# gligen/GLIGEN

Hardware: AMD Instinct MI355X
Metric: 512x512 images/sec @ 50 PLMS steps, box+text (CFG 7.5), UNet step ms (higher is better)
Workload: dtype bf16; 1 GPU; C2: box+text, 8 boxes (30 grounding tokens), 512x512, 50 PLMS steps, CFG 7.5, bf16 storage / fp32 accumulate; plms_steps=50, unet_evals_per_image=102, hipgraph=True, batches_in_flight=3

## Files before the change

gligen_amd/_lib.py:

```python
from __future__ import annotations

import ctypes as C
from pathlib import Path

_HERE = Path(__file__).resolve().parent
LIB_PATH = _HERE / "libgligen_amd.so"


class GligenAmdError(RuntimeError):
    pass


class UNetConfig(C.Structure):
    _fields_ = [
        ("in_channels", C.c_int), ("out_channels", C.c_int), ("model_channels", C.c_int),
        ("num_res_blocks", C.c_int), ("num_heads", C.c_int), ("context_dim", C.c_int),
        ("n_mult", C.c_int), ("channel_mult", C.c_int * 8),
        ("n_attn", C.c_int), ("attention_resolutions", C.c_int * 8),
        ("inpaint_mode", C.c_int), ("grounding_kind", C.c_int),
        ("gr_in_dim", C.c_int), ("gr_out_dim", C.c_int), ("max_persons", C.c_int), ("fuser_kind", C.c_int),
        ("extra_channels", C.c_int), ("tok_resize", C.c_int), ("tok_in_dim", C.c_int),
    ]


# ... 36 lines not shown
        ("fuser_scale", C.POINTER(C.c_float)), ("guidance_scale", C.c_float),
        ("x", C.c_void_p), ("inpaint_extra", C.c_void_p), ("mask", C.c_void_p), ("x0", C.c_void_p),
        ("noise", C.c_void_p), ("mask_B", C.c_int), ("x0_B", C.c_int), ("noise_B", C.c_int),
        ("sqrt_ac", C.POINTER(C.c_float)), ("sqrt_1mac", C.POINTER(C.c_float)),
        ("use_graph", C.c_int), ("sd_conv_w", C.c_void_p), ("sd_conv_b", C.c_void_p), ("sd_conv_step", C.c_int), ("ddim", C.c_int),
    ]


class TrainUNetIn(C.Structure):
    _fields_ = [(n, C.c_int) for n in ("B", "H", "W", "ctx_T", "Ng")] + \
               [(n, C.c_void_p) for n in ("x", "timesteps", "context", "boxes", "masks", "positive_embeddings", "target")] + \
               [("fuser_scale", C.c_float)] + [(n, C.c_void_p) for n in ("text_masks", "image_masks", "image_embeddings")] + [("checkpoint", C.c_int), ("use_weight_cache", C.c_int)]


class TrainSpatialIn(C.Structure):
    _fields_ = [("map", C.c_void_p)] + [(n, C.c_int) for n in ("map_channels", "map_h", "map_w")] + [("mask", C.c_void_p), ("extra", C.c_void_p)] + \
               [(n, C.c_int) for n in ("extra_in_channels", "extra_h", "extra_w", "ds_resize", "ds_mode", "ds_n_in", "ds_mid")]


class TrainSpatialClassesIn(C.Structure):
    _fields_ = [("map", C.c_void_p), ("map_h", C.c_int), ("map_w", C.c_int), ("mask", C.c_void_p), ("extra", C.c_void_p)] + \
               [(n, C.c_int) for n in ("extra_h", "extra_w", "ds_resize", "ds_mode", "ds_n_in", "ds_mid")]


class TrainStepInputsArgs(C.Structure):
    _fields_ = [("struct_size", C.c_uint)] + [(n, C.c_int) for n in ("B", "C", "H", "W", "n_t", "n_boxes", "inpaint")] + \
               [(n, C.c_void_p) for n in ("z", "noise", "timesteps", "sqrt_alphas_cumprod", "sqrt_one_minus_alphas_cumprod", "boxes", "mask",
                                          "x_rows", "target_rows", "t_float")]


class BoxCalibration(C.Structure):
    _fields_ = [("hbm_copy_gbs", C.c_float), ("lds_dma_tbs", C.c_float), ("mfma_bf16_tflops", C.c_float)]


class MfmaCalibration(C.Structure):
    _fields_ = [("tflops", C.c_float), ("sclk_mhz", C.c_float), ("ms", C.c_float), ("cycles_per_mfma", C.c_float)]


class ProfRec(C.Structure):
    _fields_ = [("name", C.c_char * 96), ("calls", C.c_int), ("ms", C.c_double), ("flops", C.c_double), ("bytes", C.c_double)]


_P = C.c_void_p
_I = C.c_int
SYMBOLS = {
    "gl_last_error": (C.c_char_p, []),
    "gl_ctx_create": (_I, [_I, C.c_size_t, C.POINTER(_P)]),
    "gl_ctx_fork": (_I, [_P, C.c_size_t, C.POINTER(_P)]),
    "gl_ctx_memory": (_I, [_P, C.POINTER(C.c_size_t), C.POINTER(C.c_size_t), C.POINTER(_I)]),
    "gl_ctx_destroy": (_I, [_P]),
    "gl_unet_configure": (_I, [_P, C.POINTER(UNetConfig)]),
    "gl_vae_configure": (_I, [_P, C.POINTER(VaeConfig)]),
    "gl_weight_upload": (_I, [_P, C.c_char_p, _P, _I, C.POINTER(C.c_int64), _I]),
    "gl_finalize": (_I, [_P]),
    "gl_clip_text_configure": (_I, [_P, C.POINTER(ClipTextConfig)]),
    "gl_clip_text_encode": (_I, [_P, _P, _P, _I, _I, _P, _P, _P]),
    "gl_clip_vision_configure": (_I, [_P, C.POINTER(ClipVisionConfig)]),
    "gl_clip_vision_encode": (_I, [_P, _P, _I, _P, _P, _P, _P]),
    "gl_op_clip_attention": (_I, [_P, _P, _P, _I, _I, _I, _I, _P]),
    "gl_unet_set_cond": (_I, [_P, _I, _P, _I, C.POINTER(Grounding), _P]),
    "gl_unet_set_fuser_scale": (_I, [_P, C.c_float, _P]),
    "gl_unet_set_fuser_scales": (_I, [_P, C.POINTER(C.c_float), _I, _P]),
    "gl_unet_grounding_tokens": (_I, [_P, _P, _P]),
    "gl_op_spatial_tokens": (_I, [_P, _P, _I, _I, _I, _I, _P, _P, _P]),
    "gl_op_grounding_downsample": (_I, [_P, _P, _I, _I, _I, _I, _I, _I, _I, _P, _P, _I, _P, _P, _I, _P, _P]),
    "gl_unet_restore_first_conv": (_I, [_P, _P, _P, _P]),
    "gl_unet_forward": (_I, [_P, _I, _I, _I, _P, _I, _P, _P, _I, _P, _P]),
    "gl_vae_decode": (_I, [_P, _I, _I, _I, _P, _P, _P]),
    "gl_vae_encode": (_I, [_P, _I, _I, _I, _P, _P, _P, _P]),
    "gl_sample_plms": (_I, [_P, C.POINTER(PlmsArgs), _P]),
    "gl_sampler_timing": (_I, [_P, C.POINTER(C.c_float), C.POINTER(C.c_float), C.POINTER(_I)]),
    "gl_unet_profile": (_I, [_P, _I, _I, _I, _P, _I, _P, _P, _I, _P, C.POINTER(ProfRec), _I, C.POINTER(_I), _P]),
    "gl_to_uint8": (_I, [_P, _P, _I, _I, _I, _P]),
    "gl_arena_high_water": (_I, [_P, C.POINTER(C.c_size_t)]),
    "gl_launch_count": (_I, [_P, C.POINTER(C.c_int64)]),
    "gl_set_ff_rows_policy": (_I, [_I]),
    "gl_ff_rows_policy_report": (_I, [C.c_char_p, C.c_size_t]),
    "gl_box_calibrate": (_I, [_P, C.POINTER(BoxCalibration), _P]),
    "gl_mfma_calibrate": (_I, [_P, _I, _I, _I, _I, C.c_float, C.POINTER(MfmaCalibration), _P]),
    "gl_op_linear": (_I, [_P, _P, _P, _P, _P, _P, _I, _I, _I, _I, _I, _P]),
    "gl_op_geglu": (_I, [_P, _P, _P, _P, _P, _I, _I, _I, _P]),
    "gl_op_ln_linear": (_I, [_P, _P, _I, _I, _P, _P, _P, _I, _P, _P, _P, _P, _I, _I, _I, _P, _P, C.POINTER(_I), _P]),
    "gl_op_feedforward": (_I, [_P, _P, _I, _I, _P, _P, _P, _P, _P, _P, _P, _P, _P, _P, C.POINTER(_I), _P]),
    "gl_train_block_param_names": (C.POINTER(C.c_char_p), []),
    "gl_op_block_train": (_I, [_P, _P, C.POINTER(_P), _P, _P, _P, _P, _P, _P, _P, _P, C.POINTER(_P), _P]),
    "gl_train_st_param_names": (C.POINTER(C.c_char_p), []),
    "gl_op_st_train": (_I, [_P, _P, C.POINTER(_P), _P, _P, _P, _P, _P, _P, _P, _P, C.POINTER(_P), _P]),
    "gl_train_resblock_param_names": (C.POINTER(C.c_char_p), []),
    "gl_op_resblock_train": (_I, [_P, _P, C.POINTER(_P), _P, _P, _P, _P, _P, _P, _P]),
    "gl_op_resample_train": (_I, [_P, _I, _I, _I, _I, _I, _P, _P, _P, _P, _P, _P, _P, _P]),
    "gl_unet_train_step": (_I, [_P, C.POINTER(UNetConfig), C.POINTER(TrainUNetIn), _I, C.POINTER(C.c_char_p), C.POINTER(_P), C.POINTER(_P), _P, _P, _P]),
    "gl_unet_train_step_spatial": (_I, [_P, C.POINTER(UNetConfig), C.POINTER(TrainUNetIn), C.POINTER(TrainSpatialIn), _I, C.POINTER(C.c_char_p),
                                        C.POINTER(_P), C.POINTER(_P), _P, _P, _P]),
    "gl_train_wait_grads": (_I, [_P, _I, _P]),
    "gl_train_weight_cache": (_I, [_P, _I, C.POINTER(C.c_size_t)]),
    "gl_op_adamw_step": (_I, [_P, _P, _P, _P, _P, C.c_int64, C.c_double, C.c_double, C.c_double, C.c_double, C.c_double, _I, _P]),
    "gl_op_ff_chain": (_I, [_P, _P, _I, _I] + [_P] * 16),
    "gl_op_conv3x3": (_I, [_P, _P, _I, _P, _I, _I, _I, _I, _P, _P, _I, _I, _I, _I, _P, _P, _P]),
    "gl_op_groupnorm": (_I, [_P, _P, _I, _P, _I, _I, _I, _P, _P, C.c_float, _I, _P, _P]),
    "gl_op_gn_silu_conv3x3": (_I, [_P, _P, _I, _P, _I, _I, _I, _I, _P, _P, C.c_float, _P, _P, _I, _P, _P, _P, _I, _P, _P]),
    "gl_op_layernorm": (_I, [_P, _P, _P, _I, _I, _I, _I, _I, _P, _P, C.c_float, _P, _P]),
    "gl_op_attention": (_I, [_P, _P, _P, _I, _I, _I, _I, _I, _I, _P, _P, _P, _P, _P]),
    "gl_attn_regime_counters": (_I, [_P, _I, C.POINTER(C.c_uint), C.POINTER(C.c_uint)]),
    "gl_op_ff_chain_q": (_I, [_P, _P, _I, _I, _I, _P, _P, _P, _P, _P, _P, _P, _P, _P, _P, _P, _P, _P, _P, _P, _P, _P]),
    "gl_op_proj_attention": (_I, [_P, _P, _I, _I, _I, _I, _P, _P, _P, _P, _P, _P, _P, _P, _I, _P, _P, C.POINTER(_I), _P]),
}

IMAGE_SYMBOLS = {
    "gl_op_image_resample": (_I, [_P, C.POINTER(ImageDesc), _I, _I, _I, C.POINTER(C.c_float), _P, _P]),
    "gl_image_resample_coeffs": (_I, [_I, _I, _I, C.POINTER(_I), C.POINTER(_I), _I, C.POINTER(_I), _I]),
}

MAP_SYMBOLS = {
    "gl_op_class_map_resize": (_I, [_P, C.POINTER(ClassMapDesc), _I, _I, _I, _P, _P]),
    "gl_class_map_index_table": (_I, [_I, _I, _I, C.POINTER(_I), _I]),
    "gl_op_spatial_tokens_classes": (_I, [_P, _P, _I, _I, _I, _P, _P, _P]),
    "gl_op_grounding_downsample_classes": (_I, [_P, _P, _I, _I, _I, _I, _I, _P, _P, _I, _P, _P, _I, _P, _P]),
}

TRAIN_MAP_SYMBOLS = {
    "gl_unet_train_step_spatial_classes": (_I, [_P, C.POINTER(UNetConfig), C.POINTER(TrainUNetIn), C.POINTER(TrainSpatialClassesIn), _I, C.POINTER(C.c_char_p),
                                                C.POINTER(_P), C.POINTER(_P), _P, _P, _P]),
    "gl_op_class_conv_wgrad": (_I, [_P, _I, _P, _I, _I, _I, _I, _I, _P, _I, _P, _P, _P]),
}

TRAIN_INPUT_SYMBOLS = {
    "gl_train_step_inputs": (_I, [_P, C.POINTER(TrainStepInputsArgs), _P]),
}

TRAIN_FUSER_SYMBOLS = {
    "gl_op_block_train_fuser": (_I, [_P, _I, _P, C.POINTER(_P), _P, _P, _P, _P, _P, _P, _P, _P, C.POINTER(_P), _P]),
    "gl_op_grid_resize": (_I, [_P, _P, _I, _I, _I, _I, _P, _P]),
    "gl_op_grid_resize_backward": (_I, [_P, _P, _I, _I, _I, _I, _P, _P]),
}

_F = C.c_float
TRAIN_PRIM_SYMBOLS = {
    "gl_op_train_attention": (_I, [_P, _I, _I, _I, _I, _I] + [_P] * 9 + [_P]),
    "gl_op_train_linear": (_I, [_P, _I, _I, _I] + [_P] * 8 + [_P]),
    "gl_op_train_layernorm": (_I, [_P, _I, _I, _F, _P, _P, _P, _P, _I] + [_P] * 6 + [_P]),
    "gl_op_train_groupnorm": (_I, [_P, _I, _I, _I, _I, _F, _P, _P, _P, _P, _I] + [_P] * 4 + [_P]),
    "gl_op_train_geglu": (_I, [_P, _I, _I, _P, _P, _P, _P, _P]),
    "gl_op_train_dot": (_I, [_P, C.c_int64, _P, _P, _P, _F, _I, _P, _P]),
}

TRAINER_SYMBOLS = {
    "gl_op_adamw_ema_step": (_I, [_P, _P, _P, _P, _P, _P, C.c_int64, C.c_double, C.c_double, C.c_double, C.c_double, C.c_double, C.c_double, _I, _P]),
}

SAMPLER_SYMBOLS = {
    "gl_set_cfg_shared_prefix": (_I, [_I]),
}

FUSER_KINDS = {"gatedSA": 0, "gatedSA2": 1, "gatedCA": 2}


def fuser_kind(fuser_type) -> int:
    try:
        return FUSER_KINDS[fuser_type or "gatedSA"]
    except KeyError:
        raise ValueError(f"fuser_type {fuser_type!r}: one of {sorted(FUSER_KINDS)}") from None


_lib = None


def load() -> C.CDLL:
    global _lib
    if _lib is not None:
        return _lib
    if not LIB_PATH.exists():
        raise GligenAmdError(
            f"{LIB_PATH} not found: build it with `python -m gligen_amd.build` "
            "(gligen_amd has no fallback path without its HIP library)")
    import torch
    lib = C.CDLL(str(LIB_PATH))
    for name, (res, args) in {**SYMBOLS, **IMAGE_SYMBOLS, **MAP_SYMBOLS, **TRAIN_MAP_SYMBOLS, **TRAIN_INPUT_SYMBOLS, **TRAIN_FUSER_SYMBOLS, **TRAIN_PRIM_SYMBOLS,
                              **TRAINER_SYMBOLS, **SAMPLER_SYMBOLS}.items():
        fn = getattr(lib, name)
        fn.restype = res
        fn.argtypes = args
    _lib = lib
    return lib


def check(rc: int) -> None:
    if rc != 0:
        msg = load().gl_last_error()
        raise GligenAmdError(f"libgligen_amd error {rc}: {msg.decode() if msg else '?'}")
```

gligen_amd/csrc/attention.h:

```cpp
#pragma once
#include "common.h"

namespace gl {

struct AttnParams {
    const bf16* q;
    const bf16* k;
    const bf16* vt;
    bf16* o;
    int H, d;
    int Nq, Nk;
    int Tq_pad, Tk_pad;
    int ldo;
    int o_rows_per_b;
    int nqb;
    float scale_log2e;
    int vt_layout;
    unsigned* counters = nullptr;
};
enum { ATTN_CTR_LAZY_MOVES = 0,
       ATTN_CTR_RERUNS = 1,
       ATTN_CTR_N = 2 };

int attn_dims(int d, int* DP, int* DPV);
int attn_vt_layout(int d, int Nk, int* DPV);
int attn_launch(const AttnParams& P, int B, hipStream_t stream);
const char* attn_kernel_name(int d, int Nk, int vt_layout = -1);
int attn_vt_ones_launch(bf16* vt, int BH, int d, int Tk_pad, hipStream_t stream, int DPV = 0);

int attn_k_init_launch(bf16* k, int BH, int d, int Tk_pad, hipStream_t stream);

}
```

gligen_amd/csrc/attention.hip:

```cpp
#include "attention.h"
#include "gemm.h"

#include <cstdlib>
#include <type_traits>

namespace gl {

__device__ __forceinline__ float max_xor32(float x) {
    const unsigned u = __float_as_uint(x);
    const auto r = __builtin_amdgcn_permlane32_swap(u, u, false, false);
    return fmaxf(__uint_as_float(r[0]), __uint_as_float(r[1]));
}

template <int DP, int DPV, bool ONES>
__global__ void __launch_bounds__(256, DP == 48 ? 3 : 1) attn_kernel(AttnParams P) {
    constexpr bool BIAS = DP == 48 && ONES;
    constexpr int KS = DP / 16;
    constexpr int DT = DPV / 32;
    constexpr int KROW = DP * 2 + 16;
    constexpr int VROW = 64 * 2 + 16;
    constexpr int KBYTES = 64 * KROW;
    constexpr int VBYTES = DPV * VROW;
    constexpr int STAGE = KBYTES + VBYTES;
    constexpr int KCH = 64 * DP / 8;
// ... 398 lines not shown
            for (int i = 0; i < DT; ++i) {
                ot[i] = __builtin_amdgcn_mfma_f32_32x32x16_bf16(vfa[2 * i], pb0, ot[i], 0, 0, 0);
                ot[i] = __builtin_amdgcn_mfma_f32_32x32x16_bf16(vfa[2 * i + 1], pb1, ot[i], 0, 0, 0);
            }
#pragma unroll
            for (int e = 0; e < 8; ++e) {
                pb2[e] = f2bf(__builtin_amdgcn_exp2f(BIAS ? sc[1][e] : sc[1][e] - m_run));
                pb3[e] = f2bf(__builtin_amdgcn_exp2f(BIAS ? sc[1][8 + e] : sc[1][8 + e] - m_run));
            }
            __builtin_amdgcn_sched_barrier(0);
            asm volatile("s_waitcnt lgkmcnt(0)");
            pin_regs(vfb);
#pragma unroll
            for (int i = 0; i < DT; ++i) {
                ot[i] = __builtin_amdgcn_mfma_f32_32x32x16_bf16(vfb[2 * i], pb2, ot[i], 0, 0, 0);
                ot[i] = __builtin_amdgcn_mfma_f32_32x32x16_bf16(vfb[2 * i + 1], pb3, ot[i], 0, 0, 0);
            }
        }
        if constexpr (QK) {
            if constexpr (TAILCK) {
                const int kv0 = j << 6;
                if (kv0 + 64 > P.Nk) {
#pragma unroll
                    for (int u = 0; u < 2; ++u)
#pragma unroll
                        for (int r = 0; r < 16; ++r) {
                            const int kv = kv0 + 32 * u + (r & 3) + 8 * (r >> 2) + 4 * half;
                            if (kv >= P.Nk) sn[u][r] = -1e30f;
                        }
                }
            }
            float mx = sn[0][0];
#pragma unroll
            for (int u = 0; u < 2; ++u)
#pragma unroll
                for (int r = 0; r < 16; ++r) mx = fmaxf(mx, sn[u][r]);
            mx = max_xor32(mx);
            __builtin_amdgcn_sched_barrier(0);
            if constexpr (BIAS) {
                const bool move = FIRSTMOVE || mx > 6.f;
                if (__builtin_amdgcn_ballot_w64(move) != 0) {
                    const bf16 mb = f2bf(m_run + mx);
                    const float m_upd = move ? (float)mb : m_run;
                    const float delta = m_upd - m_run;
                    if constexpr (!FIRSTMOVE) {
                        const float alpha = __builtin_amdgcn_exp2f(-delta);
#pragma unroll
                        for (int i = 0; i < DT; ++i)
#pragma unroll
                            for (int r = 0; r < 16; ++r) ot[i][r] *= alpha;
                    }
#pragma unroll
                    for (int u = 0; u < 2; ++u)
#pragma unroll
                        for (int r = 0; r < 16; ++r) sn[u][r] -= delta;
                    m_run = m_upd;
                    const bf16 nb = f2bf(-m_upd);
                    if (half == 1) qf[2][0] = nb;
                }
            } else {
                const bool move = FIRSTMOVE || mx - m_run > 6.f;
                if (__builtin_amdgcn_ballot_w64(move) != 0) {
                    const float m_upd = move ? mx : m_run;
                    if constexpr (!FIRSTMOVE) {
                        const float alpha = __builtin_amdgcn_exp2f(m_run - m_upd);
#pragma unroll
                        for (int i = 0; i < DT; ++i)
#pragma unroll
                            for (int r = 0; r < 16; ++r) ot[i][r] *= alpha;
                    }
                    m_run = m_upd;
                }
            }
        }
    };

    using T_ = std::true_type;
    using F_ = std::false_type;
    using S0 = std::integral_constant<int, 0>;
    using S1 = std::integral_constant<int, 1>;
    using SR = std::integral_constant<int, -1>;
    using I0 = std::integral_constant<int, 0>;
    using I1 = std::integral_constant<int, 1>;
    using I2 = std::integral_constant<int, 2>;
    using I3 = std::integral_constant<int, 3>;
    f32x16 sa[2], sb2[2];
    iter(0, sb2, sa, S0{}, I3{}, F_{}, T_{}, T_{}, T_{});
    if (nt == 1) {
        iter(1, sa, sb2, S1{}, I0{}, T_{}, F_{}, F_{}, F_{});
    } else {
        int j = 1;
        for (; j + 1 <= nt - 2; j += 2) {
            iter(j, sa, sb2, S1{}, I1{}, T_{}, T_{}, F_{}, F_{});
            iter(j + 1, sb2, sa, S0{}, I1{}, T_{}, T_{}, F_{}, F_{});
        }
        if (j <= nt - 2) {
            iter(j, sa, sb2, S1{}, I1{}, T_{}, T_{}, F_{}, F_{});
            ++j;
            iter(j, sb2, sa, S0{}, I2{}, T_{}, T_{}, T_{}, F_{});
            iter(j + 1, sa, sb2, S1{}, I0{}, T_{}, F_{}, F_{}, F_{});
        } else {
            iter(j, sa, sb2, S1{}, I2{}, T_{}, T_{}, T_{}, F_{});
            iter(j + 1, sb2, sa, S0{}, I0{}, T_{}, F_{}, F_{}, F_{});
        }
    }

    const int off = P.d & 31;
    const int rr = ((off >> 3) << 2) | (off & 3);
    float cand = 0.f;
#pragma unroll
    for (int i = 0; i < DT; ++i)
#pragma unroll
        for (int r = 0; r < 16; ++r)
            if (i == (P.d >> 5) && r == rr) cand = ot[i][r];
    const float other = __shfl_xor(cand, 32, 64);
    const float l_tot = (((off >> 2) & 1) == half) ? cand : other;
    const float inv = 1.f / l_tot;
    if (myq < P.Nq) {
        bf16* orow = P.o + ((size_t)b * P.o_rows_per_b + myq) * P.ldo + h * P.d;
#pragma unroll
        for (int i = 0; i < DT; ++i)
#pragma unroll
            for (int q4 = 0; q4 < 4; ++q4) {
                int dd0 = 32 * i + 8 * q4 + 4 * half;
                if (dd0 < P.d) {
                    U2BF4 o;
#pragma unroll
                    for (int e = 0; e < 4; ++e) o.e[e] = f2bf(ot[i][4 * q4 + e] * inv);
                    *reinterpret_cast<uint2*>(orow + dd0) = o.u;
                }
            }
    }
}

__device__ __forceinline__ void swap16(bf16x8& x, bf16x8& y) {
    typedef unsigned u32x4_t __attribute__((ext_vector_type(4)));
    u32x4_t a = __builtin_bit_cast(u32x4_t, x), b = __builtin_bit_cast(u32x4_t, y);
#pragma unroll
    for (int w = 0; w < 4; ++w) {
        const auto r = __builtin_amdgcn_permlane16_swap(a[w], b[w], false, false);
        a[w] = r[0];
        b[w] = r[1];
    }
    x = __builtin_bit_cast(bf16x8, a);
    y = __builtin_bit_cast(bf16x8, b);
}
template <int N, int I = 0>
__device__ __forceinline__ void lds_rd_v16(bf16x8 (&d)[N], unsigned a) {
    if constexpr (I < N) {
        lds_rd16<I * 2048>(d[I], a);
        lds_rd_v16<N, I + 1>(d, a);
    }
}
template <int DP, int DPV, bool BIAS, int NW, bool COUNT>
__global__ void __launch_bounds__(NW * 64, NW == 4 ? 2 : 1) attn3_kernel(AttnParams P) {
    static_assert(DP % 16 == 0 && DPV % 16 == 0 && DPV > DP - 8, "tile geometry");
    constexpr int KS = DP / 16;
    constexpr int DB = DPV / 16;
    constexpr int KP = DP / 8, VP = DPV / 8;
    constexpr int KBYTES = KP * 1024, VBYTES = VP * 1024, STAGE = KBYTES + VBYTES;
    constexpr int KR = (KP + NW - 1) / NW, VR = (VP + NW - 1) / NW;
    constexpr bool LATE_V = DPV > 64;
    typedef float f32x4_t __attribute__((ext_vector_type(4)));

    extern __shared__ __attribute__((aligned(16))) unsigned char smem[];

    const int t = threadIdx.x;
    const int lane = t & 63;
    const int wave = __builtin_amdgcn_readfirstlane(t >> 6);
    const int lrow = lane & 31;
    const int half = lane >> 5;
    const int l15 = lane & 15;
    const int g4 = lane >> 4;
    int lin = blockIdx.x;
    {
        const int total = gridDim.x;
        if ((total & 7) == 0) lin = (lin & 7) * (total >> 3) + (lin >> 3);
    }
    const int qblk = lin % P.nqb;
    const int bhi = lin / P.nqb;
    const int h = bhi % P.H;
    const int b = bhi / P.H;
    const size_t bh = (size_t)bhi;

    const bf16* __restrict__ Qg = P.q + bh * P.Tq_pad * DP;
    const bf16* __restrict__ Kg = P.k + bh * P.Tk_pad * DP;
    const bf16* __restrict__ Vg = P.vt + bh * DPV * P.Tk_pad;
    const __amdgpu_buffer_rsrc_t rk = __builtin_amdgcn_make_buffer_rsrc((void*)Kg, 0, 0x80000000u, 0x00020000);
    const __amdgpu_buffer_rsrc_t rv = __builtin_amdgcn_make_buffer_rsrc((void*)Vg, 0, 0x80000000u, 0x00020000);

    const int nt = (P.Nk + 63) >> 6;
    const int q0 = qblk * (NW * 32) + wave * 32;
    const int myq = q0 + lrow;
    const int myq_ld = myq < P.Tq_pad ? myq : P.Tq_pad - 1;

    const lds_ptr lbase = (lds_ptr)smem;
    const int w1k = wave * 1024;
    const unsigned lane16 = (unsigned)lane * 16u;
    unsigned vvoff[VR];
#pragma unroll
    for (int i = 0; i < VR; ++i) {
        const int r = 8 * (wave + NW * i) + (lane >> 3);
        const int c = (lane & 7) ^ ((r >> 1) & 7);
        vvoff[i] = (unsigned)(r * P.Tk_pad) * 2u + (unsigned)c * 16u;
    }
    auto issue_k = [&](int jj, int slot) {
        const lds_ptr st = lbase + slot * STAGE + w1k;
        const int so = jj * KBYTES + w1k;
#pragma unroll
        for (int i = 0; i < KR; ++i) {
            if ((i + 1) * NW <= KP) GL_BLDS16(rk, st + i * NW * 1024, lane16, so + i * NW * 1024);
            else if (wave < KP - i * NW) GL_BLDS16(rk, st + i * NW * 1024, lane16, so + i * NW * 1024);
        }
    };
    auto issue_v = [&](int jj, int slot) {
        const lds_ptr st = lbase + slot * STAGE + KBYTES + w1k;
        const int so = (jj - 1) * 128;
#pragma unroll
        for (int i = 0; i < VR; ++i) {
            if ((i + 1) * NW <= VP) GL_BLDS16(rv, st + i * NW * 1024, vvoff[i], so);
            else if (wave < VP - i * NW) GL_BLDS16(rv, st + i * NW * 1024, vvoff[i], so);
        }
    };
    issue_k(0, 0);

    bf16x8 qf[KS];
#pragma unroll
    for (int s = 0; s < KS; ++s) qf[s] = *reinterpret_cast<const bf16x8*>(Qg + (size_t)myq_ld * DP + 16 * s + 8 * half);
#pragma unroll
    for (int s = 0; s < KS; ++s)
#pragma unroll
        for (int e = 0; e < 8; ++e) qf[s][e] = f2bf((float)qf[s][e] * P.scale_log2e);
    if constexpr (BIAS) {
        if (half == 1) qf[2][0] = f2bf(0.f);
    }

    f32x4_t ot[2][DB];
#pragma unroll
    for (int qh = 0; qh < 2; ++qh)
#pragma unroll
        for (int i = 0; i < DB; ++i)
#pragma unroll
            for (int r = 0; r < 4; ++r) ot[qh][i][r] = 0.f;
    float m_run = BIAS ? 0.f : -1e30f;
    constexpr bool LAZY = BIAS;
    constexpr int LAZY_LOG2 = 40;
    constexpr int D_ROW = BIAS ? 40 : DP;
    constexpr int OB = D_ROW >> 4, OG = (D_ROW & 15) >> 2, ORR = D_ROW & 3;
    bool overshoot = false;

    const unsigned k_lane = (unsigned)(lrow * 16 + half * 1024);
    const unsigned v_lane = KBYTES + (unsigned)(l15 * 128) + (unsigned)((g4 ^ ((l15 >> 1) & 7)) << 4);

    auto iter = [&](int j, f32x16 (&sc)[2], f32x16 (&sn)[2], auto slot_c, auto issue_c, auto sm_c, auto qk_c, auto tail_c, auto first_c, auto safe_c) {
        constexpr bool SAFE = !LAZY || decltype(safe_c)::value;
        constexpr int SLOT = decltype(slot_c)::value, ISSUE = decltype(issue_c)::value;
        constexpr bool SM = decltype(sm_c)::value, QK = decltype(qk_c)::value, TAILCK = decltype(tail_c)::value, FIRSTMOVE = decltype(first_c)::value;
        __builtin_amdgcn_s_waitcnt(0x0F70);
        __builtin_amdgcn_s_barrier();
        asm volatile("" ::: "memory");
        const int slot = SLOT >= 0 ? SLOT : (j & 1);
        if constexpr (ISSUE != 0) {
            if constexpr (ISSUE == 1) issue_k(j + 1, slot ^ 1);
            if constexpr (ISSUE == 3) { if (j + 1 < nt) issue_k(j + 1, slot ^ 1); }
            issue_v(j + 1, slot ^ 1);
        }
        if constexpr (LAZY && SM && !SAFE) {
            {
                const bool big = g4 == OG && (ot[0][OB][ORR] > __builtin_ldexpf(1.f, LAZY_LOG2) || ot[1][OB][ORR] > __builtin_ldexpf(1.f, LAZY_LOG2));
                if (__builtin_amdgcn_ballot_w64(big) != 0) {
                    if constexpr (COUNT) { if (lane == 0) atomicAdd(P.counters + ATTN_CTR_LAZY_MOVES, 1u); }
                    const float la = __shfl(ot[0][OB][ORR], 16 * OG + l15, 64), lb = __shfl(ot[1][OB][ORR], 16 * OG + l15, 64);
                    const float lq = lrow < 16 ? la : lb;
                    overshoot |= !(lq < 1.0e30f);
                    const float e = lq > __builtin_ldexpf(1.f, LAZY_LOG2) ? (float)((int)((__float_as_uint(lq) >> 23) & 0xffu) - 127) : 0.f;
                    const bf16 mb = f2bf(m_run + e);
                    const float m_upd = (float)mb;
                    const float delta = m_upd - m_run;
                    const float alpha = __builtin_amdgcn_exp2f(-delta);
                    const auto ar = __builtin_amdgcn_permlane16_swap(__float_as_uint(alpha), __float_as_uint(alpha), false, false);
                    const float a0 = __uint_as_float(ar[0]), a1 = __uint_as_float(ar[1]);
#pragma unroll
                    for (int i = 0; i < DB; ++i)
#pragma unroll
                        for (int r = 0; r < 4; ++r) { ot[0][i][r] *= a0; ot[1][i][r] *= a1; }
#pragma unroll
                    for (int u = 0; u < 2; ++u)
#pragma unroll
                        for (int r = 0; r < 16; ++r) sc[u][r] -= delta;
                    m_run = m_upd;
                    const bf16 nb = f2bf(-m_upd);
                    if (half == 1) qf[2][0] = nb;
                }
            }
        }
        const unsigned sb = (unsigned)(slot * STAGE);
        const unsigned ak = k_lane + sb;
        const unsigned av0 = v_lane + sb, av1 = av0 ^ 64u;

        bf16x8 kf[2 * KS], vfa[DB], vfb[LATE_V ? 1 : DB];
        if constexpr (QK) lds_rd_k(kf, ak);
        if constexpr (SM && !LATE_V) lds_rd_v16(vfa, av0);
        if constexpr (QK) {
            if constexpr (SM && !LATE_V) asm volatile("s_waitcnt lgkmcnt(%0)" ::"n"(DB));
            else asm volatile("s_waitcnt lgkmcnt(0)");
            pin_regs(kf);
            const f32x16 zero = {0.f, 0.f, 0.f, 0.f, 0.f, 0.f, 0.f, 0.f, 0.f, 0.f, 0.f, 0.f, 0.f, 0.f, 0.f, 0.f};
            sn[0] = __builtin_amdgcn_mfma_f32_32x32x16_bf16(kf[0], qf[0], zero, 0, 0, 0);
            sn[1] = __builtin_amdgcn_mfma_f32_32x32x16_bf16(kf[1], qf[0], zero, 0, 0, 0);
#pragma unroll
            for (int s = 1; s < KS; ++s) {
                sn[0] = __builtin_amdgcn_mfma_f32_32x32x16_bf16(kf[2 * s], qf[s], sn[0], 0, 0, 0);
                sn[1] = __builtin_amdgcn_mfma_f32_32x32x16_bf16(kf[2 * s + 1], qf[s], sn[1], 0, 0, 0);
            }
        }
        if constexpr (SM) {
            bf16x8 px, py;
#pragma unroll
            for (int e = 0; e < 8; ++e) {
                px[e] = f2bf(__builtin_amdgcn_exp2f(BIAS ? sc[0][e] : sc[0][e] - m_run));
                py[e] = f2bf(__builtin_amdgcn_exp2f(BIAS ? sc[0][8 + e] : sc[0][8 + e] - m_run));
            }
            if constexpr (!LATE_V) {
                swap16(px, py);
                __builtin_amdgcn_sched_barrier(0);
                lds_rd_v16(vfb, av1);
                asm volatile("s_waitcnt lgkmcnt(%0)" ::"n"(DB));
            } else {
                __builtin_amdgcn_sched_barrier(0);
                lds_rd_v16(vfa, av0);
                swap16(px, py);
                asm volatile("s_waitcnt lgkmcnt(0)");
            }
            pin_regs(vfa);
#pragma unroll
            for (int i = 0; i < DB; ++i) {
                ot[0][i] = __builtin_amdgcn_mfma_f32_16x16x32_bf16(vfa[i], px, ot[0][i], 0, 0, 0);
                ot[1][i] = __builtin_amdgcn_mfma_f32_16x16x32_bf16(vfa[i], py, ot[1][i], 0, 0, 0);
            }
            bf16x8 pz, pw;
#pragma unroll
            for (int e = 0; e < 8; ++e) {
                pz[e] = f2bf(__builtin_amdgcn_exp2f(BIAS ? sc[1][e] : sc[1][e] - m_run));
                pw[e] = f2bf(__builtin_amdgcn_exp2f(BIAS ? sc[1][8 + e] : sc[1][8 + e] - m_run));
            }
            if constexpr (!LATE_V) {
                swap16(pz, pw);
                __builtin_amdgcn_sched_barrier(0);
                asm volatile("s_waitcnt lgkmcnt(0)");
                pin_regs(vfb);
            } else {
                __builtin_amdgcn_sched_barrier(0);
                lds_rd_v16(vfa, av1);
                swap16(pz, pw);
                asm volatile("s_waitcnt lgkmcnt(0)");
                pin_regs(vfa);
            }
            bf16x8 (&vf2)[DB] = *reinterpret_cast<bf16x8 (*)[DB]>(LATE_V ? &vfa[0] : &vfb[0]);
#pragma unroll
            for (int i = 0; i < DB; ++i) {
                ot[0][i] = __builtin_amdgcn_mfma_f32_16x16x32_bf16(vf2[i], pz, ot[0][i], 0, 0, 0);
                ot[1][i] = __builtin_amdgcn_mfma_f32_16x16x32_bf16(vf2[i], pw, ot[1][i], 0, 0, 0);
            }
        }
        if constexpr (QK) {
            if constexpr (TAILCK) {
                const int kv0 = j << 6;
                if (kv0 + 64 > P.Nk) {
#pragma unroll
                    for (int u = 0; u < 2; ++u)
#pragma unroll
                        for (int r = 0; r < 16; ++r) {
                            const int kv = kv0 + 32 * u + (r & 3) + 8 * (r >> 2) + 4 * half;
                            if (kv >= P.Nk) sn[u][r] = -1e30f;
                        }
                }
            }
          if constexpr (FIRSTMOVE || SAFE) {
            float mx = sn[0][0];
#pragma unroll
            for (int u = 0; u < 2; ++u)
#pragma unroll
                for (int r = 0; r < 16; ++r) mx = fmaxf(mx, sn[u][r]);
            mx = max_xor32(mx);
            __builtin_amdgcn_sched_barrier(0);
            auto rescale_o = [&](float alpha) {
                const auto ar = __builtin_amdgcn_permlane16_swap(__float_as_uint(alpha), __float_as_uint(alpha), false, false);
                const float a0 = __uint_as_float(ar[0]), a1 = __uint_as_float(ar[1]);
#pragma unroll
                for (int i = 0; i < DB; ++i)
#pragma unroll
                    for (int r = 0; r < 4; ++r) { ot[0][i][r] *= a0; ot[1][i][r] *= a1; }
            };
            if constexpr (BIAS) {
                const bool move = FIRSTMOVE || mx > 6.f;
                if (__builtin_amdgcn_ballot_w64(move) != 0) {
                    const bf16 mb = f2bf(m_run + mx);
                    const float m_upd = move ? (float)mb : m_run;
                    const float delta = m_upd - m_run;
                    if constexpr (!FIRSTMOVE) rescale_o(__builtin_amdgcn_exp2f(-delta));
#pragma unroll
                    for (int u = 0; u < 2; ++u)
#pragma unroll
                        for (int r = 0; r < 16; ++r) sn[u][r] -= delta;
                    m_run = m_upd;
                    const bf16 nb = f2bf(-m_upd);
                    if (half == 1) qf[2][0] = nb;
                }
            } else {
                const bool move = FIRSTMOVE || mx - m_run > 6.f;
                if (__builtin_amdgcn_ballot_w64(move) != 0) {
                    const float m_upd = move ? mx : m_run;
                    if constexpr (!FIRSTMOVE) rescale_o(__builtin_amdgcn_exp2f(m_run - m_upd));
                    m_run = m_upd;
                }
            }
          }
        }
    };

    using T_ = std::true_type;
    using F_ = std::false_type;
    using S0 = std::integral_constant<int, 0>;
    using S1 = std::integral_constant<int, 1>;
    using I0 = std::integral_constant<int, 0>;
    using I1 = std::integral_constant<int, 1>;
    using I2 = std::integral_constant<int, 2>;
    using I3 = std::integral_constant<int, 3>;
    f32x16 sa[2], sb2[2];
#define GL_ATTN3_TILES(SAFE_T) \
    iter(0, sb2, sa, S0{}, I3{}, F_{}, T_{}, T_{}, T_{}, SAFE_T{}); \
    if (nt == 1) { \
        iter(1, sa, sb2, S1{}, I0{}, T_{}, F_{}, F_{}, F_{}, SAFE_T{}); \
    } else { \
        int j = 1; \
        for (; j + 1 <= nt - 2; j += 2) { \
            iter(j, sa, sb2, S1{}, I1{}, T_{}, T_{}, F_{}, F_{}, SAFE_T{}); \
            iter(j + 1, sb2, sa, S0{}, I1{}, T_{}, T_{}, F_{}, F_{}, SAFE_T{}); \
        } \
        if (j <= nt - 2) { \
            iter(j, sa, sb2, S1{}, I1{}, T_{}, T_{}, F_{}, F_{}, SAFE_T{}); \
            ++j; \
            iter(j, sb2, sa, S0{}, I2{}, T_{}, T_{}, T_{}, F_{}, SAFE_T{}); \
            iter(j + 1, sa, sb2, S1{}, I0{}, T_{}, F_{}, F_{}, F_{}, SAFE_T{}); \
        } else { \
            iter(j, sa, sb2, S1{}, I2{}, T_{}, T_{}, T_{}, F_{}, SAFE_T{}); \
            iter(j + 1, sb2, sa, S0{}, I0{}, T_{}, F_{}, F_{}, F_{}, SAFE_T{}); \
        } \
    }
    GL_ATTN3_TILES(F_)
    if constexpr (LAZY) {
        const float c0 = ot[0][OB][ORR], c1 = ot[1][OB][ORR];
        const bool bad = overshoot || (g4 == OG && (!(c0 > 0.f && c0 < 1.0e30f) || !(c1 > 0.f && c1 < 1.0e30f)));
        volatile unsigned* flags = reinterpret_cast<volatile unsigned*>(smem);
        __builtin_amdgcn_s_barrier();
        const unsigned wave_bad = __builtin_amdgcn_ballot_w64(bad) != 0 ? 1u : 0u;
        if (lane == 0) flags[wave] = wave_bad;
        __builtin_amdgcn_s_waitcnt(0xC07F);
        __builtin_amdgcn_s_barrier();
        unsigned any_bad = 0;
#pragma unroll
        for (int w = 0; w < NW; ++w) any_bad |= flags[w];
        __builtin_amdgcn_s_waitcnt(0xC07F);
        __builtin_amdgcn_s_barrier();
        if (any_bad) {
            if constexpr (COUNT) { if (t == 0) atomicAdd(P.counters + ATTN_CTR_RERUNS, 1u); }
#pragma unroll
            for (int qh = 0; qh < 2; ++qh)
#pragma unroll
                for (int i = 0; i < DB; ++i)
#pragma unroll
                    for (int r = 0; r < 4; ++r) ot[qh][i][r] = 0.f;
            m_run = 0.f;
            if (half == 1) qf[2][0] = f2bf(0.f);
            issue_k(0, 0);
            GL_ATTN3_TILES(T_)
        }
    }
#undef GL_ATTN3_TILES

    const int ob = P.d >> 4, og = (P.d & 15) >> 2, orr = P.d & 3;
#pragma unroll
    for (int qh = 0; qh < 2; ++qh) {
        float cand = 0.f;
#pragma unroll
        for (int i = 0; i < DB; ++i)
#pragma unroll
            for (int r = 0; r < 4; ++r)
                if (i == ob && r == orr) cand = ot[qh][i][r];
        const float l_tot = __shfl(cand, 16 * og + l15, 64);
        const float inv = 1.f / l_tot;
        const int q = q0 + 16 * qh + l15;
        if (q < P.Nq) {
            bf16* orow = P.o + ((size_t)b * P.o_rows_per_b + q) * P.ldo + h * P.d;
#pragma unroll
            for (int i = 0; i < DB; ++i) {
                const int dd0 = 16 * i + 4 * g4;
                if (dd0 < P.d) {
                    U2BF4 o;
#pragma unroll
                    for (int e = 0; e < 4; ++e) o.e[e] = f2bf(ot[qh][i][e] * inv);
                    *reinterpret_cast<uint2*>(orow + dd0) = o.u;
                }
            }
        }
    }
}

template <int DP, int DPV, bool BIAS, int NW>
static int launch_attn3(const AttnParams& P, int B, hipStream_t stream) {
    const size_t lds = 2 * ((DP / 8) * 1024 + (DPV / 8) * 1024);
    AttnParams Q = P;
    Q.nqb = cdiv(P.Nq, NW * 32);
    dim3 grid(Q.nqb * P.H * B);
    if (P.counters) hipLaunchKernelGGL((attn3_kernel<DP, DPV, BIAS, NW, true>), grid, dim3(NW * 64), lds, stream, Q);
    else hipLaunchKernelGGL((attn3_kernel<DP, DPV, BIAS, NW, false>), grid, dim3(NW * 64), lds, stream, Q);
    GL_LAUNCH_CHECK();
    return GL_OK;
}

template <int DP, int DPV, bool BIAS, int NW>
static int launch_attn2(const AttnParams& P, int B, hipStream_t stream) {
    const size_t lds = 2 * ((DP / 8) * 1024 + (DPV / 8) * 1024);
    AttnParams Q = P;
    Q.nqb = cdiv(P.Nq, NW * 32);
    dim3 grid(Q.nqb * P.H * B);
    return launch_lds<attn2_kernel<DP, DPV, BIAS, NW>>(grid, dim3(NW * 64), lds, stream, Q);
}

template <int DP, int DPV, bool ONES>
static int launch_attn(const AttnParams& P, int B, hipStream_t stream) {
    constexpr int KROW = DP * 2 + 16, VROW = 144;
    size_t lds = 2 * (64 * KROW + DPV * VROW);
    AttnParams Q = P;
    Q.nqb = cdiv(P.Nq, 128);
    dim3 grid(Q.nqb * P.H * B);
    return launch_lds<attn_kernel<DP, DPV, ONES>>(grid, dim3(256), lds, stream, Q);
}

int attn_dims(int d, int* DP, int* DPV) {
    switch (d) {
        case 40: *DP = 48; *DPV = 64; return GL_OK;
        case 80: *DP = 80; *DPV = 96; return GL_OK;
        case 160: *DP = 160; *DPV = 160; return GL_OK;
        default: return set_error(GL_ERR_UNSUPPORTED, "attention: head dim %d not supported (40, 80, 160)", d);
    }
}

__global__ void vt_ones_kernel(bf16* vt, int DPV, int Tk_pad, int d) {
    bf16* row = vt + ((size_t)blockIdx.x * DPV + d) * Tk_pad;
    for (int i = threadIdx.x; i < Tk_pad; i += blockDim.x) row[i] = (bf16)1.0f;
}
int attn_vt_ones_launch(bf16* vt, int BH, int d, int Tk_pad, hipStream_t stream, int DPV) {
    int dp, dpv;
    GL_TRY(attn_dims(d, &dp, &dpv));
    if (DPV) dpv = DPV;
    if (dpv == d) return GL_OK;
    hipLaunchKernelGGL(vt_ones_kernel, dim3(BH), dim3(256), 0, stream, vt, dpv, Tk_pad, d);
    GL_LAUNCH_CHECK();
    return GL_OK;
}

static int attn_v2_mode() {
    static const int m = dev_env("GL_ATTN_V2") ? atoi(dev_env("GL_ATTN_V2")) : 3;
    return m;
}

static bool attn_use_v2(int d, int Nk) { return Nk > 128 && ((d == 40 && attn_v2_mode() != 0) || (d == 80 && attn_v2_mode() == 3)); }

int attn_vt_layout(int d, int Nk, int* DPV) {
    int dp, dpv = 0;
    (void)attn_dims(d, &dp, &dpv);
    const int layout = (attn_use_v2(d, Nk) && attn_v2_mode() >= 3) ? 1 : 0;
    if (DPV) *DPV = (layout && d == 40) ? 48 : dpv;
    return layout;
}

const char* attn_kernel_name(int d, int Nk, int vt_layout) {
    int v2 = attn_use_v2(d, Nk) ? attn_v2_mode() : 0;
    if (vt_layout == 0 && v2 >= 3) v2 = 1;
    if (d == 40) return v2 == 0 ? "attn_kernel<48, 64, true>" : v2 == 1 ? "attn2_kernel<48, 64, true, 4>" : v2 == 2 ? "attn2_kernel<48, 64, true, 8>" : "attn3_kernel<48, 48, true, 4>";
    if (d == 80) return (v2 >= 3 && vt_layout != 0) ? "attn3_kernel<80, 96, false, 4>" : "attn_kernel<80, 96, true>";
    return "attn_kernel<160, 160, false>";
}

__global__ void k_ones_kernel(bf16* k, int DP, int Tk_pad, int col) {
    bf16* slab = k + (size_t)blockIdx.x * Tk_pad * DP;
    for (int t = threadIdx.x; t < Tk_pad; t += blockDim.x) slab[ktile_off(0, Tk_pad, t, col, DP)] = (bf16)1.0f;
}
int attn_k_init_launch(bf16* k, int BH, int d, int Tk_pad, hipStream_t stream) {
    if (d != 40) return GL_OK;
    hipLaunchKernelGGL(k_ones_kernel, dim3(BH), dim3(256), 0, stream, k, 48, Tk_pad, 40);
    GL_LAUNCH_CHECK();
    return GL_OK;
}

int attn_launch(const AttnParams& P, int B, hipStream_t stream) {
    if (P.Nq <= 0 || P.Nk <= 0) return set_error(GL_ERR_ARG, "attention: empty Nq=%d Nk=%d", P.Nq, P.Nk);
    if (P.Tq_pad % 128 != 0 || P.Tk_pad % 64 != 0 || P.Tq_pad < P.Nq || P.Tk_pad < P.Nk)
        return set_error(GL_ERR_ARG, "attention: bad padding Tq_pad=%d Tk_pad=%d (Nq=%d Nk=%d)", P.Tq_pad, P.Tk_pad, P.Nq, P.Nk);
    int v2 = attn_use_v2(P.d, P.Nk) ? attn_v2_mode() : 0;
    if (P.vt_layout == 1) {
        if (P.d == 40) return launch_attn3<48, 48, true, 4>(P, B, stream);
        if (P.d == 80) return launch_attn3<80, 96, false, 4>(P, B, stream);
        return set_error(GL_ERR_ARG, "attention: vt_layout 1 exists for head dims 40 and 80 (d = %d)", P.d);
    }
    if (v2 >= 3) v2 = 1;
    switch (P.d) {
        case 40:
            if (v2 == 1) return launch_attn2<48, 64, true, 4>(P, B, stream);
            if (v2 >= 2) return launch_attn2<48, 64, true, 8>(P, B, stream);
            return launch_attn<48, 64, true>(P, B, stream);
        case 80:
            return launch_attn<80, 96, true>(P, B, stream);
        case 160: return launch_attn<160, 160, false>(P, B, stream);
        default: return set_error(GL_ERR_UNSUPPORTED, "attention: head dim %d not supported (40, 80, 160)", P.d);
    }
}

}
```

gligen_amd/csrc/capi.hip:

```cpp
#include "classmap.h"
#include "engine_impl.h"
#include "image.h"
#include "train.h"
#include "train_fusers.h"
#include "../../include/gligen_amd_train_maps.h"
#include "../../include/gligen_amd_train_inputs.h"
#include "../../include/gligen_amd_train_fusers.h"
#include "../../include/gligen_amd_train_prims.h"
#include "../../include/gligen_amd_trainer.h"
#include "../../include/gligen_amd_sampler.h"

#include <cstdlib>

#include <cmath>

using namespace gl;

struct gl_ctx {
    std::shared_ptr<Engine> holder;
    Engine* eng;
    ImageStage image_stage;
};

#define GL_API_BEGIN try {
#define GL_API_END                                       \
    }                                                    \
    catch (const gl::GlError& e) {                       \
        return gl::set_error(e.code, "%s", e.what());    \
    }                                                    \
    catch (const std::exception& e) {                    \
        return gl::set_error(GL_ERR_STATE, "%s", e.what()); \
    }                                                    \
    return GL_OK;

struct DeviceGuard {
    int prev = -1;
    bool ok = true;
    explicit DeviceGuard(int dev) {
        if (hipGetDevice(&prev) != hipSuccess) prev = -1;
        if (prev != dev) ok = hipSetDevice(dev) == hipSuccess;
        else prev = -1;
    }
    ~DeviceGuard() {
        if (prev >= 0) (void)hipSetDevice(prev);
    }
};
#define NEED(ctx)                                                         \
    if (!(ctx) || !(ctx)->eng) return gl::set_error(GL_ERR_ARG, "null context"); \
    DeviceGuard device_guard_((ctx)->eng->device());                      \
    if (!device_guard_.ok) return gl::set_error(GL_ERR_HIP, "hipSetDevice(%d) failed", (ctx)->eng->device());

static inline hipStream_t S(gl_stream s) { return reinterpret_cast<hipStream_t>(s); }
#define HIPCK_API(expr)                                                                           \
    do {                                                                                          \
        hipError_t _e = (expr);                                                                   \
        if (_e != hipSuccess) throw GlError(GL_ERR_HIP, std::string(#expr) + ": " + hipGetErrorString(_e)); \
    } while (0)

extern "C" {

const char* gl_last_error(void) { return gl::last_error(); }

int gl_ctx_create(int device, size_t arena_bytes, gl_ctx** out) {
    if (!out) return gl::set_error(GL_ERR_ARG, "null out pointer");
    GL_API_BEGIN
    int ndev = 0;
    hipError_t e = hipGetDeviceCount(&ndev);
    if (e != hipSuccess || ndev <= 0)
        throw GlError(GL_ERR_HIP, "no HIP device available: libgligen_amd has no CPU path");
    if (device < 0 || device >= ndev) throw GlError(GL_ERR_ARG, "device index out of range");
    if (hipSetDevice(device) != hipSuccess) throw GlError(GL_ERR_HIP, "hipSetDevice failed");
    hipDeviceProp_t prop;
    if (hipGetDeviceProperties(&prop, device) != hipSuccess) throw GlError(GL_ERR_HIP, "hipGetDeviceProperties failed");
    if (std::string(prop.gcnArchName).rfind("gfx950", 0) != 0)
        throw GlError(GL_ERR_UNSUPPORTED, std::string("libgligen_amd is built for gfx950 (MI355X); device is ") + prop.gcnArchName);
    std::shared_ptr<Engine> eng(new Engine(device));
    eng->arena().init(arena_bytes ? arena_bytes : (size_t(8) << 30));
    eng->init_workspace();
    *out = new gl_ctx{eng, eng.get(), {}};
    GL_API_END
}

int gl_ctx_fork(gl_ctx* parent, size_t arena_bytes, gl_ctx** out) {
    NEED(parent);
    if (!out) return gl::set_error(GL_ERR_ARG, "null out pointer");
    GL_API_BEGIN
    std::shared_ptr<Engine> e = Engine::fork(parent->holder, arena_bytes);
    *out = new gl_ctx{e, e.get(), {}};
    GL_API_END
}

int gl_ctx_memory(gl_ctx* ctx, size_t* own_bytes, size_t* arena_bytes, int* is_fork) {
    NEED(ctx);
    GL_API_BEGIN
    if (own_bytes) *own_bytes = ctx->eng->weight_bytes();
    if (arena_bytes) *arena_bytes = ctx->eng->arena_bytes();
    if (is_fork) *is_fork = ctx->eng->is_fork() ? 1 : 0;
    GL_API_END
}

int gl_ctx_destroy(gl_ctx* ctx) {
    if (!ctx) return GL_OK;
    GL_API_BEGIN
    (void)hipDeviceSynchronize();
    delete ctx;
    GL_API_END
}

int gl_unet_configure(gl_ctx* ctx, const gl_unet_config* cfg) {
    NEED(ctx);
    if (!cfg) return gl::set_error(GL_ERR_ARG, "null config");
    GL_API_BEGIN
    ctx->eng->configure_unet(*cfg);
    GL_API_END
}

int gl_vae_configure(gl_ctx* ctx, const gl_vae_config* cfg) {
    NEED(ctx);
    if (!cfg) return gl::set_error(GL_ERR_ARG, "null config");
    GL_API_BEGIN
    ctx->eng->configure_vae(*cfg);
    GL_API_END
}

int gl_weight_upload(gl_ctx* ctx, const char* key, const void* data, int ndim, const int64_t* shape, int is_device) {
    NEED(ctx);
    if (!key || !data || ndim < 0 || (ndim > 0 && !shape)) return gl::set_error(GL_ERR_ARG, "bad weight upload arguments");
    GL_API_BEGIN
    ctx->eng->upload(key, data, ndim, shape, is_device != 0);
    GL_API_END
}

int gl_finalize(gl_ctx* ctx) {
    NEED(ctx);
    GL_API_BEGIN
    ctx->eng->finalize();
    GL_API_END
}

int gl_clip_text_configure(gl_ctx* ctx, const gl_clip_text_config* cfg) {
    NEED(ctx);
    if (!cfg) return gl::set_error(GL_ERR_ARG, "null config");
    GL_API_BEGIN
    ctx->eng->configure_clip_text(*cfg);
    GL_API_END
}

int gl_clip_text_encode(gl_ctx* ctx, const int32_t* ids, const int32_t* eos_index, int n_seq, int n_tok, float* last_hidden, float* pooled, gl_stream s) {
    NEED(ctx);
    GL_API_BEGIN
    ctx->eng->clip_text_encode(ids, eos_index, n_seq, n_tok, last_hidden, pooled, S(s));
    GL_API_END
}

int gl_clip_vision_configure(gl_ctx* ctx, const gl_clip_vision_config* cfg) {
    NEED(ctx);
    if (!cfg) return gl::set_error(GL_ERR_ARG, "null config");
    GL_API_BEGIN
    ctx->eng->configure_clip_vision(*cfg);
    GL_API_END
}

int gl_clip_vision_encode(gl_ctx* ctx, const float* pixel_values, int n_img, float* last_hidden, float* pooled, float* image_embeds, gl_stream s) {
// ... 818 lines not shown
    return train_step_spatial("gl_unet_train_step_spatial_classes", ctx, cfg, in, spi, n_params, names, params, grads, eps_out, loss, s);
}

int gl_train_step_inputs(gl_ctx* ctx, const gl_train_step_inputs_args* args, gl_stream s) {
    NEED(ctx);
    if (!args) return gl::set_error(GL_ERR_ARG, "gl_train_step_inputs: null args");
    if (args->struct_size != sizeof(gl_train_step_inputs_args))
        return gl::set_error(GL_ERR_ARG, "gl_train_step_inputs: args->struct_size is %u, this library's gl_train_step_inputs_args has %zu bytes (set it to "
                                         "sizeof(gl_train_step_inputs_args))", args->struct_size, sizeof(gl_train_step_inputs_args));
    GL_API_BEGIN
    gl::TrainStepInputs a{args->B, args->C, args->H, args->W, args->n_t, args->n_boxes, args->inpaint ? 1 : 0, args->z, args->noise, args->timesteps,
                          args->sqrt_alphas_cumprod, args->sqrt_one_minus_alphas_cumprod, args->boxes, args->mask, args->x_rows, args->target_rows, args->t_float};
    GL_TRY(gl::train_step_inputs_launch(a, S(s)));
    ++ctx->eng->n_launches;
    GL_API_END
}

int gl_op_class_conv_wgrad(gl_ctx* ctx, int kind, const uint8_t* cls, int B, int H, int W, int n_classes, int R, const float* dy, int c_out,
                           float* dW, float* db, gl_stream s) {
    NEED(ctx);
    if (!cls || !dy || (!dW && !db)) return gl::set_error(GL_ERR_ARG, "gl_op_class_conv_wgrad: null class map / dy, or neither gradient asked for");
    GL_API_BEGIN
    size_t n = 0;
    GL_TRY(class_conv_wgrad_partial_floats(kind, B, H, W, n_classes, c_out, R, &n));
    gl::Arena& ar = ctx->eng->arena();
    const size_t mk = ar.mark();
    float* part = ar.get<float>(n);
    const size_t Ro = kind == kClassWgradDown ? R / 2 : R;
    const int rc = class_conv_wgrad_launch(kind, cls, dy, {(size_t)c_out * Ro * Ro, Ro * Ro, Ro, 1}, part, dW, db, B, H, W, n_classes, c_out, R, S(s));
    ar.release(mk);
    if (rc != GL_OK) return rc;
    ctx->eng->n_launches += 2;
    GL_API_END
}

int gl_train_weight_cache(gl_ctx* ctx, int enable, size_t* bytes) {
    NEED(ctx);
    GL_API_BEGIN
    Engine& eng = *ctx->eng;
    if (enable && !eng.train_cache) eng.train_cache = gl::train_cache_create();
    if (!enable && eng.train_cache) {
        HIPCK_API(hipDeviceSynchronize());
        gl::train_cache_destroy(eng.train_cache);
        eng.train_cache = nullptr;
    }
    if (bytes) *bytes = gl::train_cache_bytes(eng.train_cache);
    GL_API_END
}

int gl_train_wait_grads(gl_ctx* ctx, int index, gl_stream s) {
    NEED(ctx);
    GL_API_BEGIN
    Engine& eng = *ctx->eng;
    if (index < 0 || index >= Engine::kTrainEvents) throw GlError(GL_ERR_ARG, "gl_train_wait_grads: milestone index out of range");
    if (!eng.train_events_recorded) throw GlError(GL_ERR_STATE, "gl_train_wait_grads: no gl_unet_train_step has run on this context");
    HIPCK_API(hipStreamWaitEvent(S(s), eng.train_events()[index], 0));
    GL_API_END
}

int gl_op_conv3x3(gl_ctx* ctx, const void* x0, int C0, const void* x1, int C1, int B, int H, int W,
                  const float* w_oihw, const float* bias, int Cout, int stride, int ups, int pad_lo,
                  const void* res, void* y, gl_stream s) {
    NEED(ctx);
    GL_API_BEGIN
    Arena& ar = ctx->eng->arena();
    ar.reset();
    const int Cin = C0 + C1;
    if (stride == 1 && ups == 1 && pad_lo == 1 && !res && Engine::upconv_phase_form(Cin, Cout)) {
        ConvW c;
        c.Cin = Cin; c.Cout = Cout; c.Npad = Cout; c.b = bias;
        bf16* w4 = ar.get<bf16>((size_t)16 * Cout * Cin);
        const int rp = pack_upconv_phases_launch(w_oihw, w4, Cout, Cin, Cout, S(s));
        if (rp != GL_OK) throw GlError(rp, gl::last_error());
        c.w4 = w4;
        ctx->eng->conv3x3(TRef{(const bf16*)x0, C0, (const bf16*)x1, C1}, B, H, W, c, 1, 1, 1, nullptr, 0, nullptr, S(s), (bf16*)y);
        return GL_OK;
    }
    bf16* wp = ar.get<bf16>((size_t)Cout * 9 * Cin);
    int r = pack_conv_weight_launch(w_oihw, wp, Cout, Cin, 3, 3, Cout, S(s));
    if (r != GL_OK) throw GlError(r, gl::last_error());
    const int Hup = H << ups, Wup = W << ups;
    const int Ho = stride == 1 ? Hup : (pad_lo ? (Hup + 2 - 3) / 2 + 1 : (Hup + 1 - 3) / 2 + 1);
    const int Wo = stride == 1 ? Wup : (pad_lo ? (Wup + 2 - 3) / 2 + 1 : (Wup + 1 - 3) / 2 + 1);
    AOperand A{};
    A.p0 = (const bf16*)x0; A.C0 = C0; A.ld0 = C0; A.p1 = (const bf16*)x1; A.C1 = C1; A.ld1 = C1;
    A.mode = A_CONV3; A.Hin = H; A.Win = W; A.Ho = Ho; A.Wo = Wo; A.stride = stride; A.ups = ups; A.pad_lo = pad_lo;
    Epilogue E;
    epilogue_defaults(E);
    E.out = y; E.ldo = Cout; E.bias = bias; E.res = (const bf16*)res; E.ldres = Cout; E.rows_per_b = Ho * Wo;
    r = gemm_launch(A, wp, B * Ho * Wo, Cout, 9 * Cin, E, ctx->eng->splitk_ws(), ctx->eng->splitk_ws_bytes(), S(s));
    if (r != GL_OK) throw GlError(r, gl::last_error());
    GL_API_END
}

int gl_op_gn_silu_conv3x3(gl_ctx* ctx, const void* x0, int C0, const void* x1, int C1, int B, int H, int W, const float* gamma, const float* beta,
                          float eps, const float* w_oihw, const float* bias, int Cout, const float* bias2, const void* res, void* y, int mode,
                          int* used_prologue, gl_stream s) {
    NEED(ctx);
    if (!x0 || !gamma || !beta || !w_oihw || !y || !used_prologue) return gl::set_error(GL_ERR_ARG, "gl_op_gn_silu_conv3x3: null pointer");
    GL_API_BEGIN
    Engine& eng = *ctx->eng;
    Arena& ar = eng.arena();
    ar.reset();
    const int Cin = C0 + C1;
    bf16* wp = ar.get<bf16>((size_t)Cout * 9 * Cin);
    int r = pack_conv_weight_launch(w_oihw, wp, Cout, Cin, 3, 3, Cout, S(s));
    if (r != GL_OK) throw GlError(r, gl::last_error());
    NormW n;
    n.g = gamma; n.b = beta; n.C = Cin;
    ConvW c;
    c.w = wp; c.b = bias; c.Cin = Cin; c.Cout = Cout;
    const bool saved = eng.gn_prologue_;
    if (mode >= 0) eng.gn_prologue_ = mode != 0;
    const int64_t n0 = eng.n_prologue_convs;
    try {
        eng.gn_silu_conv3x3(TRef{(const bf16*)x0, C0, (const bf16*)x1, C1}, B, H, W, n, eps, c, bias2, Cout, (const bf16*)res, (bf16*)y, S(s));
    } catch (...) {
        eng.gn_prologue_ = saved;
        throw;
    }
    eng.gn_prologue_ = saved;
    *used_prologue = eng.n_prologue_convs > n0 ? 1 : 0;
    if (mode == 1 && !*used_prologue) throw GlError(GL_ERR_UNSUPPORTED, "gl_op_gn_silu_conv3x3: this shape has no GroupNorm prologue (conv_halo_kernel, H W % 256 == 0)");
    GL_API_END
}

int gl_op_groupnorm(gl_ctx* ctx, const void* x0, int C0, const void* x1, int C1, int B, int HW,
                    const float* gamma, const float* beta, float eps, int silu, void* y, gl_stream s) {
    NEED(ctx);
    GL_API_BEGIN
    Arena& ar = ctx->eng->arena();
    ar.reset();
    GNParams P{};
    P.x0 = (const bf16*)x0; P.C0 = C0; P.x1 = (const bf16*)x1; P.C1 = C1; P.B = B; P.HW = HW; P.eps = eps;
    P.gamma = gamma; P.beta = beta; P.y = (bf16*)y; P.silu = silu;
    P.partial = reinterpret_cast<float*>(ar.alloc(gn_partial_bytes(B, HW)));
    int r = groupnorm_launch(P, S(s));
    if (r != GL_OK) throw GlError(r, gl::last_error());
    GL_API_END
}

int gl_op_layernorm(gl_ctx* ctx, const void* x, const void* x2, int B, int N1, int N2, int Tpad, int C,
                    const float* gamma, const float* beta, float eps, void* y, gl_stream s) {
    NEED(ctx);
    GL_API_BEGIN
    LNParams P{};
    P.x = (const bf16*)x; P.x2 = (const bf16*)x2; P.B = B; P.N1 = N1; P.N2 = N2; P.Tpad = Tpad; P.C = C; P.eps = eps;
    P.gamma = gamma; P.beta = beta; P.y = (bf16*)y;
    int r = layernorm_launch(P, S(s));
    if (r != GL_OK) throw GlError(r, gl::last_error());
    GL_API_END
}

int gl_op_attention(gl_ctx* ctx, const void* xq, const void* xkv, int B, int Nq, int Nk, int C, int Ck, int H,
                    const float* wq, const float* wk, const float* wv, void* o, gl_stream s) {
    NEED(ctx);
    GL_API_BEGIN
    Engine& eng = *ctx->eng;
    Arena& ar = eng.arena();
    ar.reset();
    if (C % H != 0) throw GlError(GL_ERR_ARG, "C must be divisible by H");
    const int d = C / H;
    int dp, dpv;
    int r = attn_dims(d, &dp, &dpv);
    if (r != GL_OK) throw GlError(r, gl::last_error());
    const int Tq = round_up(Nq, 64), Tk = round_up(Nk, 64);
    const int vt_layout = attn_vt_layout(d, Nk, &dpv);
    AttnBufs& bufs = eng.attn_bufs(B, H, d, Tq, Tk, dpv);
    bf16* wqb = ar.get<bf16>((size_t)C * C);
    bf16* wkb = ar.get<bf16>((size_t)C * Ck);
    bf16* wvb = ar.get<bf16>((size_t)C * Ck);
    bf16* xqp = ar.get<bf16>((size_t)B * Tq * C);
    bf16* xkp = ar.get<bf16>((size_t)B * Tk * Ck);
    auto ck = [&](int rc) { if (rc != GL_OK) throw GlError(rc, gl::last_error()); };
    ck(cast_f32_bf16_launch(wq, wqb, (int64_t)C * C, S(s)));
    ck(cast_f32_bf16_launch(wk, wkb, (int64_t)C * Ck, S(s)));
    ck(cast_f32_bf16_launch(wv, wvb, (int64_t)C * Ck, S(s)));
    ck(pad_rows_bf16_launch((const bf16*)xq, xqp, B, Nq, Tq, C, S(s)));
    ck(pad_rows_bf16_launch((const bf16*)xkv, xkp, B, Nk, Tk, Ck, S(s)));
    const bool fused = xq == xkv && C == Ck && Nq == Nk && gemm_supports_qkv() && (2 * C) % 128 == 0 &&
                       !(dev_env("GL_QKV_FUSED") && atoi(dev_env("GL_QKV_FUSED")) == 0);
    if (fused) {
        bf16* wqkv = ar.get<bf16>((size_t)3 * C * C);
        ck(cast_f32_bf16_launch(wq, wqkv, (int64_t)C * C, S(s)));
        ck(cast_f32_bf16_launch(wk, wqkv + (size_t)C * C, (int64_t)C * C, S(s)));
        ck(cast_f32_bf16_launch(wv, wqkv + (size_t)2 * C * C, (int64_t)C * C, S(s)));
        Epilogue E = e_heads(EPI_QKV_HEADS, bufs.q, bufs.k, C, H, d, dp, Tq, bufs.Tq_pad, bufs.Tk_pad);
        E.vt = bufs.vt; E.DPV = dpv; E.vt_perm32 = vt_layout;
        ck(gemm_launch(a_rows(xqp, C), wqkv, B * Tq, 3 * C, C, E, nullptr, 0, S(s)));
    } else {
        ck(gemm_launch(a_rows(xqp, C), wqb, B * Tq, C, C, e_heads(EPI_QK_HEADS, bufs.q, nullptr, C, H, d, dp, Tq, bufs.Tq_pad, 0), eng.splitk_ws(),
                       eng.splitk_ws_bytes(), S(s)));
        {
            Epilogue E = e_heads(EPI_QK_HEADS, bufs.k, nullptr, C, H, d, dp, Tk, bufs.Tk_pad, 0);
            E.q_tiled = 1;
            ck(gemm_launch(a_rows(xkp, Ck), wkb, B * Tk, C, Ck, E, eng.splitk_ws(), eng.splitk_ws_bytes(), S(s)));
        }
        {
            Epilogue E;
            epilogue_defaults(E);
            E.mode = EPI_VT_HEADS; E.out = bufs.vt; E.H = H; E.d = d; E.DPV = dpv; E.T = Tk; E.Tpad_k = bufs.Tk_pad; E.vt_perm32 = vt_layout;
            ck(gemm_launch_t(wvb, C, xkp, B * Tk, Ck, E, S(s)));
        }
    }
    AttnParams P = attn_params(bufs.q, bufs.k, bufs.vt, (bf16*)o, H, d, Nq, Nk, bufs.Tq_pad, bufs.Tk_pad, vt_layout);
    P.counters = eng.attn_counters();
    ck(attn_launch(P, B, S(s)));
    GL_API_END
}

int gl_attn_regime_counters(gl_ctx* ctx, int enable, unsigned* lazy_moves, unsigned* reruns) {
    NEED(ctx);
    if (!lazy_moves || !reruns) return gl::set_error(GL_ERR_ARG, "gl_attn_regime_counters: null pointer");
    GL_API_BEGIN
    unsigned c[ATTN_CTR_N];
    ctx->eng->attn_regime_counters(enable, c);
    *lazy_moves = c[ATTN_CTR_LAZY_MOVES];
    *reruns = c[ATTN_CTR_RERUNS];
    GL_API_END
}


int gl_op_proj_attention(gl_ctx* ctx, const void* x, int B, int N, int C, int H, const float* pre_w, const float* pre_b, const void* pre_res,
                         const float* gamma, const float* beta, const float* wq, const float* wk, const float* wv, int Nkv_extra,
                         void* mid, void* o, int* used_rows, gl_stream s) {
    NEED(ctx);
    if (!x || !pre_w || !pre_b || !gamma || !beta || !wq || !wk || !wv || !mid || !o || !used_rows)
        return gl::set_error(GL_ERR_ARG, "gl_op_proj_attention: null pointer");
    GL_API_BEGIN
    Engine& eng = *ctx->eng;
    Arena& ar = eng.arena();
    ar.reset();
    auto ck = [&](int rc) { if (rc != GL_OK) throw GlError(rc, gl::last_error()); };
    if (C % H != 0 || N % 64 != 0 || Nkv_extra != 0) throw GlError(GL_ERR_ARG, "gl_op_proj_attention: C % H == 0, N % 64 == 0");
    const int d = C / H, M = B * N;
    int dp, dpv;
    ck(attn_dims(d, &dp, &dpv));
    const int vt_layout = attn_vt_layout(d, N, &dpv);
    AttnBufs& bufs = eng.attn_bufs(B, H, d, N, N, dpv);
    bf16* wqkv = ar.get<bf16>((size_t)3 * C * C);
    float* bias = ar.get<float>((size_t)3 * C);
    {
        float* wf = ar.get<float>((size_t)C * C);
        const float* ws[3] = {wq, wk, wv};
        for (int i = 0; i < 3; ++i) {
            ck(ln_fold_launch(ws[i], nullptr, gamma, beta, wf, bias + (size_t)i * C, C, C, S(s)));
            ck(cast_f32_bf16_launch(wf, wqkv + (size_t)i * C * C, (int64_t)C * C, S(s)));
        }
    }
    const bool want = *used_rows != 0;
    const bool rows = want && qkv_rows_supported(M, C, d, N) && vt_layout == 1;
    *used_rows = rows ? 1 : 0;
    if (rows) {
        void* st = ar.alloc(qkv_rows_stream_bytes(C, true, 3));
        ck(qkv_rows_pack_launch(pre_w, wqkv, 3, st, C, S(s)));
        QkvRowsParams P{};
        P.x = (const bf16*)x; P.ldx = C; P.eps = 1e-5f; P.stream = st; P.M = M;
        P.pre = 1; P.pre_b = pre_b; P.pre_res = (const bf16*)pre_res; P.ld_pre_res = C; P.mid_out = (bf16*)mid; P.ld_mid = C;
        P.np = 3; P.bias = bias; P.q = bufs.q; P.k = bufs.k; P.vt = bufs.vt;
        P.H = H; P.d = d; P.DP = dp; P.DPV = dpv; P.T = N; P.Tpad_q = bufs.Tq_pad; P.Tpad_k = bufs.Tk_pad; P.vt_perm32 = vt_layout;
        ck(qkv_rows_launch(P, C, S(s)));
    } else {
        bf16* pw = ar.get<bf16>((size_t)C * C);
        ck(cast_f32_bf16_launch(pre_w, pw, (int64_t)C * C, S(s)));
        {
            ck(gemm_launch(a_rows((const bf16*)x, C), pw, M, C, C, e_rows_res(mid, C, pre_b, (const bf16*)pre_res), eng.splitk_ws(), eng.splitk_ws_bytes(), S(s)));
        }
        bf16* xn = ar.get<bf16>((size_t)M * C);
        LNParams L{};
        L.x = (const bf16*)mid; L.B = 1; L.N1 = M; L.N2 = 0; L.Tpad = M; L.C = C; L.eps = 1e-5f; L.y = xn;
        ck(layernorm_launch(L, S(s)));
        Epilogue E = e_heads(EPI_QKV_HEADS, bufs.q, bufs.k, C, H, d, dp, N, bufs.Tq_pad, bufs.Tk_pad);
        E.vt = bufs.vt; E.DPV = dpv; E.vt_perm32 = vt_layout; E.bias = bias;
        ck(gemm_launch(a_rows(xn, C), wqkv, M, 3 * C, C, E, nullptr, 0, S(s)));
    }
    ck(attn_launch(attn_params(bufs.q, bufs.k, bufs.vt, (bf16*)o, H, d, N, N, bufs.Tq_pad, bufs.Tk_pad, vt_layout), B, S(s)));
    GL_API_END
}

}
```

gligen_amd/csrc/engine.h:

```cpp
#pragma once
#include <array>
#include <map>
#include <memory>
#include <stdexcept>
#include <string>
#include <unordered_map>
#include <unordered_set>
#include <vector>

#include "arena.h"
#include "attention.h"
#include "clip.h"
#include "common.h"
#include "convnext.h"
#include "ffn.h"
#include "gemm.h"
#include "misc.h"
#include "norm.h"
#include "train.h"
#include "../../include/gligen_amd.h"

namespace gl {

struct RawTensor {
// ... 123 lines not shown
    Arena& arena() { return arena_; }
    float* splitk_ws() { return ws_; }
    size_t splitk_ws_bytes() const { return ws_bytes_; }
    void* persist(size_t bytes, bool zero);
    void init_workspace();
    AttnBufs& attn_bufs(int B, int H, int d, int Tq, int Tk, int dpv_layout = 0, int slot = 0);
    void attn_regime_counters(int enable, unsigned* out);
    unsigned* attn_counters() const { return attn_counting_ ? attn_ctr_ : nullptr; }

    bf16* gn_silu_conv3x3(const TRef& x, int B, int H, int W, const NormW& n, float eps, const ConvW& c, const float* bias2, int bias2_ld,
                          const bf16* res, bf16* out, hipStream_t s);
    bf16* conv3x3(const TRef& x, int B, int Hin, int Win, const ConvW& c, int stride, int ups, int pad_lo,
                  const float* bias2, int bias2_ld, const bf16* res, hipStream_t s, bf16* out = nullptr);
    static bool upconv_phase_form(int Cin, int Cout);
    bool gn_prologue_ = dev_env("GL_GN_PROLOGUE") && atoi(dev_env("GL_GN_PROLOGUE")) == 1;
    int64_t n_prologue_convs = 0;
    int device() const { return device_; }
    int64_t n_launches = 0;
    static constexpr int kTrainEvents = 64;
    hipEvent_t* train_events();
    bool train_events_recorded = false;
    TrainWeightCache* train_cache = nullptr;

    struct ProfRec { std::string name; int calls = 0; double ms = 0, flops = 0, bytes = 0; };
    void profile_begin();
    std::vector<ProfRec> profile_end(hipStream_t s);

   private:
    struct ProfEvt { std::string name; double flops, bytes; hipEvent_t e0, e1; };
    bool profiling_ = false;
    std::vector<ProfEvt> prof_;
    std::vector<hipEvent_t> prof_pool_;
    struct ProfScope {
        Engine* e; hipStream_t s; size_t idx;
        ProfScope(Engine* eng, hipStream_t st, const std::string& name, double flops, double bytes);
        ~ProfScope();
        void rename(const std::string& n) { if (e->profiling_) e->prof_[idx].name = n; }
    };
    friend struct ProfScope;
    const RawTensor& raw(const std::string& key) const;
    bool has(const std::string& key) const { return raw_.count(key) != 0; }
    const float* F(const std::string& key) const { return raw(key).p; }
    const float* FK(const std::string& key) { keep_raw_.insert(key); return raw(key).p; }
    std::unordered_set<std::string> keep_raw_;
    NormW norm(const std::string& prefix);
    LinW linear(const std::string& prefix, bool bias = true);
    ConvW conv3(const std::string& prefix, int Npad = 0, bool up2x = false);
    ConvW conv3_small(const std::string& prefix, int Cout);
    LinW conv1(const std::string& prefix);
    const bf16* cast_rows(const std::vector<std::string>& weight_keys);
    FFW ffw(const std::string& prefix, int C, const NormW* fold = nullptr, const std::string& pre_key = "", const std::string& post_key = "",
            const float* post_q_w = nullptr, const float* post_q_b = nullptr);
    struct FoldTmp { float* w = nullptr; float* b = nullptr; int N = 0, K = 0; };
    FoldTmp fold_ln(const std::string& weight_key, const float* bias, const NormW& n);
    std::vector<void*> fold_tmps_;
    ResW resw(const std::string& prefix, int Cin, int Cout, bool unet);

    void gemm(const AOperand& A, const bf16* W, int M, int N, int K, const Epilogue& E, hipStream_t s);
    bf16* linear_rows(const bf16* x, int M, const LinW& L, int act, const bf16* res, const float* gate, hipStream_t s, RowStats* stats = nullptr);
    bf16* layernorm_plain(const bf16* x, int B, int N, int C, bool pad64, hipStream_t s);
    bf16* groupnorm(const TRef& x, int B, int HW, const NormW& n, float eps, bool silu, hipStream_t s);
    bf16* layernorm(const bf16* x, int B, int N, int C, const NormW& n, bool pad64, hipStream_t s);
    bf16* conv3x3_small(const ConvW& c, Im2colParams P, int reps, hipStream_t s);
    void gn_silu_conv3x3_nchw(const bf16* x, int C, int B, int H, int W, const NormW& n, float eps, const ConvW& c, int n_real, float* out, hipStream_t s);
    bf16* resblock(const ResW& r, const TRef& x, int B, int H, int W, const float* embout, int emb_ld, float eps, hipStream_t s, bf16* out = nullptr);
    void replicate(const bf16* src, bf16* dst, size_t n, int reps, hipStream_t s);
    void attention(const bf16* q, const bf16* k, const bf16* vt, bf16* o, int B, int H, int d, int Nq, int Nk, int Tq_pad, int Tk_pad, int vt_layout,
                   hipStream_t s);
    void spatial_tokens_tail(int B, const float* img, const float* mask, float* out, hipStream_t s);

    Engine(const Engine&) = default;
    Engine& operator=(const Engine&) = delete;
    std::shared_ptr<Engine> parent_;
    size_t persist_bytes_ = 0;
    int device_;
    bool finalized_ = false;
    std::unordered_map<std::string, RawTensor> raw_;
    std::vector<void*> owned_;
    Arena arena_;
    float* ws_ = nullptr;
    size_t ws_bytes_ = 0;
    typedef std::array<int, 7> AttnKey;
    std::map<AttnKey, AttnBufs> attn_bufs_;
    unsigned* attn_ctr_ = nullptr;
    bool attn_counting_ = false;
    std::vector<hipEvent_t> train_events_;

    struct Unet {
        bool present = false;
        gl_unet_config cfg{};
        LinW te0, te2;
        LinW embcat;
        ConvW conv_in_small;
        std::vector<ResW> res;
        std::vector<STW> st;
        std::vector<ConvW> updown;
        std::vector<UNetBlock> in_blocks, out_blocks;
        UNetBlock mid_block;
        NormW out_norm;
        ConvW out_conv;
        const float* const* alpha_ptrs = nullptr;
        int gkind = 0;
        LinW pn[2][3];
        const float* pn_null_feat[2] = {nullptr, nullptr};
        const float* pn_null_pos = nullptr;
        const float* kp_table = nullptr;
        CnxNet cnx;
    } unet_;
    bool ln_fold_ = false;
    bool ff_rows_ = true;
    int ff_chain_ = 2;
    int qkv_rows_ = 1;
    bool fuser_hoist_ = true;
    void build_unet();
    float* gates_ = nullptr;
    float* fuser_scale_ = nullptr;
    bool fuser_off_ = false;
    struct Cond {
        int Beff = 0, Ng = 0, ctx_T = 0, ctx_Tpad = 0, obj_Tpad = 0;
        bf16* tokens = nullptr;
        int obj_stride = 0;
        std::vector<bf16*> objs;
        std::vector<bf16*> obj_k;
        std::vector<bf16*> obj_vt;
        std::vector<bf16*> ctx_k;
        std::vector<bf16*> ctx_vt;
        std::vector<void*> allocs;
    } cond_;
    void fuser_kv_fill(const STW& t, int B, int HW, hipStream_t s);
    void ensure_fuser_kv(const STW& t, int B, int HW, hipStream_t s);
    struct FuserKV { uint64_t epoch = 0; int B = 0, HW = 0; };
    std::vector<FuserKV> fuser_kv_;
    uint64_t cond_epoch_ = 0;

    bf16* transformer(const STW& t, const bf16* x, int B, int Bp, int H, int W, hipStream_t s);
    bf16* feedforward(const FFW& f, const bf16* ln, int M, const bf16* res, const float* gate, hipStream_t s, const RowStats* in_stats = nullptr,
                      RowStats* out_stats = nullptr, bool raw_rows = false, bool use_rows = false);
    bf16* fuser_ff_tail(const STW& t, const bf16* o, const bf16* t1, int B, int HW, bool rows, hipStream_t s, RowStats* st3, bool* q_done = nullptr);
    AttnBufs& to_q_heads(const LinW& q, const bf16* ln, int B, int Tp, int C, int d, int Tk_pad, const RowStats* st, const float* csum, hipStream_t s);
    void cross_q_gemm(const STW& t, const bf16* rows, const RowStats& st, int B, int HW, hipStream_t s);
    bf16* concat_layernorm(const STW& t, const bf16* x, int B, int HW, int Tf, hipStream_t s);
    void block_ff_tail(const STW& t, const bf16* o, const bf16* t3, const bf16* x, bf16* out, int B, int HW, bool rows, hipStream_t s);
    bf16* ff_behind(const FFW& f, const NormW& nw, const bf16* rows_in, RowStats& st_in, int B, int HW, const float* gate, bool rows, hipStream_t s,
                    RowStats* out_stats);
    bool can_fold(const RowStats& st, int M, int C, int Nc, int mode, int act, bool aligned);
    struct ChainQ { bf16* q; int DP, T, Tpad; };
    bf16* feedforward_chain(const FFW& f, const bf16* x, int M, const LinW& pre, const bf16* pre_res, const float* pre_gate, const float* gate,
                            const LinW* post, const bf16* post_res, bf16* out, hipStream_t s, RowStats* out_stats, const ChainQ* cq = nullptr);
    void self_attention(const SelfAttnW& a, const bf16* ln, int B, int T, int Nq, int Nk, int C, int d, bf16* o, hipStream_t s,
                        const RowStats* in_stats = nullptr, int Tbuf = 0, int slot = 0, bool projected = false);
    bool qkv_rows_ok(const SelfAttnW& a, int B, int T, int Nk, int C, int d) const;
    void qkv_project_gemm(const SelfAttnW& a, const bf16* ln, int B, int T, int Nk, int C, int d, hipStream_t s, const RowStats* in_stats, int Tbuf, int slot);
    void qkv_rows_project(const SelfAttnW& a, const bf16* x, int B, int T, int Nk, int C, int d, const LinW& pre, const bf16* pre_res, bf16* mid,
                          RowStats* mid_stats, int Tbuf, int slot, hipStream_t s, int Bin = 0);
    float* emb_rows(const int64_t* t_dev, int R, float* out, hipStream_t s);
    void emb_table_build(const int64_t* t_host, int R, hipStream_t s);
    float* emb_table_ = nullptr;
    float* emb_cur_ = nullptr;
    int64_t* emb_t_dev_ = nullptr;
    int emb_table_cap_ = 0;
    std::vector<int64_t> emb_t_cache_;

    bool ff_rows_for(const STW& t, int which, int B, int HW, hipStream_t s);
    bool qkv_rows_for(const STW& t, int which, int B, int HW, int Nk, hipStream_t s);
    template <class Run>
    bool timed_form(uint64_t key, int M, int C, int n_zero, const char* name, int form, hipStream_t s, Run&& run);

    void build_convnext(const std::string& PN);

    struct VaeLevel { std::vector<ResW> blocks; bool has_resample = false; ConvW resample; };
    struct VaeHalf {
        bool present = false;
        ConvW in_small;
        ResW mid1, mid2;
        VaeAttnW attn;
        std::vector<VaeLevel> levels;
        NormW norm_out;
        ConvW conv_out;
        const float* quant_w = nullptr;
        const float* quant_b = nullptr;
    };
    struct Vae { gl_vae_config cfg{}; VaeHalf dec, enc; } vae_;
    void build_vae();
    void build_vae_encoder();
    void build_vae_mid(VaeHalf& h, const std::string& prefix, int C);
    bf16* vae_attn(const VaeAttnW& a, const bf16* x, int B, int HW, hipStream_t s);

    struct ClipLayerW { NormW ln1, ln2; LinW qkv, out, fc1, fc2; };
    struct ClipText {
        bool present = false;
        gl_clip_text_config cfg{};
        const float* tok = nullptr;
        const float* pos = nullptr;
        std::vector<ClipLayerW> layers;
        NormW final_ln;
        unsigned* bad_ids = nullptr;
    } clipt_;
    void build_clip_text();
    void clip_expect_shape(const std::string& key, int64_t d0, int64_t d1) const;
    void build_clip_layers(const std::string& P, int n, int width, int intermediate, std::vector<ClipLayerW>& out);
    struct ClipStack { int width, heads, intermediate; float ln_eps; };
    const float* clip_layers_run(const std::vector<ClipLayerW>& layers, const ClipStack& c, float* h, float* tmp, int S, int T, bool causal, hipStream_t s);
    struct ClipVision {
        bool present = false;
        gl_clip_vision_config cfg{};
        const float* cls = nullptr;
        const float* pos = nullptr;
        LinW patch;
        NormW pre_ln, post_ln;
        LinW proj;
        std::vector<ClipLayerW> layers;
    } clipv_;
    void build_clip_vision();

    struct Sampler {
        int B = 0, h = 0, w = 0;
        float* x2 = nullptr;
        float* eps_pair = nullptr;
        float* hist[4] = {nullptr, nullptr, nullptr, nullptr};
        float* x_tmp = nullptr;
        int64_t* t_dev = nullptr;
        hipGraph_t graph[2] = {nullptr, nullptr};
        hipGraphExec_t exec[2] = {nullptr, nullptr};
        hipStream_t stream = nullptr;
        hipStream_t run_stream = nullptr;
        bool ran = false;
        hipEvent_t ev_in = nullptr, ev_out = nullptr;
        hipEvent_t ev_done = nullptr;
        std::vector<hipEvent_t> tev;
        int n_evals = 0;
        bool has_extra = false;
        const float* extra = nullptr;
        bool warm[2] = {false, false};
        unsigned policy_epoch = 0;
    } smp_;
    void sampler_release_graph();
    void sampler_wait_idle();
};

}
```

gligen_amd/csrc/engine_policy.hip:

```cpp
#include "engine_impl.h"
#include <algorithm>
#include <atomic>
#include <map>
#include <mutex>

namespace gl {

namespace ff_policy {
static std::mutex mu;
struct Entry { int rows; float us_rows, us_gemm; };
static std::map<uint64_t, Entry> table;
static std::atomic<int> mode{-1};
static std::atomic<unsigned> epoch{1};
static uint64_t key(int dev, int which, int form, int C, int M) {
    return ((uint64_t)dev << 56) | ((uint64_t)which << 52) | ((uint64_t)form << 48) | ((uint64_t)C << 32) | (uint64_t)(unsigned)M;
}
static bool static_rule(int M) { return M / 128 >= 224; }
static int current_mode() {
    static const bool env_once = [] {
        if (const char* e = dev_env("GL_FF_POLICY")) mode.store(atoi(e));
        return true;
    }();
    (void)env_once;
    return mode.load();
}
}

int ff_rows_policy_set(int mode) {
    if (mode < -1 || mode > 2) return set_error(GL_ERR_ARG, "ff_rows policy %d (expected -1 timed, 0 never, 1 wherever supported, 2 static rule)", mode);
    if (ff_policy::mode.exchange(mode) != mode) ff_policy::epoch.fetch_add(1);
    return GL_OK;
}
unsigned ff_rows_policy_epoch() { return ff_policy::epoch.load(); }

namespace cfg_prefix {
static std::atomic<int> on{-1};
static int current() {
    int v = on.load();
    if (v < 0) {
        const char* e = dev_env("GL_CFG_SHARED_PREFIX");
        const int want = (e && atoi(e) == 0) ? 0 : 1;
        int expect = -1;
        on.compare_exchange_strong(expect, want);
        v = on.load();
    }
    return v;
}
static std::atomic<long long> count[3];
}
bool cfg_shared_prefix() { return cfg_prefix::current() != 0; }
void cfg_shared_prefix_note(int what) { cfg_prefix::count[what].fetch_add(1); }
int cfg_shared_prefix_set(int on) {
    if (on != 0 && on != 1) return set_error(GL_ERR_ARG, "cfg shared prefix %d (expected 0 or 1)", on);
    if (cfg_prefix::current() != on) {
        cfg_prefix::on.store(on);
        ff_policy::epoch.fetch_add(1);
    }
    return GL_OK;
}
int ff_rows_policy_report(char* buf, size_t cap) {
    if (!buf || !cap) return set_error(GL_ERR_ARG, "ff_rows_policy_report: no buffer");
    std::lock_guard<std::mutex> lk(ff_policy::mu);
    size_t n = (size_t)snprintf(buf, cap, "mode=%d", ff_policy::mode.load());
    for (const auto& kv : ff_policy::table) {
        if (n + 96 + 128 >= cap) break;
        const uint64_t k = kv.first;
        n += (size_t)snprintf(buf + n, cap - n, ";dev%d %s form%d C%d M%d -> %s (rows %.1f us, gemm %.1f us)", (int)(k >> 56),
                              ((k >> 52) & 15) == 1 ? "fuser.ff" : ((k >> 52) & 15) == 2 ? "ff" : ((k >> 52) & 15) == 3 ? "proj_in+attn1.qkv" : "attn1.to_out+fuser.qkv", (int)((k >> 48) & 15), (int)((k >> 32) & 0xffff), (int)(k & 0xffffffffu),
                              kv.second.rows ? "rows" : "gemm", kv.second.us_rows, kv.second.us_gemm);
    }
    if (n + 128 < cap)
        snprintf(buf + n, cap - n, ";cfg_shared_prefix=%d evals=%lld rows_at_prefix=%lld rows_periodic=%lld", cfg_prefix::current(),
                 cfg_prefix::count[0].load(), cfg_prefix::count[1].load(), cfg_prefix::count[2].load());
    return GL_OK;
}

template <class Run>
bool Engine::timed_form(uint64_t key, int M, int C, int n_zero, const char* name, int form, hipStream_t s, Run&& run) {
    const int mode = ff_policy::current_mode();
    if (mode == 0) return false;
    if (mode == 1) return true;
    if (mode == 2) return ff_policy::static_rule(M);
    std::unique_lock<std::mutex> lk(ff_policy::mu);
    auto it = ff_policy::table.find(key);
    if (it != ff_policy::table.end()) return it->second.rows != 0;
    hipStreamCaptureStatus cap = hipStreamCaptureStatusNone;
    (void)hipStreamIsCapturing(s, &cap);
    if (cap != hipStreamCaptureStatusNone) {
        const bool rows = ff_policy::static_rule(M);
        ff_policy::table[key] = ff_policy::Entry{rows ? 1 : 0, 0.f, 0.f};
        return rows;
    }

    HIPCK(hipDeviceSynchronize());
    struct Restore {
        Engine* e; size_t mk; int64_t launches; bool prof;
        ~Restore() { e->arena_.release(mk); e->n_launches = launches; e->profiling_ = prof; }
    } restore{this, arena_.mark(), n_launches, profiling_};
    profiling_ = false;
    bf16* z[4];
    for (bf16*& p : z) p = arena_.get<bf16>((size_t)M * C);
    for (int i = 0; i < n_zero; ++i) HIPCK(hipMemsetAsync(z[i], 0, (size_t)M * C * sizeof(bf16), s));
    auto once = [&](bool rows) {
        const size_t m2 = arena_.mark();
        run(rows, z);
        arena_.release(m2);
    };
    hipEvent_t ev[2];
    HIPCK(hipEventCreate(&ev[0]));
    HIPCK(hipEventCreate(&ev[1]));
    struct EvGuard { hipEvent_t* e; ~EvGuard() { (void)hipEventDestroy(e[0]); (void)hipEventDestroy(e[1]); } } guard{ev};
    float best[2] = {1e30f, 1e30f};
    constexpr int REPS = 4, ROUNDS = 3;
    for (int form_i = 0; form_i < 2; ++form_i) once(form_i == 1);
    for (int r = 0; r < ROUNDS; ++r)
        for (int form_i = 0; form_i < 2; ++form_i) {
            HIPCK(hipEventRecord(ev[0], s));
            for (int i = 0; i < REPS; ++i) once(form_i == 1);
            HIPCK(hipEventRecord(ev[1], s));
            HIPCK(hipEventSynchronize(ev[1]));
            float ms = 0.f;
            HIPCK(hipEventElapsedTime(&ms, ev[0], ev[1]));
            best[form_i] = std::min(best[form_i], ms * 1e3f / REPS);
        }
    const ff_policy::Entry e{best[1] < best[0] ? 1 : 0, best[1], best[0]};
    ff_policy::table[key] = e;
    static const bool log = dev_env("GL_FF_POLICY_LOG") != nullptr;
    if (log) {
        const std::string f = form < 0 ? "" : fmt(" form %d", form);
        fprintf(stderr, "[ff policy] %s%s C %d M %d: rows %.1f us, gemm %.1f us -> %s\n", name, f.c_str(), C, M, e.us_rows, e.us_gemm, e.rows ? "rows" : "gemm");
    }
    return e.rows != 0;
}

bool Engine::ff_rows_for(const STW& t, int which, int B, int HW, hipStream_t s) {
    if (which == 1 && unet_.cfg.fuser_kind != 0) which = 2;
    const FFW& f = which == 1 ? t.fff : t.ff;
    const int M = B * HW, C = t.C;
    if (!f.folded || !f.rows_stream || !ff_rows_supported(M, C)) return false;
    const int form = f.chain_stream ? (f.chain_post ? 2 : 1) : 0;
    return timed_form(ff_policy::key(device_, which, form, C, M), M, C, 3, which == 1 ? "fuser.ff" : "ff", form, s, [&](bool rows, bf16* const* z) {
        RowStats st;
        if (which == 1) {
            bool qd = false;
            bf16* t3z = fuser_ff_tail(t, z[0], z[1], B, HW, rows, s, &st, &qd);
            if (!qd && unet_.cfg.fuser_kind == 0 && t.fff.chain_q_stream) cross_q_gemm(t, t3z, st, B, HW, s);
        } else block_ff_tail(t, z[0], z[1], z[2], z[3], B, HW, rows, s);
    });
}

bool Engine::qkv_rows_for(const STW& t, int which, int B, int HW, int Nk, hipStream_t s) {
    const SelfAttnW& a = which ? t.fa : t.a1;
    const int M = B * HW, C = t.C, d = t.d;
    if (!qkv_rows_ok(a, B, HW, Nk, C, d)) return false;
    if (qkv_rows_ >= 2) return true;
    const LinW& pre = which ? t.a1.out : t.proj_in;
    const int Tf = which ? round_up(Nk, 64) : 0, slot = which ? t.idx + 1 : 0;
    return timed_form(ff_policy::key(device_, 3 + which, 0, C, M), M, C, 2, which ? "attn1.to_out+fuser.qkv" : "proj_in+attn1.qkv", -1, s, [&](bool rows, bf16* const* z) {
        if (rows) {
            qkv_rows_project(a, z[0], B, HW, Nk, C, d, pre, which ? z[1] : nullptr, z[2], nullptr, Tf, slot, s);
        } else {
            RowStats st;
            bf16* mid = linear_rows(z[0], M, pre, ACT_NONE, which ? z[1] : nullptr, nullptr, s, &st);
            const bool f = can_fold(st, M, C, 3 * C, EPI_QKV_HEADS, ACT_NONE, true);
            const bf16* ln = f ? mid : layernorm_plain(mid, B, HW, C, !which, s);
            qkv_project_gemm(a, ln, B, HW, Nk, C, d, s, f ? &st : nullptr, Tf, slot);
        }
        self_attention(a, nullptr, B, HW, HW, Nk, C, d, z[3], s, nullptr, Tf, slot, true);
    });
}

}
```

gligen_amd/csrc/engine_unet.hip:

```cpp
#include "engine_impl.h"
#include <algorithm>
#include <cmath>

namespace gl {

void Engine::configure_unet(const gl_unet_config& c) {
    if (c.n_mult < 1 || c.n_mult > 8 || c.n_attn < 0 || c.n_attn > 8) throw GlError(GL_ERR_ARG, "bad unet config");
    if (c.model_channels % 64 != 0) throw GlError(GL_ERR_UNSUPPORTED, "model_channels must be a multiple of 64");
    if (c.fuser_kind < 0 || c.fuser_kind > 2) throw GlError(GL_ERR_ARG, "fuser_kind: 0 gatedSA, 1 gatedSA2, 2 gatedCA");
    if (c.extra_channels < 0 || c.extra_channels > 64) throw GlError(GL_ERR_ARG, "extra_channels out of range");
    if (c.extra_channels && c.inpaint_mode) throw GlError(GL_ERR_UNSUPPORTED, "inpaint_mode with a grounding downsampler is undefined in the reference");
    unet_.cfg = c;
    unet_.present = true;
}

void Engine::build_unet() {
    const gl_unet_config& c = unet_.cfg;
    const int mc = c.model_channels;
    const std::string U = "unet/";
    auto in_attn = [&](int ds) {
        for (int i = 0; i < c.n_attn; ++i)
            if (c.attention_resolutions[i] == ds) return true;
        return false;
    };
// ... 131 lines not shown
    for (int level = 0; level < c.n_mult; ++level) {
        const int mult = c.channel_mult[level];
        for (int r = 0; r < c.num_res_blocks; ++r) {
            UNetBlock b;
            const std::string p = U + fmt("input_blocks.%d", n);
            b.layers.push_back(add_res(p + ".0", ch, mult * mc));
            ch = mult * mc;
            if (in_attn(ds)) {
                b.layers.push_back(add_st(p + ".1", ch));
                st_prefix.push_back(p + ".1");
            }
            unet_.in_blocks.push_back(b);
            chans.push_back(ch);
            ++n;
        }
        if (level != c.n_mult - 1) {
            unet_.updown.push_back(conv3(U + fmt("input_blocks.%d.0.op", n)));
            unet_.in_blocks.push_back(UNetBlock{{Layer{L_DOWN, (int)unet_.updown.size() - 1}}});
            chans.push_back(ch);
            ds *= 2;
            ++n;
        }
    }
    unet_.mid_block.layers.clear();
    unet_.mid_block.layers.push_back(add_res(U + "middle_block.0", ch, ch));
    unet_.mid_block.layers.push_back(add_st(U + "middle_block.1", ch));
    st_prefix.push_back(U + "middle_block.1");
    unet_.mid_block.layers.push_back(add_res(U + "middle_block.2", ch, ch));

    unet_.out_blocks.clear();
    n = 0;
    for (int level = c.n_mult - 1; level >= 0; --level) {
        const int mult = c.channel_mult[level];
        for (int i = 0; i <= c.num_res_blocks; ++i) {
            const int ich = chans.back();
            chans.pop_back();
            UNetBlock b;
            const std::string p = U + fmt("output_blocks.%d", n);
            b.layers.push_back(add_res(p + ".0", ch + ich, mc * mult));
            ch = mc * mult;
            int j = 1;
            if (in_attn(ds)) {
                b.layers.push_back(add_st(p + ".1", ch));
                st_prefix.push_back(p + ".1");
                j = 2;
            }
            if (level && i == c.num_res_blocks) {
                unet_.updown.push_back(conv3(p + fmt(".%d.conv", j), 0, true));
                b.layers.push_back(Layer{L_UP, (int)unet_.updown.size() - 1});
                ds /= 2;
            }
            unet_.out_blocks.push_back(b);
            ++n;
        }
    }
    unet_.out_norm = norm(U + "out.0");
    unet_.out_conv = conv3(U + "out.2", 32);
    if (unet_.out_conv.Cout != c.out_channels) throw GlError(GL_ERR_ARG, "out conv channels do not match out_channels");

    unet_.embcat.w = cast_rows(emb_keys);
    unet_.embcat.K = 4 * mc;
    unet_.embcat.N = emb_total;
    {
        float* b = reinterpret_cast<float*>(persist(emb_total * sizeof(float), false));
        int off = 0;
        for (size_t i = 0; i < emb_bias.size(); ++i) {
            HIPCK(hipMemcpy(b + off, emb_bias[i], emb_n[i] * sizeof(float), hipMemcpyDeviceToDevice));
            off += emb_n[i];
        }
        unet_.embcat.b = b;
    }

    {
        std::vector<const float*> ptrs;
        for (auto& p : st_prefix) {
            ptrs.push_back(F(p + ".transformer_blocks.0.fuser.alpha_attn"));
            ptrs.push_back(F(p + ".transformer_blocks.0.fuser.alpha_dense"));
        }
        void* d = persist(ptrs.size() * sizeof(float*), false);
        HIPCK(hipMemcpy(d, ptrs.data(), ptrs.size() * sizeof(float*), hipMemcpyHostToDevice));
        unet_.alpha_ptrs = reinterpret_cast<const float* const*>(d);
        gates_ = reinterpret_cast<float*>(persist(ptrs.size() * sizeof(float), true));
        fuser_scale_ = reinterpret_cast<float*>(persist(unet_.st.size() * sizeof(float), true));
        CK(fill_f32_launch(fuser_scale_, 1.f, (int)unet_.st.size(), 0));
    }

    unet_.gkind = c.grounding_kind;
    const std::string PN = U + "position_net.";
    if (unet_.gkind == 0) {
        for (int i = 0; i < 3; ++i) unet_.pn[0][i] = linear(PN + fmt("linears.%d", 2 * i));
        unet_.pn_null_feat[0] = F(PN + "null_positive_feature");
        unet_.pn_null_pos = F(PN + "null_position_feature");
    } else if (unet_.gkind == 1) {
        for (int i = 0; i < 3; ++i) {
            unet_.pn[0][i] = linear(PN + fmt("linears_text.%d", 2 * i));
            unet_.pn[1][i] = linear(PN + fmt("linears_image.%d", 2 * i));
        }
        unet_.pn_null_feat[0] = F(PN + "null_text_feature");
        unet_.pn_null_feat[1] = F(PN + "null_image_feature");
        unet_.pn_null_pos = F(PN + "null_position_feature");
    } else if (unet_.gkind == 2) {
        for (int i = 0; i < 3; ++i) unet_.pn[0][i] = linear(PN + fmt("linears.%d", 2 * i));
        unet_.pn_null_feat[0] = F(PN + "null_person_feature");
        unet_.pn_null_pos = F(PN + "null_xy_feature");
        const RawTensor& pe = raw(PN + "person_embeddings");
        const RawTensor& ke = raw(PN + "keypoint_embeddings");
        const int P = (int)pe.shape[0], D = (int)pe.shape[1];
        std::vector<float> hp(pe.numel), hk(ke.numel), tab((size_t)P * 17 * D);
        HIPCK(hipMemcpy(hp.data(), pe.p, pe.numel * sizeof(float), hipMemcpyDeviceToHost));
        HIPCK(hipMemcpy(hk.data(), ke.p, ke.numel * sizeof(float), hipMemcpyDeviceToHost));
        for (int p = 0; p < P; ++p)
            for (int j = 0; j < 17; ++j)
                for (int k = 0; k < D; ++k) tab[((size_t)p * 17 + j) * D + k] = hp[(size_t)p * D + k] + hk[(size_t)j * D + k];
        float* d = reinterpret_cast<float*>(persist(tab.size() * sizeof(float), false));
        HIPCK(hipMemcpy(d, tab.data(), tab.size() * sizeof(float), hipMemcpyHostToDevice));
        unet_.kp_table = d;
    } else if (unet_.gkind == 3) {
        if (has(PN + "convnext_tiny_backbone.downsample_layers.0.0.weight")) build_convnext(PN);
    } else {
        throw GlError(GL_ERR_UNSUPPORTED, "grounding_kind must be 0 (text), 1 (text+image), 2 (keypoint) or 3 (precomputed tokens)");
    }
}

void Engine::fuser_kv_fill(const STW& t, int B, int HW, hipStream_t s) {
    const int Ng = cond_.Ng, C = t.C, d = t.d, H = C / d;
    const int Ng64 = round_up(Ng, 64), Tf = HW + Ng64;
    int dp, dpv;
    CK(attn_dims(d, &dp, &dpv));
    const int vt_layout = attn_vt_layout(d, HW + Ng, &dpv);
    AttnBufs& bufs = attn_bufs(B, H, d, Tf, Tf, dpv, t.idx + 1);
    const size_t mk = arena_.mark();
    bf16* lno = arena_.get<bf16>((size_t)B * Ng64 * C);
    {
        LNParams P{};
        P.x = cond_.objs[t.idx]; P.B = B; P.N1 = Ng; P.N2 = 0; P.Tpad = Ng64; P.C = C; P.eps = 1e-5f; P.y = lno;
        CK(layernorm_launch(P, s));
    }
    Epilogue E = e_heads(EPI_QKV_HEADS, bufs.q, bufs.k, C, H, d, dp, Ng64, bufs.Tq_pad, bufs.Tk_pad);
    E.vt = bufs.vt; E.DPV = dpv; E.tok_off = HW; E.vt_perm32 = vt_layout;
    E.bias = t.fa.b;
    CK(gemm_launch(a_rows(lno, C), t.fa.wqk, B * Ng64, 3 * C, C, E, ws_, ws_bytes_, s));
    arena_.release(mk);
    if (fuser_kv_.size() < unet_.st.size()) fuser_kv_.resize(unet_.st.size());
    fuser_kv_[t.idx] = FuserKV{cond_epoch_, B, HW};
}

bool Engine::qkv_rows_ok(const SelfAttnW& a, int B, int T, int Nk, int C, int d) const {
    if (!qkv_rows_ || !a.rows_stream || !a.fused || !a.folded || !qkv_rows_supported(B * T, C, d, T)) return false;
    int dpv = 0;
    return attn_vt_layout(d, Nk, &dpv) == 1;
}

void Engine::qkv_rows_project(const SelfAttnW& a, const bf16* x, int B, int T, int Nk, int C, int d, const LinW& pre, const bf16* pre_res, bf16* mid,
                              RowStats* mid_stats, int Tbuf, int slot, hipStream_t s, int Bin) {
    const int H = C / d, M = B * T;
    if (Bin < 0 || (Bin && B % Bin != 0)) throw GlError(GL_ERR_STATE, fmt("qkv_rows_project: %d input samples for a batch of %d", Bin, B));
    int dp, dpv;
    CK(attn_dims(d, &dp, &dpv));
    const int vt_layout = attn_vt_layout(d, Nk, &dpv);
    AttnBufs& bufs = attn_bufs(B, H, d, Tbuf ? Tbuf : T, Tbuf ? Tbuf : T, dpv, slot);
    QkvRowsParams P{};
    P.x = x; P.ldx = C; P.eps = 1e-5f; P.stream = a.rows_stream; P.M = M;
    P.in_period = (Bin && Bin != B) ? Bin * T : 0;
    P.pre = 1; P.pre_b = pre.b; P.pre_res = pre_res; P.ld_pre_res = C; P.mid_out = mid; P.ld_mid = C;
    if (mid_stats) {
        *mid_stats = RowStats{};
        if (ln_fold_) {
            mid_stats->ld = 1; mid_stats->nb = 1;
            mid_stats->p = arena_.get<float2>((size_t)M);
            P.stats_out = mid_stats->p;
        }
    }
    P.np = 3; P.bias = a.b; P.q = bufs.q; P.k = bufs.k; P.vt = bufs.vt;
    P.H = H; P.d = d; P.DP = dp; P.DPV = dpv; P.T = T; P.Tpad_q = bufs.Tq_pad; P.Tpad_k = bufs.Tk_pad; P.vt_perm32 = vt_layout;
    ProfScope ps(this, s, "qkv_rows_kernel<pre, 3>", 8.0 * M * (double)C * C, 0.0);
    CK(qkv_rows_launch(P, C, s));
    FILE* launch_log = launch_log_file();
    if (launch_log) {
        fprintf(launch_log, "qkv_rows_kernel<320, 40, true, 3>|%d|%d|%d|0|%.0f\n", M, 4 * C, C,
                (double)qkv_rows_stream_bytes(C, true, 3) + (pre_res ? 6.0 : 4.0) * M * C + 2.0 * M * H * (2.0 * dp + dpv));
        fflush(launch_log);
    }
    ++n_launches;
}

void Engine::self_attention(const SelfAttnW& a, const bf16* ln, int B, int T, int Nq, int Nk, int C, int d, bf16* o, hipStream_t s,
                            const RowStats* in_stats, int Tbuf, int slot, bool projected) {
    const int H = C / d;
    int dp, dpv;
    CK(attn_dims(d, &dp, &dpv));
    const int vt_layout = attn_vt_layout(d, Nk, &dpv);
    AttnBufs& bufs = attn_bufs(B, H, d, Tbuf ? Tbuf : T, Tbuf ? Tbuf : T, dpv, slot);
    if (in_stats && !(a.fused && a.folded)) throw GlError(GL_ERR_STATE, "self_attention: row statistics given to an unfolded projection");
    if (!projected) qkv_project_gemm(a, ln, B, T, Nk, C, d, s, in_stats, Tbuf, slot);
    attention(bufs.q, bufs.k, bufs.vt, o, B, H, d, Nq, Nk, bufs.Tq_pad, bufs.Tk_pad, vt_layout, s);
}

void Engine::qkv_project_gemm(const SelfAttnW& a, const bf16* ln, int B, int T, int Nk, int C, int d, hipStream_t s, const RowStats* in_stats, int Tbuf, int slot) {
    const int H = C / d;
    int dp, dpv;
    CK(attn_dims(d, &dp, &dpv));
    const int vt_layout = attn_vt_layout(d, Nk, &dpv);
    AttnBufs& bufs = attn_bufs(B, H, d, Tbuf ? Tbuf : T, Tbuf ? Tbuf : T, dpv, slot);
    if (a.fused) {
        Epilogue E = e_heads(EPI_QKV_HEADS, bufs.q, bufs.k, C, H, d, dp, T, bufs.Tq_pad, bufs.Tk_pad);
        E.vt = bufs.vt; E.DPV = dpv; E.vt_perm32 = vt_layout;
        if (a.folded) E.bias = a.b;
        if (in_stats) e_fold_ln(E, *in_stats, a.csum, C);
        gemm(a_rows(ln, C), a.wqk, B * T, 3 * C, C, E, s);
    } else {
        gemm(a_rows(ln, C), a.wqk, B * T, 2 * C, C, e_heads(EPI_QK_HEADS, bufs.q, bufs.k, C, H, d, dp, T, bufs.Tq_pad, bufs.Tk_pad), s);
        Epilogue E;
        epilogue_defaults(E);
        E.mode = EPI_VT_HEADS;
        E.out = bufs.vt; E.H = H; E.d = d; E.DPV = dpv; E.T = T; E.Tpad_k = bufs.Tk_pad; E.vt_perm32 = vt_layout;
        ProfScope ps(this, s, "gemm", 2.0 * C * (double)B * T * C, 0.0);
        CK(gemm_launch_t(a.wv, C, ln, B * T, C, E, s));
        if (profiling_) ps.rename(gemm_last_kernel_name());
        ++n_launches;
    }
}

bf16* Engine::feedforward_chain(const FFW& f, const bf16* x, int M, const LinW& pre, const bf16* pre_res, const float* pre_gate, const float* gate,
                                const LinW* post, const bf16* post_res, bf16* out, hipStream_t s, RowStats* out_stats, const ChainQ* cq) {
    const int C = f.C;
    if (!f.chain_stream || !ff_rows_supported(M, C) || (post != nullptr) != f.chain_post || (cq && (post || !f.chain_q_stream)))
        throw GlError(GL_ERR_STATE, "feedforward_chain: no chained stream of this shape");
    if (!out) out = arena_.get<bf16>((size_t)M * C);
    FFRowsParams P{};
    P.x = x; P.ldx = C; P.normalize = 1; P.eps = 1e-5f; P.stream = f.chain_stream; P.b2 = f.w2.b; P.gate = gate; P.out = out; P.ldo = C; P.M = M;
    P.pre = 1; P.pre_b = pre.b; P.pre_res = pre_res; P.ld_pre_res = C; P.pre_gate = pre_gate;
    P.mid_out = arena_.get<bf16>((size_t)M * C);
    P.ld_mid = C;
    if (post) { P.post = 1; P.post_b = post->b; P.post_res = post_res; P.ld_post_res = C; }
    if (cq) { P.post = 2; P.stream = f.chain_q_stream; P.post_b = f.chain_q_bias; P.q = cq->q; P.qDP = cq->DP; P.qT = cq->T; P.qTpad = cq->Tpad; }
    if (out_stats) {
        *out_stats = RowStats{};
        if (ln_fold_) {
            out_stats->ld = 1; out_stats->nb = 1;
            out_stats->p = arena_.get<float2>((size_t)M);
            P.stats_out = out_stats->p; P.stats_ld = 1;
        }
    }
    ProfScope ps(this, s, post ? "ff_rows_kernel<pre, post>" : cq ? "ff_rows_kernel<pre, to_q>" : "ff_rows_kernel<pre>", (24.0 + ((post || cq) ? 4.0 : 2.0)) * M * (double)C * C, 0.0);
    CK(ff_rows_launch(P, C, s));
    FILE* launch_log = launch_log_file();
    if (launch_log) {
        fprintf(launch_log, "ff_rows_kernel<320, 0, true, %d>|%d|%d|%d|0|%.0f\n", post ? 1 : cq ? 2 : 0, M, C, 4 * C,
                (double)ff_chain_stream_bytes(C, true, post != nullptr || cq != nullptr) + (post ? 8.0 : 6.0) * M * C + (cq ? 2.0 * M * (C / 40) * cq->DP : 0.0));
        fflush(launch_log);
    }
    ++n_launches;
    return out;
}

bool Engine::can_fold(const RowStats& st, int M, int C, int Nc, int mode, int act, bool aligned) {
    if (!st.nb || !aligned) return false;
    Epilogue E;
    epilogue_defaults(E);
    E.mode = mode; E.act = act; E.geglu16 = gemm_geglu_layout();
    return gemm_ln_fold_supported(a_rows(nullptr, C), M, Nc, C, E);
}

bf16* Engine::ff_behind(const FFW& f, const NormW& nw, const bf16* rows_in, RowStats& st_in, int B, int HW, const float* gate, bool rows, hipStream_t s,
                        RowStats* out_stats) {
    const int M = B * HW, C = f.C;
    const bool fold = rows || (f.folded && can_fold(st_in, M, C, 8 * C, EPI_ROWMAJOR, ACT_GEGLU, round_up(HW, 64) == HW));
    const bf16* ln = fold ? rows_in : (f.folded ? layernorm_plain(rows_in, B, HW, C, false, s) : layernorm(rows_in, B, HW, C, nw, false, s));
    return feedforward(f, ln, M, rows_in, gate, s, (fold && !rows) ? &st_in : nullptr, out_stats, rows, rows);
}

bf16* Engine::fuser_ff_tail(const STW& t, const bf16* o, const bf16* t1, int B, int HW, bool rows, hipStream_t s, RowStats* st3, bool* q_done) {
    const int M = B * HW;
    const float* g_attn = gates_ + 2 * t.idx;
    if (q_done) *q_done = false;
    if (rows && t.fff.chain_stream && !t.fff.chain_post) {
        if (q_done && t.fff.chain_q_stream && t.a2.folded && HW % 128 == 0) {
            int dp, dpv;
            CK(attn_dims(t.d, &dp, &dpv));
            AttnBufs& bufs = attn_bufs(B, t.C / t.d, t.d, HW, cond_.ctx_Tpad);
            const ChainQ cq{bufs.q, dp, HW, bufs.Tq_pad};
            *q_done = true;
            return feedforward_chain(t.fff, o, M, t.fa.out, t1, g_attn, g_attn + 1, nullptr, nullptr, nullptr, s, st3, &cq);
        }
        return feedforward_chain(t.fff, o, M, t.fa.out, t1, g_attn, g_attn + 1, nullptr, nullptr, nullptr, s, st3);
    }
    RowStats st2;
    bf16* t2 = linear_rows(o, M, t.fa.out, ACT_NONE, t1, g_attn, s, rows ? nullptr : &st2);
    return ff_behind(t.fff, t.fn2, t2, st2, B, HW, g_attn + 1, rows, s, st3);
}

void Engine::block_ff_tail(const STW& t, const bf16* o, const bf16* t3, const bf16* x, bf16* out, int B, int HW, bool rows, hipStream_t s) {
    const int M = B * HW, C = t.C;
    if (rows && t.ff.chain_stream && t.ff.chain_post) {
        feedforward_chain(t.ff, o, M, t.a2.out, t3, nullptr, nullptr, &t.proj_out, x, out, s, nullptr);
        return;
    }
    RowStats st4;
    bf16* t4 = linear_rows(o, M, t.a2.out, ACT_NONE, t3, nullptr, s, rows ? nullptr : &st4);
    bf16* t5 = ff_behind(t.ff, t.ln3, t4, st4, B, HW, nullptr, rows, s, nullptr);
    gemm(a_rows(t5, C), t.proj_out.w, M, C, C, e_rows_res(out, C, t.proj_out.b, x), s);
}

bf16* Engine::feedforward(const FFW& f, const bf16* ln, int M, const bf16* res, const float* gate, hipStream_t s, const RowStats* in_stats,
                          RowStats* out_stats, bool raw_rows, bool use_rows) {
    const int C = f.C;
    if (use_rows) {
        if (!f.rows_stream || !ff_rows_supported(M, C)) throw GlError(GL_ERR_STATE, "feedforward: no row-local stream of this shape");
        bf16* out = arena_.get<bf16>((size_t)M * C);
        FFRowsParams P{};
        P.x = ln; P.ldx = C; P.normalize = (raw_rows || in_stats) ? 1 : 0; P.eps = 1e-5f;
        if (P.normalize && !f.folded) throw GlError(GL_ERR_STATE, "feedforward: raw rows given to an unfolded projection");
        P.stream = f.rows_stream; P.b2 = f.w2.b; P.res = res; P.ldres = C; P.gate = gate; P.out = out; P.ldo = C; P.M = M;
        if (out_stats) {
            *out_stats = RowStats{};
            if (ln_fold_) {
                out_stats->ld = 1; out_stats->nb = 1;
                out_stats->p = arena_.get<float2>((size_t)M);
                P.stats_out = out_stats->p; P.stats_ld = 1;
            }
        }
        ProfScope ps(this, s, "ff_rows_kernel", 24.0 * M * (double)C * C, 0.0);
        CK(ff_rows_launch(P, C, s));
        FILE* launch_log = launch_log_file();
        if (launch_log) {
            fprintf(launch_log, "ff_rows_kernel<320, 0, false, false>|%d|%d|%d|0|%.0f\n", M, C, 4 * C, (double)ff_stream_bytes(C) + (res ? 6.0 : 4.0) * M * C);
            fflush(launch_log);
        }
        ++n_launches;
        return out;
    }
    if (raw_rows && !in_stats) throw GlError(GL_ERR_STATE, "feedforward: raw rows without statistics outside the row-local kernel");
    bf16* hbuf = arena_.get<bf16>((size_t)M * 4 * C);
    Epilogue E = e_rows(hbuf, 4 * C, f.b1);
    E.act = ACT_GEGLU; E.geglu16 = f.geglu16;
    if (in_stats) {
        if (!f.folded) throw GlError(GL_ERR_STATE, "feedforward: row statistics given to an unfolded projection");
        e_fold_ln(E, *in_stats, f.csum1, C);
    }
    gemm(a_rows(ln, C), f.w1, M, 8 * C, C, E, s);
    return linear_rows(hbuf, M, f.w2, ACT_NONE, res, gate, s, out_stats);
}

AttnBufs& Engine::to_q_heads(const LinW& q, const bf16* ln, int B, int Tp, int C, int d, int Tk_pad, const RowStats* st, const float* csum, hipStream_t s) {
    const int heads = C / d;
    int dp, dpv;
    CK(attn_dims(d, &dp, &dpv));
    AttnBufs& bufs = attn_bufs(B, heads, d, Tp, Tk_pad);
    Epilogue E = e_heads(EPI_QK_HEADS, bufs.q, nullptr, C, heads, d, dp, Tp, bufs.Tq_pad, 0);
    E.bias = q.b;
    if (st) e_fold_ln(E, *st, csum, C);
    gemm(a_rows(ln, C), q.w, B * Tp, C, C, E, s);
    return bufs;
}

void Engine::cross_q_gemm(const STW& t, const bf16* rows, const RowStats& st, int B, int HW, hipStream_t s) {
    const int C = t.C, M = B * HW;
    const int Tp = round_up(HW, 64);
    const bool f3 = t.a2.folded && can_fold(st, M, C, C, EPI_QK_HEADS, ACT_NONE, Tp == HW);
    const bf16* ln = f3 ? rows : (t.a2.folded ? layernorm_plain(rows, B, HW, C, true, s) : layernorm(rows, B, HW, C, t.ln2, true, s));
    to_q_heads(t.a2.q, ln, B, Tp, C, t.d, cond_.ctx_Tpad, f3 ? &st : nullptr, t.a2.q_csum, s);
}

void Engine::ensure_fuser_kv(const STW& t, int B, int HW, hipStream_t s) {
    if (fuser_kv_.size() < unet_.st.size()) fuser_kv_.resize(unet_.st.size());
    const FuserKV& kv = fuser_kv_[t.idx];
    if (kv.epoch == cond_epoch_ && kv.B == B && kv.HW == HW) return;
    hipStreamCaptureStatus cap = hipStreamCaptureStatusNone;
    (void)hipStreamIsCapturing(s, &cap);
    if (cap != hipStreamCaptureStatusNone) throw GlError(GL_ERR_STATE, "fuser keys of this prompt / shape were not projected before the graph capture");
    fuser_kv_fill(t, B, HW, s);
    n_launches += 2;
}

bf16* Engine::concat_layernorm(const STW& t, const bf16* x, int B, int HW, int Tf, hipStream_t s) {
    const int Ng = cond_.Ng, C = t.C;
    bf16* lnc = arena_.get<bf16>((size_t)B * Tf * C);
    LNParams P{};
    P.x = x; P.x2 = cond_.objs[t.idx]; P.B = B; P.N1 = HW; P.N2 = Ng; P.Tpad = Tf; P.C = C; P.eps = 1e-5f;
    P.gamma = t.fa.folded ? nullptr : t.fn1.g; P.beta = t.fa.folded ? nullptr : t.fn1.b; P.y = lnc;
    ProfScope ps(this, s, "ln_kernel", 0.0, 2.0 * B * (HW + Ng) * (double)C * 2);
    CK(layernorm_launch(P, s));
    ++n_launches;
    return lnc;
}

bf16* Engine::transformer(const STW& t, const bf16* x, int B, int Bp, int H, int W, hipStream_t s) {
    const int HW = H * W, M = B * HW, C = t.C, d = t.d, heads = C / d;
    bf16* out = arena_.get<bf16>((size_t)M * C);
    const size_t mk = arena_.mark();
    if (cond_.Beff != B) throw GlError(GL_ERR_STATE, fmt("unet_forward batch %d != batch %d of the conditioning set by gl_unet_set_cond", B, cond_.Beff));
    if (Bp <= 0 || B % Bp != 0) throw GlError(GL_ERR_STATE, fmt("transformer: prefix batch %d does not divide batch %d", Bp, B));
    const bool shared = Bp < B;
    const int Mp = Bp * HW;

    bf16* n = groupnorm(TRef{x, C, nullptr, 0}, Bp, HW, t.gn, 1e-6f, false, s);
    const int Tp = round_up(HW, 64);
    const bool aligned = Tp == HW;
    auto normed = [&](const bf16* rows, const NormW& nw, bool folded, bool fuse, bool pad64) -> const bf16* {
        if (fuse) return rows;
        return folded ? layernorm_plain(rows, Bp, HW, C, pad64, s) : layernorm(rows, Bp, HW, C, nw, pad64, s);
    };
    RowStats st0, st1, st2, st3;
    const bool r2 = !fuser_off_ && ff_rows_for(t, 1, B, HW, s), r4 = ff_rows_for(t, 2, B, HW, s);
    bf16* t0;
    const bf16* ln = nullptr;
    bf16* o = arena_.get<bf16>((size_t)M * C);
    bool rq1;
    {
    PlanAsBatch plan_as(B / Bp);
    rq1 = aligned && qkv_rows_for(t, 0, Bp, HW, HW, s);
    if (rq1) {
        t0 = arena_.get<bf16>((size_t)Mp * C);
        qkv_rows_project(t.a1, n, Bp, HW, HW, C, d, t.proj_in, nullptr, t0, nullptr, 0, 0, s);
        self_attention(t.a1, nullptr, Bp, Tp, HW, HW, C, d, o, s, nullptr, 0, 0, true);
        if (shared) cfg_shared_prefix_note(1);
    } else {
        t0 = linear_rows(n, Mp, t.proj_in, ACT_NONE, nullptr, nullptr, s, &st0);
        const bool f1 = t.a1.folded && can_fold(st0, Mp, C, 3 * C, EPI_QKV_HEADS, ACT_NONE, aligned);
        ln = normed(t0, t.ln1, t.a1.folded, f1, true);
        self_attention(t.a1, ln, Bp, Tp, HW, HW, C, d, o, s, f1 ? &st0 : nullptr);
    }
    }
    const int Ng = cond_.Ng;
    const bool rq2 = !fuser_off_ && unet_.cfg.fuser_kind == 0 && fuser_hoist_ && aligned && cond_.Ng > 0 && qkv_rows_for(t, 1, B, HW, HW + Ng, s);
    if (shared && !rq2) {
        replicate(o, o + (size_t)Mp * C, (size_t)Mp * C, B / Bp - 1, s);
        bf16* t0b = arena_.get<bf16>((size_t)M * C);
        replicate(t0, t0b, (size_t)Mp * C, B / Bp, s);
        t0 = t0b;
    }
    bf16* t1 = rq2 ? arena_.get<bf16>((size_t)M * C) : linear_rows(o, M, t.a1.out, ACT_NONE, t0, nullptr, s, &st1);

    bf16* t3;
    bool q_done = false;
    if (fuser_off_) {
        t3 = t1;
        st3 = st1;
    } else if (unet_.cfg.fuser_kind == 0) {
        const int Tf = round_up(HW + Ng, 64);
        if (rq2) {
            ensure_fuser_kv(t, B, HW, s);
            qkv_rows_project(t.fa, o, B, HW, HW + Ng, C, d, t.a1.out, t0, t1, nullptr, Tf, t.idx + 1, s, shared ? Bp : 0);
            if (shared) cfg_shared_prefix_note(2);
            self_attention(t.fa, nullptr, B, HW, HW, HW + Ng, C, d, o, s, nullptr, Tf, t.idx + 1, true);
        } else if (fuser_hoist_ && t.fa.fused && t.fa.folded && aligned) {
            ensure_fuser_kv(t, B, HW, s);
            const bool ff = can_fold(st1, M, C, 3 * C, EPI_QKV_HEADS, ACT_NONE, aligned);
            const bf16* rows = ff ? t1 : layernorm_plain(t1, B, HW, C, false, s);
            self_attention(t.fa, rows, B, HW, HW, HW + Ng, C, d, o, s, ff ? &st1 : nullptr, Tf, t.idx + 1);
        } else {
            self_attention(t.fa, concat_layernorm(t, t1, B, HW, Tf, s), B, Tf, HW, HW + Ng, C, d, o, s);
        }
        t3 = fuser_ff_tail(t, o, t1, B, HW, r2, s, &st3, &q_done);
    } else {
        bf16* t2;
        if (unet_.cfg.fuser_kind == 1) {
            int sg = 0;
            while (sg * sg < Ng) ++sg;
            if (sg * sg != Ng || H != W) throw GlError(GL_ERR_ARG, fmt("gatedSA2 needs square token grids (visual %dx%d, %d grounding tokens)", H, W, Ng));
            const int Ta = HW + Ng;
            const int Tf = round_up(Ta, 64);
            bf16* lnc = concat_layernorm(t, t1, B, HW, Tf, s);
            bf16* oa = arena_.get<bf16>((size_t)B * Ta * C);
            self_attention(t.fa, lnc, B, Tf, Ta, Ta, C, d, oa, s);
            bf16* pr = linear_rows(oa, B * Ta, t.fa.out, ACT_NONE, nullptr, nullptr, s);
            t2 = arena_.get<bf16>((size_t)M * C);
            CK(fuser_resize_launch(pr, t1, gates_ + 2 * t.idx, t2, B, Ta, HW, sg, H, C, s));
            ++n_launches;
        } else {
            ln = layernorm(t1, B, HW, C, t.fn1, true, s);
            const AttnBufs& bufs = to_q_heads(t.fca.q, ln, B, Tp, C, d, cond_.obj_Tpad, nullptr, nullptr, s);
            attention(bufs.q, cond_.obj_k[t.idx], cond_.obj_vt[t.idx], o, B, heads, d, HW, Ng, bufs.Tq_pad, cond_.obj_Tpad, 0, s);
            t2 = linear_rows(o, M, t.fca.out, ACT_NONE, t1, gates_ + 2 * t.idx, s, r2 ? nullptr : &st2);
        }
        t3 = ff_behind(t.fff, t.fn2, t2, st2, B, HW, gates_ + 2 * t.idx + 1, r2, s, &st3);
    }

    if (!q_done) cross_q_gemm(t, t3, st3, B, HW, s);
    {
        const AttnBufs& bufs = attn_bufs(B, heads, d, Tp, cond_.ctx_Tpad);
        attention(bufs.q, cond_.ctx_k[t.idx], cond_.ctx_vt[t.idx], o, B, heads, d, HW, cond_.ctx_T, bufs.Tq_pad, cond_.ctx_Tpad, 0, s);
    }
    block_ff_tail(t, o, t3, x, out, B, HW, r4, s);
    arena_.release(mk);
    return out;
}

void Engine::set_fuser_scale(float v, hipStream_t s) {
    if (!unet_.present || !finalized_) throw GlError(GL_ERR_STATE, "unet not finalized");
    CK(fill_f32_launch(fuser_scale_, v, (int)unet_.st.size(), s));
    fuser_off_ = v == 0.f;
}

void Engine::restore_first_conv(const float* w, const float* b, hipStream_t s) {
    if (!unet_.present || !finalized_) throw GlError(GL_ERR_STATE, "unet not finalized");
    if (unet_.cfg.inpaint_mode) throw GlError(GL_ERR_STATE, "first conv of an inpainting model is not restorable");
    const int mc = unet_.cfg.model_channels;
    CK(pack_conv_small_launch(w, const_cast<bf16*>(unet_.conv_in_small.w), mc, unet_.conv_in_small.Cin, unet_.conv_in_small.Kpad, s, unet_.cfg.in_channels));
    HIPCK(hipMemcpyAsync(const_cast<float*>(unet_.conv_in_small.b), b, mc * sizeof(float), hipMemcpyDeviceToDevice, s));
}

void Engine::set_cond(int Beff, const float* context, int n_ctx, const gl_grounding& g, hipStream_t s) {
    if (!unet_.present || !finalized_) throw GlError(GL_ERR_STATE, "unet not finalized");
    if (Beff <= 0 || n_ctx <= 0 || g.n <= 0) throw GlError(GL_ERR_ARG, "set_cond: empty batch / context / grounding");
    if (unet_.cfg.fuser_kind == 1) {
        int sg = 0;
        while (sg * sg < (unet_.gkind == 1 ? 2 * g.n : g.n)) ++sg;
        if (sg * sg != (unet_.gkind == 1 ? 2 * g.n : g.n)) throw GlError(GL_ERR_ARG, "gatedSA2 needs a square number of grounding tokens");
    }
    const gl_unet_config& c = unet_.cfg;
    const int Ng = unet_.gkind == 1 ? 2 * g.n : g.n;
    const int ctx_Tpad = round_up(n_ctx, 64);
    const int heads = c.num_heads;
    const bool ca = c.fuser_kind == 2;
    const int obj_Tpad = round_up(Ng, 64);
    const int obj_stride = ca ? obj_Tpad : Ng;
    if (cond_.Beff != Beff || cond_.Ng != Ng || cond_.ctx_Tpad != ctx_Tpad) {
        sampler_wait_idle();
        HIPCK(hipStreamSynchronize(s));
        sampler_release_graph();
        for (void* p : cond_.allocs) (void)hipFree(p);
        cond_ = Cond{};
        auto palloc = [&](size_t bytes) {
            void* p = nullptr;
            HIPCK(hipMalloc(&p, bytes));
            HIPCK(hipMemset(p, 0, bytes));
            cond_.allocs.push_back(p);
            return p;
        };
        for (const STW& t : unet_.st) {
            int dp, dpv;
            CK(attn_dims(t.d, &dp, &dpv));
            if (ca) {
                cond_.objs.push_back(nullptr);
                cond_.obj_k.push_back(reinterpret_cast<bf16*>(palloc((size_t)Beff * heads * obj_Tpad * dp * sizeof(bf16))));
                cond_.obj_vt.push_back(reinterpret_cast<bf16*>(palloc((size_t)Beff * heads * dpv * obj_Tpad * sizeof(bf16))));
                CK(attn_vt_ones_launch(cond_.obj_vt.back(), Beff * heads, t.d, obj_Tpad, 0));
                CK(attn_k_init_launch(cond_.obj_k.back(), Beff * heads, t.d, obj_Tpad, 0));
            } else {
                cond_.objs.push_back(reinterpret_cast<bf16*>(palloc((size_t)Beff * Ng * t.C * sizeof(bf16))));
            }
            cond_.ctx_k.push_back(reinterpret_cast<bf16*>(palloc((size_t)Beff * heads * ctx_Tpad * dp * sizeof(bf16))));
            cond_.ctx_vt.push_back(reinterpret_cast<bf16*>(palloc((size_t)Beff * heads * dpv * ctx_Tpad * sizeof(bf16))));
            CK(attn_vt_ones_launch(cond_.ctx_vt.back(), Beff * heads, t.d, ctx_Tpad, 0));
            CK(attn_k_init_launch(cond_.ctx_k.back(), Beff * heads, t.d, ctx_Tpad, 0));
        }
        cond_.tokens = reinterpret_cast<bf16*>(palloc((size_t)Beff * obj_stride * c.gr_out_dim * sizeof(bf16)));
        HIPCK(hipStreamSynchronize(0));
        cond_.Beff = Beff;
        cond_.Ng = Ng;
        cond_.ctx_Tpad = ctx_Tpad;
        cond_.obj_Tpad = obj_Tpad;
    }
    if (cond_.ctx_T != n_ctx && (smp_.exec[0] || smp_.exec[1])) {
        sampler_wait_idle();
        sampler_release_graph();
    }
    cond_.ctx_T = n_ctx;
    arena_.reset();

    const int out_dim = c.gr_out_dim;
    bf16* objs = arena_.get<bf16>((size_t)Beff * obj_stride * out_dim);
    if (ca) HIPCK(hipMemsetAsync(objs, 0, (size_t)Beff * obj_stride * out_dim * sizeof(bf16), s));
    const int rows = Beff * g.n;
    auto mlp = [&](int which, const PosNetIn& pin_in, int remap_off) {
        PosNetIn pin = pin_in;
        const int Kp = unet_.pn[which][0].K;
        pin.out = arena_.get<bf16>((size_t)rows * Kp);
        pin.ld_out = Kp;
        pin.rows = rows;
        CK(posnet_input_launch(pin, s));
        bf16* h1 = linear_rows(pin.out, rows, unet_.pn[which][0], ACT_SILU, nullptr, nullptr, s);
        bf16* h2 = linear_rows(h1, rows, unet_.pn[which][1], ACT_SILU, nullptr, nullptr, s);
        Epilogue E = e_rows(objs, out_dim, unet_.pn[which][2].b);
        E.remap_in = g.n; E.remap_out = obj_stride; E.remap_off = remap_off;
        gemm(a_rows(h2, unet_.pn[which][2].K), unet_.pn[which][2].w, rows, out_dim, unet_.pn[which][2].K, E, s);
    };
    PosNetIn pin{};
    pin.null_pos = unet_.pn_null_pos;
    pin.mask = g.masks;
    if (unet_.gkind == 0) {
        if (!g.boxes || !g.masks || !g.text_embeddings) throw GlError(GL_ERR_ARG, "text grounding needs boxes, masks, text_embeddings");
        pin.feat = g.text_embeddings; pin.pos = g.boxes; pin.F = c.gr_in_dim; pin.P = 4; pin.null_feat = unet_.pn_null_feat[0];
        mlp(0, pin, 0);
    } else if (unet_.gkind == 1) {
        if (!g.boxes || !g.masks || !g.text_masks || !g.image_masks || !g.text_embeddings || !g.image_embeddings)
            throw GlError(GL_ERR_ARG, "text+image grounding needs boxes, masks, text/image masks and embeddings");
        pin.pos = g.boxes; pin.F = c.gr_in_dim; pin.P = 4;
        pin.feat = g.text_embeddings; pin.fmask = g.text_masks; pin.null_feat = unet_.pn_null_feat[0];
        mlp(0, pin, 0);
        pin.feat = g.image_embeddings; pin.fmask = g.image_masks; pin.null_feat = unet_.pn_null_feat[1];
        mlp(1, pin, g.n);
    } else if (unet_.gkind == 3) {
// ... 195 lines not shown
```

gligen_amd/csrc/ffn.h:

```cpp
#pragma once
#include "common.h"

namespace gl {

struct FFRowsParams {
    const bf16* x;
    int ldx;
    int normalize;
    float eps;
    const void* stream;
    const float* b2;
    const bf16* res;
    int ldres;
    const float* gate;
    bf16* out;
    int ldo;
    float2* stats_out;
    int stats_ld;
    int M;
    int pre, post;
    const float* pre_b;
    const bf16* pre_res;
    int ld_pre_res;
    const float* pre_gate;
    bf16* mid_out;
    int ld_mid;
    const float* post_b;
    const bf16* post_res;
    int ld_post_res;
    bf16* q;
    int qDP, qT, qTpad;
};

bool ff_rows_supported(int M, int C);
size_t ff_stream_bytes(int C);
int ff_pack_launch(const float* w1, const float* b1, const float* w2, void* stream, int C, hipStream_t s);
int ff_rows_launch(const FFRowsParams& p, int C, hipStream_t s);
size_t ff_chain_stream_bytes(int C, bool pre, bool post);
int ff_chain_pack_launch(const float* w1, const float* b1, const float* w2, const float* pre_w, const float* post_w, void* stream, int C, hipStream_t s);

struct QkvRowsParams {
    const bf16* x;
    int ldx;
    int normalize;
    float eps;
    const void* stream;
    int M;
    int pre;
    const float* pre_b;
    const bf16* pre_res;
    int ld_pre_res;
    bf16* mid_out;
    int ld_mid;
    float2* stats_out;
    int np;
    const float* bias;
    bf16* q;
    bf16* k;
    bf16* vt;
    int H, d, DP, DPV, T, Tpad_q, Tpad_k, vt_perm32;
    int in_period;
};
bool qkv_rows_supported(int M, int C, int d, int T);
size_t qkv_rows_stream_bytes(int C, bool pre, int np);
int qkv_rows_pack_launch(const float* pre_w, const bf16* w, int np, void* stream, int C, hipStream_t s);
int qkv_rows_launch(const QkvRowsParams& p, int C, hipStream_t s);

}
```

gligen_amd/csrc/ffn.hip:

```cpp
#include "ffn.h"

#include <type_traits>
#include <utility>

namespace gl {

namespace {

typedef unsigned u32x4 __attribute__((ext_vector_type(4)));

template <int C>
struct FFGeom {
    static_assert(C % 32 == 0, "C must be a multiple of 32");
    static constexpr int KS = C / 16;
    static constexpr int NKP = KS + 1;
    static constexpr int NCB = C / 32;
    static constexpr int NCH = 4 * C / 32;
    static constexpr int NPB = 2 * NKP;
    static constexpr int NOB = 2 * NCB;
    static constexpr int NBLK = NPB + NOB;
    static constexpr int NBS = (NBLK + 3) / 4 * 4;
    static constexpr int STAGE = NBS * 1024;
    static_assert((NBLK - 1) * 1024 < 65536, "fragment reads address a stage through the 16-bit offset field");
    static constexpr int NSTAGE = NCH + 1;
// ... 641 lines not shown

    u32x4 rs;
    {
        const unsigned long long a = (unsigned long long)(uintptr_t)p.stream;
        rs.x = (unsigned)a;
        rs.y = (unsigned)(a >> 32);
        rs.z = (unsigned)((size_t)NSEG * G::PJ_BYTES);
        rs.w = 0x00020000u;
    }
    const unsigned lds0 = (unsigned)(uintptr_t)(__attribute__((address_space(3))) unsigned char*)smem;
    const unsigned lds_w = lds0 + (unsigned)wave * 1024u;
    unsigned dma_lds = lds_w;
    unsigned dma_off = (unsigned)wave * 1024u;
#pragma unroll
    for (int i = 0; i < 2 * (PJ_BLK / 4); ++i) ffr_dma<true>(rs, lane16, dma_lds, dma_off);

    bf16x8 xf[KS];
    {
        const bf16* src = p.x + (size_t)row_in * p.ldx + h * 8;
#pragma unroll
        for (int ks = 0; ks < KS; ++ks) xf[ks] = *reinterpret_cast<const bf16x8*>(src + ks * 16);
    }
    uint2 rv[PRE ? NCB : 1][4];
    const bool has_res = PRE && p.pre_res != nullptr;
    if constexpr (PRE) {
        if (has_res) {
            const bf16* src = p.pre_res + (size_t)row_in * p.ld_pre_res + h * 4;
#pragma unroll
            for (int cb = 0; cb < NCB; ++cb)
#pragma unroll
                for (int j = 0; j < 4; ++j) rv[cb][j] = *reinterpret_cast<const uint2*>(src + cb * 32 + j * 8);
        } else {
#pragma unroll
            for (int cb = 0; cb < NCB; ++cb)
#pragma unroll
                for (int j = 0; j < 4; ++j) rv[cb][j] = make_uint2(0u, 0u);
        }
    }
    float* lbias = reinterpret_cast<float*>(smem + 3 * PSTAGE);
    for (int i = t; i < NBIAS; i += 256) {
        float v;
        if (PRE && i < C) v = p.pre_b[i];
        else v = p.bias[i - (PRE ? C : 0)];
        lbias[i] = v;
    }
    if (!PRE && p.normalize) {
        float s = 0.f, ss = 0.f;
#pragma unroll
        for (int ks = 0; ks < KS; ++ks)
#pragma unroll
            for (int e = 0; e < 8; ++e) {
                const float v = bf2f(xf[ks][e]);
                s += v;
                ss = fmaf(v, v, ss);
            }
        s += __shfl_xor(s, 32, 64);
        ss += __shfl_xor(ss, 32, 64);
        const float mean = s * (1.f / C);
        const float var = fmaxf(ss * (1.f / C) - mean * mean, 0.f);
        const float rstd = rsqrtf(var + p.eps);
        const float nm = -mean * rstd;
#pragma unroll
        for (int ks = 0; ks < KS; ++ks)
#pragma unroll
            for (int e = 0; e < 8; ++e) xf[ks][e] = f2bf(fmaf(bf2f(xf[ks][e]), rstd, nm));
    }

    f32x16 acc[NCB];
    const unsigned ra_st[3] = {lds0 + lane16, lds0 + (unsigned)PSTAGE + lane16, lds0 + 2u * (unsigned)PSTAGE + lane16};
    constexpr int NSTG = NSEG * PJ_ST;

    auto phase = [&](bf16x8 (&xin)[KS], auto seg_c, auto swap_c, auto skip_c) {
        constexpr int SEG = decltype(seg_c)::value;
        constexpr bool SWAP = decltype(swap_c)::value, SKIP = decltype(skip_c)::value;
        static_for<PJ_ST>([&](auto sc) {
            constexpr int st = decltype(sc)::value, g = SEG * PJ_ST + st, BUF = g % 3;
            constexpr int pieces = g + 2 < NSTG ? PJ_BLK / 4 : 0;
            if constexpr (!(SKIP && st < 2)) asm volatile("s_waitcnt vmcnt(0)");
            __builtin_amdgcn_s_barrier();
            const unsigned ra = ra_st[BUF];
            dma_lds = lds_w + (unsigned)((g + 2) % 3) * (unsigned)PSTAGE;
            bf16x8 fr[NR];
            static_for<RD>([&](auto ic) {
                constexpr int i = decltype(ic)::value;
                ffr_rd16<i * 1024>(fr[i % NR], ra);
            });
            static_for<PJ_BLK>([&](auto ic) {
                constexpr int i = decltype(ic)::value;
                if constexpr (i % 4 == 0) {
                    constexpr int last = (i + RD - 1 < PJ_BLK - 1) ? i + RD - 1 : PJ_BLK - 1;
                    constexpr int need = (i + 3 < PJ_BLK - 1) ? i + 3 : PJ_BLK - 1;
                    ffr_wait_lgkm<last - need>();
                }
                constexpr int ks = st * PJ_KS + i / NCB, cb = i % NCB;
                if constexpr (ks == 0) {
                    if constexpr (SWAP) asm volatile("v_mfma_f32_32x32x16_bf16 %0, %1, %2, 0" : "=&a"(acc[cb]) : "a"(xin[0]), "v"(fr[i % NR]));
                    else asm volatile("v_mfma_f32_32x32x16_bf16 %0, %1, %2, 0" : "=&a"(acc[cb]) : "v"(fr[i % NR]), "a"(xin[0]));
                } else {
                    if constexpr (SWAP) asm volatile("v_mfma_f32_32x32x16_bf16 %0, %1, %2, %0" : "+a"(acc[cb]) : "a"(xin[ks]), "v"(fr[i % NR]));
                    else asm volatile("v_mfma_f32_32x32x16_bf16 %0, %1, %2, %0" : "+a"(acc[cb]) : "v"(fr[i % NR]), "a"(xin[ks]));
                }
                if constexpr (i + RD < PJ_BLK) ffr_rd16<(i + RD) * 1024>(fr[(i + RD) % NR], ra);
                if constexpr (i % 2 == 1 && i / 2 < pieces) ffr_dma(rs, lane16, dma_lds, dma_off);
            });
        });
        ffr_settle(acc);
        if constexpr (SEG + 1 < NSEG) asm volatile("s_waitcnt vmcnt(0)");
    };
    auto pin_x = [&]() {
#pragma unroll
        for (int ks = 0; ks < KS; ++ks) asm volatile("" : "+a"(xf[ks]));
        asm volatile("s_nop 7\n\ts_nop 7");
    };

    using S0 = std::integral_constant<int, 0>;
    using S1 = std::integral_constant<int, 1>;
    using S2 = std::integral_constant<int, 2>;
    using S3 = std::integral_constant<int, 3>;
    using T_ = std::true_type;
    using F_ = std::false_type;

    __builtin_amdgcn_s_waitcnt(0x0070);
    if constexpr (PRE) {
#pragma unroll
        for (int cb = 0; cb < NCB; ++cb)
#pragma unroll
            for (int j = 0; j < 4; ++j) asm volatile("" : "+v"(rv[cb][j].x), "+v"(rv[cb][j].y));
    }
    pin_x();
    if constexpr (PRE) {
        phase(xf, S0{}, F_{}, F_{});
        float tv[NCB][16];
        float s = 0.f, ss = 0.f;
        bf16* mrow = p.mid_out + (size_t)row * p.ld_mid + h * 4;
#pragma unroll
        for (int cb = 0; cb < NCB; ++cb) {
            float4 bv[4];
#pragma unroll
            for (int j = 0; j < 4; ++j) bv[j] = *reinterpret_cast<const float4*>(lbias + cb * 32 + j * 8 + h * 4);
#pragma unroll
            for (int j = 0; j < 4; ++j) {
                U2BF4 r, o;
                r.u = rv[cb][j];
                const float bj[4] = {bv[j].x, bv[j].y, bv[j].z, bv[j].w};
#pragma unroll
                for (int e = 0; e < 4; ++e) {
                    o.e[e] = f2bf(acc[cb][4 * j + e] + bj[e] + bf2f(r.e[e]));
                    const float t_ = bf2f(o.e[e]);
                    tv[cb][4 * j + e] = t_;
                    s += t_;
                    ss = fmaf(t_, t_, ss);
                }
                if constexpr (GL_QKV_ABL & 2) asm volatile("" ::"v"(o.u.x), "v"(o.u.y));
                else *reinterpret_cast<uint2*>(mrow + cb * 32 + j * 8) = o.u;
            }
        }
        s += __shfl_xor(s, 32, 64);
        ss += __shfl_xor(ss, 32, 64);
        if (p.stats_out && h == 0) p.stats_out[row] = make_float2(s, ss);
        const float mean = s * (1.f / C);
        const float var = fmaxf(ss * (1.f / C) - mean * mean, 0.f);
        const float rstd = rsqrtf(var + p.eps);
        const float nm = -mean * rstd;
#pragma unroll
        for (int ks = 0; ks < KS; ++ks)
#pragma unroll
            for (int e = 0; e < 8; ++e) xf[ks][e] = f2bf(fmaf(tv[ks >> 1][4 * (2 * (ks & 1) + (e >> 2)) + (e & 3)], rstd, nm));
        pin_x();
    }

    const int b = row0 / p.T;
    const int tw = row0 - b * p.T;
    const int tok = tw + l31;
    const float* hbias = lbias + (PRE ? C : 0);
    auto heads_qk = [&](auto which_c) {
        constexpr int WHICH = decltype(which_c)::value;
        const int tp = WHICH ? p.Tpad_k : p.Tpad_q;
        const size_t head_stride = (size_t)tp * p.DP;
        bf16* base = (WHICH ? p.k : p.q) + (size_t)b * p.H * head_stride +
                     (WHICH ? (size_t)(tok & ~63) * p.DP + (size_t)(tok & 63) * 8 + 4 * h : (size_t)tok * p.DP + 4 * h);
        const float* bias = hbias + WHICH * C + 4 * h;
#pragma unroll
        for (int cb = 0; cb < NCB; ++cb) {
            float4 bv[4];
#pragma unroll
            for (int j = 0; j < 4; ++j) bv[j] = *reinterpret_cast<const float4*>(bias + cb * 32 + j * 8);
#pragma unroll
            for (int j = 0; j < 4; ++j) {
                const int f0 = cb * 32 + j * 8, hd = f0 / D, dd = f0 % D;
                const float v[4] = {acc[cb][4 * j] + bv[j].x, acc[cb][4 * j + 1] + bv[j].y, acc[cb][4 * j + 2] + bv[j].z, acc[cb][4 * j + 3] + bv[j].w};
                U2BF4 o;
#pragma unroll
                for (int e = 0; e < 4; ++e) o.e[e] = f2bf(v[e]);
                bf16* dst = base + (size_t)hd * head_stride + (WHICH ? (size_t)(dd >> 3) * 512 : (size_t)dd);
                if constexpr (GL_QKV_ABL & 1) asm volatile("" ::"v"(o.u.x), "v"(o.u.y), "v"(dst));
                else *reinterpret_cast<uint2*>(dst) = o.u;
            }
        }
    };
    auto heads_vt = [&]() {
#pragma unroll
        for (int cb = 0; cb < NCB; ++cb) {
            const int f = cb * 32 + l31, hd = f / D, dd = f - hd * D;
            const float bn = hbias[2 * C + f];
            bf16* dst = p.vt + ((size_t)(b * p.H + hd) * p.DPV + dd) * p.Tpad_k + tw + 16 * h;
            U4BF8 o0, o1;
#pragma unroll
            for (int e = 0; e < 8; ++e) {
                o0.e[e] = f2bf(acc[cb][e] + bn);
                o1.e[e] = f2bf(acc[cb][8 + e] + bn);
            }
            if constexpr (GL_QKV_ABL & 1) asm volatile("" ::"v"(o0.u.x), "v"(o0.u.w), "v"(o1.u.x), "v"(o1.u.w), "v"(dst));
            else {
                *reinterpret_cast<uint4*>(dst) = o0.u;
                *reinterpret_cast<uint4*>(dst + 8) = o1.u;
            }
        }
    };
    if constexpr (NP == 1) {
        if constexpr (PRE) phase(xf, S1{}, F_{}, T_{}); else phase(xf, S0{}, F_{}, F_{});
        heads_qk(S0{});
    } else if constexpr ((GL_QKV_ABL & 4) != 0) {
        heads_qk(S0{});
        heads_qk(S1{});
        heads_vt();
    } else {
        if constexpr (PRE) phase(xf, S1{}, F_{}, T_{}); else phase(xf, S0{}, F_{}, F_{});
        heads_qk(S0{});
        if constexpr (PRE) phase(xf, S2{}, F_{}, T_{}); else phase(xf, S1{}, F_{}, T_{});
        heads_qk(S1{});
        if constexpr (PRE) phase(xf, S3{}, T_{}, T_{}); else phase(xf, S2{}, T_{}, T_{});
        heads_vt();
    }
}

template <int C>
__global__ void __launch_bounds__(256) qkv_rows_pack_kernel(const float* __restrict__ pre_w, const bf16* __restrict__ w, int np,
                                                            unsigned char* __restrict__ stream) {
    using G = FFGeom<C>;
    const size_t pre_bytes = pre_w ? G::PJ_BYTES : 0;
    const size_t n_pieces = (pre_bytes + (size_t)np * G::PJ_BYTES) / 16;
    for (size_t pc = (size_t)blockIdx.x * blockDim.x + threadIdx.x; pc < n_pieces; pc += (size_t)gridDim.x * blockDim.x) {
        const size_t byte = pc * 16;
        const int L = (int)(byte >> 4) & 63, r = L & 31, h = L >> 5;
        const bool pre = byte < pre_bytes;
        const size_t sb = pre ? byte : byte - pre_bytes;
        const int seg = (int)(sb / G::PJ_BYTES);
        const int blk = (int)((sb % G::PJ_BYTES) >> 10);
        const int st = blk / G::PJ_BLK, i = blk % G::PJ_BLK, ks = st * G::PJ_KS + i / G::NCB, cb = i % G::NCB;
        U4BF8 o;
        if (pre) {
            const float* src = pre_w + (size_t)(cb * 32 + r) * C;
#pragma unroll
            for (int e = 0; e < 8; ++e) o.e[e] = f2bf(src[ff_kidx(ks, h, e, false)]);
        } else {
            const bf16* src = w + (size_t)(seg * C + cb * 32 + r) * C;
#pragma unroll
            for (int e = 0; e < 8; ++e) o.e[e] = src[ff_kidx(ks, h, e, pre_w != nullptr)];
        }
        *reinterpret_cast<uint4*>(stream + byte) = o.u;
    }
}

}

bool ff_rows_supported(int M, int C) { return C == 320 && M > 0 && M % 128 == 0; }

size_t ff_stream_bytes(int C) {
    if (C == 320) return FFGeom<320>::STREAM_BYTES;
    return 0;
}

size_t ff_chain_stream_bytes(int C, bool pre, bool post) {
    if (C == 320) return FFGeom<320>::chain_bytes(pre, post);
    return 0;
}

int ff_chain_pack_launch(const float* w1, const float* b1, const float* w2, const float* pre_w, const float* post_w, void* stream, int C, hipStream_t s) {
    if (C != 320) return set_error(GL_ERR_UNSUPPORTED, "ff_pack: no row-local feed-forward kernel for C = %d", C);
    if (post_w && !pre_w) return set_error(GL_ERR_UNSUPPORTED, "ff_pack: a trailing projection is built only together with a leading one");
    hipLaunchKernelGGL(ff_pack_kernel<320>, dim3(1024), dim3(256), 0, s, w1, b1, w2, pre_w, post_w, reinterpret_cast<unsigned char*>(stream));
    GL_LAUNCH_CHECK();
    return GL_OK;
}

int ff_pack_launch(const float* w1, const float* b1, const float* w2, void* stream, int C, hipStream_t s) {
    return ff_chain_pack_launch(w1, b1, w2, nullptr, nullptr, stream, C, s);
}

#ifdef GL_FFN_ABLATE
static int g_ff_abl = 0;
void ff_rows_set_ablation(int abl) { g_ff_abl = abl; }
template <int ABL>
static int ff_abl_launch(const FFRowsParams& p, hipStream_t s) {
    using G = FFGeom<320>;
    auto kfn = ff_rows_kernel<320, ABL>;
    GL_HIP(hipFuncSetAttribute((const void*)kfn, hipFuncAttributeMaxDynamicSharedMemorySize, G::LDS_BYTES));
    hipLaunchKernelGGL(kfn, dim3(p.M / 128), dim3(256), G::LDS_BYTES, s, p);
    GL_LAUNCH_CHECK();
    return GL_OK;
}
#endif

int ff_rows_launch(const FFRowsParams& p, int C, hipStream_t s) {
#ifdef GL_FFN_ABLATE
    switch (g_ff_abl) {
        case 1: return ff_abl_launch<1>(p, s);
        case 2: return ff_abl_launch<2>(p, s);
        case 4: return ff_abl_launch<4>(p, s);
        case 8: return ff_abl_launch<8>(p, s);
        case 16: return ff_abl_launch<16>(p, s);
        case 24: return ff_abl_launch<24>(p, s);
        case 32: return ff_abl_launch<32>(p, s);
        case 3: return ff_abl_launch<3>(p, s);
        case 7: return ff_abl_launch<7>(p, s);
        case 6: return ff_abl_launch<6>(p, s);
        case 25: return ff_abl_launch<25>(p, s);
        case 31: return ff_abl_launch<31>(p, s);
        default: break;
    }
#endif
    if (!ff_rows_supported(p.M, C)) return set_error(GL_ERR_UNSUPPORTED, "ff_rows: M = %d, C = %d has no row-local kernel", p.M, C);
    if (p.ldx % 8 || p.ldo % 4 || (p.res && p.ldres % 4)) return set_error(GL_ERR_ARG, "ff_rows: row strides must keep 16-byte loads / 8-byte stores aligned");
    using G = FFGeom<320>;
    if (p.post && !p.pre) return set_error(GL_ERR_UNSUPPORTED, "ff_rows: a trailing projection is built only together with a leading one");
    if (p.post == 2 && (!p.post_b || !p.q || p.qT <= 0 || p.M % p.qT || p.qT % 32 || p.qDP < 40 || p.qDP % 4))
        return set_error(GL_ERR_ARG, "ff_rows: the trailing to_q projection needs its folded bias, the q buffer and its geometry");
    if (p.pre && (!p.normalize || !p.pre_b || !p.pre_res || !p.mid_out || p.ld_pre_res % 4 || p.ld_mid % 4))
        return set_error(GL_ERR_ARG, "ff_rows: the leading projection needs normalize = 1, its bias, residual and the buffer for its result");
    if (p.post == 1 && (!p.post_b || !p.post_res || p.ld_post_res % 4)) return set_error(GL_ERR_ARG, "ff_rows: the trailing projection needs its bias and residual");
    const dim3 grid(p.M / 128), block(256);
    if (p.pre && p.post == 2) return launch_lds<ff_rows_kernel<320, 0, true, 2>>(grid, block, G::LDS_BYTES, s, p);
    if (p.pre && p.post) return launch_lds<ff_rows_kernel<320, 0, true, 1>>(grid, block, G::LDS_BYTES, s, p);
    if (p.pre) return launch_lds<ff_rows_kernel<320, 0, true, 0>>(grid, block, G::LDS_BYTES, s, p);
    return launch_lds<ff_rows_kernel<320, 0, false, 0>>(grid, block, G::LDS_BYTES, s, p);
}


bool qkv_rows_supported(int M, int C, int d, int T) { return C == 320 && d == 40 && M > 0 && M % 128 == 0 && T > 0 && T % 128 == 0 && M % T == 0; }

size_t qkv_rows_stream_bytes(int C, bool pre, int np) {
    if (C != 320 || (np != 1 && np != 3)) return 0;
    return ((pre ? 1 : 0) + (size_t)np) * FFGeom<320>::PJ_BYTES;
}

int qkv_rows_pack_launch(const float* pre_w, const bf16* w, int np, void* stream, int C, hipStream_t s) {
    if (C != 320 || (np != 1 && np != 3) || !w || !stream) return set_error(GL_ERR_UNSUPPORTED, "qkv_rows_pack: C = %d, np = %d has no row-local projection kernel", C, np);
    hipLaunchKernelGGL(qkv_rows_pack_kernel<320>, dim3(512), dim3(256), 0, s, pre_w, w, np, reinterpret_cast<unsigned char*>(stream));
    GL_LAUNCH_CHECK();
    return GL_OK;
}

int qkv_rows_launch(const QkvRowsParams& p, int C, hipStream_t s) {
    if (!qkv_rows_supported(p.M, C, p.d, p.T)) return set_error(GL_ERR_UNSUPPORTED, "qkv_rows: M = %d, C = %d, d = %d, T = %d has no row-local projection kernel", p.M, C, p.d, p.T);
    if (p.np != 1 && p.np != 3) return set_error(GL_ERR_ARG, "qkv_rows: np must be 1 (q) or 3 (q, k, v^T)");
    if (p.ldx % 8 || !p.x || !p.stream || !p.q || !p.bias || (p.np == 3 && (!p.k || !p.vt))) return set_error(GL_ERR_ARG, "qkv_rows: null pointer / unaligned rows");
    if (p.np == 3 && (p.vt_perm32 != 1 || p.Tpad_k % 32)) return set_error(GL_ERR_UNSUPPORTED, "qkv_rows: v^T is written in the 32-token form only (attn3_kernel)");
    if (p.H * p.d != C || p.DP < p.d || p.DP % 8 || (p.np == 3 && p.DPV < p.d)) return set_error(GL_ERR_ARG, "qkv_rows: head geometry");
    if (p.pre && (!p.pre_b || !p.mid_out || p.ld_mid % 4 || (p.pre_res && p.ld_pre_res % 4))) return set_error(GL_ERR_ARG, "qkv_rows: the leading projection needs its bias and the buffer for its result");
    if (p.in_period < 0 || (p.in_period && (p.in_period % p.T || p.M % p.in_period))) return set_error(GL_ERR_ARG, "qkv_rows: the input period must be whole samples and divide M");
    using G = FFGeom<320>;
    constexpr int LDS = 3 * G::PJ_BLK * 1024 + 4 * 320 * (int)sizeof(float);
    const dim3 grid(p.M / 128), block(256);
    if (p.pre && p.np == 3) return launch_lds<qkv_rows_kernel<320, 40, true, 3>>(grid, block, LDS, s, p);
    if (p.pre) return launch_lds<qkv_rows_kernel<320, 40, true, 1>>(grid, block, LDS, s, p);
    if (p.np == 3) return launch_lds<qkv_rows_kernel<320, 40, false, 3>>(grid, block, LDS, s, p);
    return launch_lds<qkv_rows_kernel<320, 40, false, 1>>(grid, block, LDS, s, p);
}

}
```

gligen_amd/engine.py:

```python
from __future__ import annotations

import ctypes as C
from typing import Dict, Mapping, Optional, Sequence

import numpy as np
import torch

from . import _lib
from ._lib import Grounding, PlmsArgs, UNetConfig, VaeConfig, check

GROUNDING_KINDS = {"text": 0, "text_image": 1, "keypoint": 2, "tokens": 3}


def _stream(device=None) -> C.c_void_p:
    return C.c_void_p(torch.cuda.current_stream(device).cuda_stream)


def _ptr(t: Optional[torch.Tensor]) -> C.c_void_p:
    return C.c_void_p(0 if t is None else t.data_ptr())


def _f32(t: torch.Tensor, device) -> torch.Tensor:
    return t.to(device=device, dtype=torch.float32).contiguous()

# ... 890 lines not shown
        Nk = k.shape[1]
        if HD % heads or k.shape != (B, Nk, HD) or v.shape != k.shape or (dout is not None and dout.shape != q.shape):
            raise ValueError("op_train_attention: q / dout [B, Nq, H D], k / v [B, Nk, H D]")
        shapes = {"o": q.shape, "lse": (B, heads, Nq)}
        if dout is not None:
            shapes.update(dq=q.shape, dk=k.shape, dv=k.shape)
        o = self._prim_outs(shapes, out, required=("o", "lse"))
        check(self.lib.gl_op_train_attention(self._ctx, int(B), int(heads), int(HD // heads), int(Nq), int(Nk), _ptr(q), _ptr(k), _ptr(v), _ptr(dout),
                                             *[_ptr(o.get(n)) for n in ("o", "lse", "dq", "dk", "dv")], _stream(dev)))
        return o

    def op_train_linear(self, x, W, b=None, dy=None, out=None):
        dev = self.device
        x, W = _f32(x, dev), _f32(W, dev)
        b, dy = (None if t is None else _f32(t, dev) for t in (b, dy))
        (M, K), N = x.shape, W.shape[0]
        if W.shape != (N, K) or (b is not None and b.shape != (N,)) or (dy is not None and dy.shape != (M, N)):
            raise ValueError("op_train_linear: x [M, K], W [N, K], b [N], dy [M, N]")
        shapes = {"y": (M, N)}
        if dy is not None:
            shapes.update(dx=(M, K), dW=(N, K), db=(N,))
        o = self._prim_outs(shapes, out)
        check(self.lib.gl_op_train_linear(self._ctx, int(M), int(N), int(K), _ptr(x), _ptr(W), _ptr(b), _ptr(dy),
                                          *[_ptr(o.get(n)) for n in ("y", "dx", "dW", "db")], _stream(dev)))
        return o

    def op_train_layernorm(self, x, g, b, eps=1e-5, dy=None, accumulate=False, out=None):
        dev = self.device
        x, g, b = (_f32(t, dev) for t in (x, g, b))
        dy = None if dy is None else _f32(dy, dev)
        R, Cc = x.shape
        if g.shape != (Cc,) or b.shape != (Cc,) or (dy is not None and dy.shape != x.shape):
            raise ValueError("op_train_layernorm: x / dy [R, C], g / b [C]")
        shapes = {"y": x.shape, "xhat": x.shape, "rstd": (R,)}
        if dy is not None:
            shapes.update(dx=x.shape, dgamma=(Cc,), dbeta=(Cc,))
        o = self._prim_outs(shapes, out, required=("dx",) if accumulate else ())
        if accumulate and out is None:
            raise ValueError("op_train_layernorm: accumulate adds to out['dx']")
        check(self.lib.gl_op_train_layernorm(self._ctx, int(R), int(Cc), C.c_float(eps), _ptr(x), _ptr(g), _ptr(b), _ptr(dy), 1 if accumulate else 0,
                                             *[_ptr(o.get(n)) for n in ("y", "xhat", "rstd", "dx", "dgamma", "dbeta")], _stream(dev)))
        return o

    def op_train_groupnorm(self, x, g, b, silu=True, eps=1e-5, da=None, accumulate=False, out=None):
        dev = self.device
        x, g, b = (_f32(t, dev) for t in (x, g, b))
        da = None if da is None else _f32(da, dev)
        B, HW, Cc = x.shape
        if g.shape != (Cc,) or b.shape != (Cc,) or (da is not None and da.shape != x.shape):
            raise ValueError("op_train_groupnorm: x / da [B, HW, C], g / b [C]")
        shapes = {"a": x.shape, "xhat": x.shape, "rstd": (B, 32)}
        if da is not None:
            shapes.update(dx=x.shape)
        o = self._prim_outs(shapes, out, required=("dx",) if accumulate else ())
        if accumulate and out is None:
            raise ValueError("op_train_groupnorm: accumulate adds to out['dx']")
        check(self.lib.gl_op_train_groupnorm(self._ctx, int(B), int(HW), int(Cc), 1 if silu else 0, C.c_float(eps), _ptr(x), _ptr(g), _ptr(b), _ptr(da),
                                             1 if accumulate else 0, *[_ptr(o.get(n)) for n in ("a", "xhat", "rstd", "dx")], _stream(dev)))
        return o

    def op_train_geglu(self, u, dh=None, out=None):
        dev = self.device
        u = _f32(u, dev)
        dh = None if dh is None else _f32(dh, dev)
        R, I2 = u.shape
        if I2 % 2 or (dh is not None and dh.shape != (R, I2 // 2)):
            raise ValueError("op_train_geglu: u [R, 2 I], dh [R, I]")
        shapes = {"h": (R, I2 // 2)}
        if dh is not None:
            shapes.update(du=u.shape)
        o = self._prim_outs(shapes, out)
        check(self.lib.gl_op_train_geglu(self._ctx, int(R), int(I2 // 2), _ptr(u), _ptr(dh), _ptr(o.get("h")), _ptr(o.get("du")), _stream(dev)))
        return o

    def op_train_dot(self, a, b, mode, alpha=None, scale=1.0, out=None):
        dev = self.device
        a, b = _f32(a, dev).reshape(-1), _f32(b, dev).reshape(-1)
        alpha = None if alpha is None else _f32(alpha, dev)
        if a.shape != b.shape:
            raise ValueError("op_train_dot: a and b hold the same number of elements")
        o = self._prim_outs({"out": (1,)}, out, required=("out",))
        check(self.lib.gl_op_train_dot(self._ctx, int(a.numel()), _ptr(a), _ptr(b), _ptr(alpha), C.c_float(scale), int(mode), _ptr(o["out"]), _stream(dev)))
        return o

    def op_conv3x3(self, x0, w_oihw, bias, x1=None, stride=1, ups=0, pad_lo=1, res=None):
        B, H, W, C0 = x0.shape
        C1 = 0 if x1 is None else x1.shape[3]
        Cout = w_oihw.shape[0]
        Hup, Wup = H << ups, W << ups
        if stride == 1:
            Ho, Wo = Hup, Wup
        else:
            Ho = (Hup + (2 if pad_lo else 1) - 3) // 2 + 1
            Wo = (Wup + (2 if pad_lo else 1) - 3) // 2 + 1
        y = torch.empty((B, Ho, Wo, Cout), device=x0.device, dtype=torch.bfloat16)
        check(self.lib.gl_op_conv3x3(self._ctx, _ptr(x0), C0, _ptr(x1), C1, B, H, W, _ptr(w_oihw), _ptr(bias), Cout,
                                     stride, ups, pad_lo, _ptr(res), _ptr(y), _stream(self.device)))
        return y

    def op_gn_silu_conv3x3(self, x0, gamma, beta, eps, w_oihw, bias, x1=None, bias2=None, res=None, mode=-1):
        B, H, W, C0 = x0.shape
        C1 = 0 if x1 is None else x1.shape[3]
        Cout = w_oihw.shape[0]
        y = torch.empty((B, H, W, Cout), device=x0.device, dtype=torch.bfloat16)
        used = C.c_int(0)
        check(self.lib.gl_op_gn_silu_conv3x3(self._ctx, _ptr(x0), C0, _ptr(x1), C1, B, H, W, _ptr(gamma), _ptr(beta), C.c_float(eps),
                                             _ptr(w_oihw), _ptr(bias), Cout, _ptr(bias2), _ptr(res), _ptr(y), int(mode), C.byref(used),
                                             _stream(self.device)))
        return y, bool(used.value)

    def op_groupnorm(self, x0, gamma, beta, eps, silu, x1=None):
        B, HW, C0 = x0.shape
        C1 = 0 if x1 is None else x1.shape[2]
        y = torch.empty((B, HW, C0 + C1), device=x0.device, dtype=torch.bfloat16)
        check(self.lib.gl_op_groupnorm(self._ctx, _ptr(x0), C0, _ptr(x1), C1, B, HW, _ptr(gamma), _ptr(beta),
                                       C.c_float(eps), int(silu), _ptr(y), _stream(self.device)))
        return y

    def op_layernorm(self, x, gamma, beta, eps=1e-5, x2=None, Tpad=None):
        B, N1, Cc = x.shape
        N2 = 0 if x2 is None else x2.shape[1]
        Tpad = Tpad or (N1 + N2)
        y = torch.empty((B, Tpad, Cc), device=x.device, dtype=torch.bfloat16)
        check(self.lib.gl_op_layernorm(self._ctx, _ptr(x), _ptr(x2), B, N1, N2, Tpad, Cc, _ptr(gamma), _ptr(beta),
                                       C.c_float(eps), _ptr(y), _stream(self.device)))
        return y

    def op_ff_chain_q(self, x, pre_w, pre_b, pre_res, gamma, beta, w1, b1, w2, b2, gamma_q, beta_q, wq, pre_gate=None, gate=None):
        B, N, Cc = x.shape
        y = torch.empty_like(x)
        qbuf = torch.zeros((B * 8, N, 48), device=x.device, dtype=torch.bfloat16)
        check(self.lib.gl_op_ff_chain_q(self._ctx, _ptr(x), B, N, Cc, _ptr(pre_w), _ptr(pre_b), _ptr(pre_res), _ptr(pre_gate), _ptr(gamma), _ptr(beta),
                                        _ptr(w1), _ptr(b1), _ptr(w2), _ptr(b2), _ptr(gate), _ptr(gamma_q), _ptr(beta_q), _ptr(wq), _ptr(y), _ptr(qbuf),
                                        _stream(self.device)))
        return y, qbuf.view(B, 8, N, 48)[..., :40]

    def op_proj_attention(self, x, pre_w, pre_b, pre_res, gamma, beta, wq, wk, wv, heads, rows=True):
        B, N, Cc = x.shape
        mid = torch.empty_like(x)
        o = torch.empty_like(x)
        used = C.c_int(1 if rows else 0)
        check(self.lib.gl_op_proj_attention(self._ctx, _ptr(x), B, N, Cc, heads, _ptr(pre_w), _ptr(pre_b), _ptr(pre_res), _ptr(gamma), _ptr(beta),
                                            _ptr(wq), _ptr(wk), _ptr(wv), 0, _ptr(mid), _ptr(o), C.byref(used), _stream(self.device)))
        return mid, o, used.value

    def op_attention(self, xq, xkv, wq, wk, wv, heads):
        B, Nq, Cc = xq.shape
        _, Nk, Ck = xkv.shape
        o = torch.empty((B, Nq, Cc), device=xq.device, dtype=torch.bfloat16)
        check(self.lib.gl_op_attention(self._ctx, _ptr(xq), _ptr(xkv), B, Nq, Nk, Cc, Ck, heads, _ptr(wq), _ptr(wk), _ptr(wv),
                                       _ptr(o), _stream(self.device)))
        return o

    def attn_regime_counters(self, enable):
        lazy, reruns = C.c_uint(0), C.c_uint(0)
        check(self.lib.gl_attn_regime_counters(self._ctx, 1 if enable else 0, C.byref(lazy), C.byref(reruns)))
        return lazy.value, reruns.value
```

Baseline: 6.590 images/s.

## Share fuser attention prefix across CFG pair in one paired kernel

Adds a paired attention kernel for the gated self-attention fuser under classifier-free guidance. The cond and uncond samples share the same visual-token prefix and differ only in the last key tile of grounding tokens, so the shared tiles are processed once and the online-softmax state is then forked for each sample's final tile. The qkv-rows projection writes its mid output twice instead of computing the fuser q/k/v for both halves. This removes duplicated attention and projection work over the shared prefix, at the cost of extra register state, a second set of LDS slots, and a fallback rerun path.

```diff
diff --git a/gligen_amd/_lib.py b/gligen_amd/_lib.py
--- a/gligen_amd/_lib.py
+++ b/gligen_amd/_lib.py
@@ -212,6 +212,10 @@
     "gl_set_cfg_shared_prefix": (_I, [_I]),
 }
 
+PAIR_SYMBOLS = {
+    "gl_op_attention_pair": (_I, [_P, _P, _P, _I, _I, _I, _I, _I, _I, _P, _P, _P, _P, _I, _P]),
+}
+
 FUSER_KINDS = {"gatedSA": 0, "gatedSA2": 1, "gatedCA": 2}
 
 
@@ -236,7 +240,7 @@
     import torch
     lib = C.CDLL(str(LIB_PATH))
     for name, (res, args) in {**SYMBOLS, **IMAGE_SYMBOLS, **MAP_SYMBOLS, **TRAIN_MAP_SYMBOLS, **TRAIN_INPUT_SYMBOLS, **TRAIN_FUSER_SYMBOLS, **TRAIN_PRIM_SYMBOLS,
-                              **TRAINER_SYMBOLS, **SAMPLER_SYMBOLS}.items():
+                              **TRAINER_SYMBOLS, **SAMPLER_SYMBOLS, **PAIR_SYMBOLS}.items():
         fn = getattr(lib, name)
         fn.restype = res
         fn.argtypes = args
diff --git a/gligen_amd/csrc/attention.h b/gligen_amd/csrc/attention.h
--- a/gligen_amd/csrc/attention.h
+++ b/gligen_amd/csrc/attention.h
@@ -17,6 +17,8 @@
     float scale_log2e;
     int vt_layout;
     unsigned* counters = nullptr;
+    int n_shared = 0;
+    int Bp = 0;
 };
 enum { ATTN_CTR_LAZY_MOVES = 0,
        ATTN_CTR_RERUNS = 1,
@@ -25,6 +27,8 @@
 int attn_dims(int d, int* DP, int* DPV);
 int attn_vt_layout(int d, int Nk, int* DPV);
 int attn_launch(const AttnParams& P, int B, hipStream_t stream);
+bool attn_pair_supported(int d, int Nk, int n_shared, int vt_layout);
+int attn_pair_launch(const AttnParams& P, int Bp, hipStream_t stream);
 const char* attn_kernel_name(int d, int Nk, int vt_layout = -1);
 int attn_vt_ones_launch(bf16* vt, int BH, int d, int Tk_pad, hipStream_t stream, int DPV = 0);
 
diff --git a/gligen_amd/csrc/attention.hip b/gligen_amd/csrc/attention.hip
--- a/gligen_amd/csrc/attention.hip
+++ b/gligen_amd/csrc/attention.hip
@@ -574,9 +574,10 @@
         lds_rd_v16<N, I + 1>(d, a);
     }
 }
-template <int DP, int DPV, bool BIAS, int NW, bool COUNT>
-__global__ void __launch_bounds__(NW * 64, NW == 4 ? 2 : 1) attn3_kernel(AttnParams P) {
+template <int DP, int DPV, bool BIAS, int NW, bool COUNT, bool PAIR>
+__device__ __forceinline__ void attn3_body(const AttnParams& P) {
     static_assert(DP % 16 == 0 && DPV % 16 == 0 && DPV > DP - 8, "tile geometry");
+    static_assert(!PAIR || (BIAS && DPV <= 64), "the pair form exists for d = 40");
     constexpr int KS = DP / 16;
     constexpr int DB = DPV / 16;
     constexpr int KP = DP / 8, VP = DPV / 8;
@@ -610,8 +611,15 @@
     const bf16* __restrict__ Vg = P.vt + bh * DPV * P.Tk_pad;
     const __amdgpu_buffer_rsrc_t rk = __builtin_amdgcn_make_buffer_rsrc((void*)Kg, 0, 0x80000000u, 0x00020000);
     const __amdgpu_buffer_rsrc_t rv = __builtin_amdgcn_make_buffer_rsrc((void*)Vg, 0, 0x80000000u, 0x00020000);
+    const size_t bh1 = bh + (PAIR ? (size_t)P.Bp * P.H : 0);
+    [[maybe_unused]] const __amdgpu_buffer_rsrc_t rk1 = __builtin_amdgcn_make_buffer_rsrc((void*)(P.k + bh1 * P.Tk_pad * DP), 0, 0x80000000u, 0x00020000);
+    [[maybe_unused]] const __amdgpu_buffer_rsrc_t rv1 = __builtin_amdgcn_make_buffer_rsrc((void*)(P.vt + bh1 * DPV * P.Tk_pad), 0, 0x80000000u, 0x00020000);
+    [[maybe_unused]] int rep = 0;
 
     const int nt = (P.Nk + 63) >> 6;
+    [[maybe_unused]] const int ns = PAIR ? P.n_shared : nt;
+    [[maybe_unused]] int nt_run = nt;
+    [[maybe_unused]] int tslot = 2;
     const int q0 = qblk * (NW * 32) + wave * 32;
     const int myq = q0 + lrow;
     const int myq_ld = myq < P.Tq_pad ? myq : P.Tq_pad - 1;
@@ -629,21 +637,33 @@
     auto issue_k = [&](int jj, int slot) {
         const lds_ptr st = lbase + slot * STAGE + w1k;
         const int so = jj * KBYTES + w1k;
+        __amdgpu_buffer_rsrc_t rkj = rk;
+        if constexpr (PAIR) { if (rep && jj >= ns) rkj = rk1; }
 #pragma unroll
         for (int i = 0; i < KR; ++i) {
-            if ((i + 1) * NW <= KP) GL_BLDS16(rk, st + i * NW * 1024, lane16, so + i * NW * 1024);
-            else if (wave < KP - i * NW) GL_BLDS16(rk, st + i * NW * 1024, lane16, so + i * NW * 1024);
+            if ((i + 1) * NW <= KP) GL_BLDS16(rkj, st + i * NW * 1024, lane16, so + i * NW * 1024);
+            else if (wave < KP - i * NW) GL_BLDS16(rkj, st + i * NW * 1024, lane16, so + i * NW * 1024);
         }
     };
     auto issue_v = [&](int jj, int slot) {
         const lds_ptr st = lbase + slot * STAGE + KBYTES + w1k;
         const int so = (jj - 1) * 128;
+        __amdgpu_buffer_rsrc_t rvj = rv;
+        if constexpr (PAIR) { if (rep && jj - 1 >= ns) rvj = rv1; }
 #pragma unroll
         for (int i = 0; i < VR; ++i) {
-            if ((i + 1) * NW <= VP) GL_BLDS16(rv, st + i * NW * 1024, vvoff[i], so);
-            else if (wave < VP - i * NW) GL_BLDS16(rv, st + i * NW * 1024, vvoff[i], so);
+            if ((i + 1) * NW <= VP) GL_BLDS16(rvj, st + i * NW * 1024, vvoff[i], so);
+            else if (wave < VP - i * NW) GL_BLDS16(rvj, st + i * NW * 1024, vvoff[i], so);
         }
     };
+    if constexpr (PAIR) {
+        rep = 1;
+        issue_k(ns, 3);
+        issue_v(ns + 1, 3);
+        rep = 0;
+        issue_k(ns, 2);
+        issue_v(ns + 1, 2);
+    }
     issue_k(0, 0);
 
     bf16x8 qf[KS];
@@ -681,10 +701,10 @@
         __builtin_amdgcn_s_waitcnt(0x0F70);
         __builtin_amdgcn_s_barrier();
         asm volatile("" ::: "memory");
-        const int slot = SLOT >= 0 ? SLOT : (j & 1);
+        const int slot = SLOT >= 0 ? SLOT : SLOT == -2 ? tslot : (j & 1);
         if constexpr (ISSUE != 0) {
             if constexpr (ISSUE == 1) issue_k(j + 1, slot ^ 1);
-            if constexpr (ISSUE == 3) { if (j + 1 < nt) issue_k(j + 1, slot ^ 1); }
+            if constexpr (ISSUE == 3) { if (j + 1 < (PAIR ? nt_run : nt)) issue_k(j + 1, slot ^ 1); }
             issue_v(j + 1, slot ^ 1);
         }
         if constexpr (LAZY && SM && !SAFE) {
@@ -850,17 +870,17 @@
     using I2 = std::integral_constant<int, 2>;
     using I3 = std::integral_constant<int, 3>;
     f32x16 sa[2], sb2[2];
-#define GL_ATTN3_TILES(SAFE_T) \
+#define GL_ATTN3_TILES(SAFE_T, NT_) \
     iter(0, sb2, sa, S0{}, I3{}, F_{}, T_{}, T_{}, T_{}, SAFE_T{}); \
-    if (nt == 1) { \
+    if ((NT_) == 1) { \
         iter(1, sa, sb2, S1{}, I0{}, T_{}, F_{}, F_{}, F_{}, SAFE_T{}); \
     } else { \
         int j = 1; \
-        for (; j + 1 <= nt - 2; j += 2) { \
+        for (; j + 1 <= (NT_) - 2; j += 2) { \
             iter(j, sa, sb2, S1{}, I1{}, T_{}, T_{}, F_{}, F_{}, SAFE_T{}); \
             iter(j + 1, sb2, sa, S0{}, I1{}, T_{}, T_{}, F_{}, F_{}, SAFE_T{}); \
         } \
-        if (j <= nt - 2) { \
+        if (j <= (NT_) - 2) { \
             iter(j, sa, sb2, S1{}, I1{}, T_{}, T_{}, F_{}, F_{}, SAFE_T{}); \
             ++j; \
             iter(j, sb2, sa, S0{}, I2{}, T_{}, T_{}, T_{}, F_{}, SAFE_T{}); \
@@ -870,8 +890,7 @@
             iter(j + 1, sb2, sa, S0{}, I0{}, T_{}, F_{}, F_{}, F_{}, SAFE_T{}); \
         } \
     }
-    GL_ATTN3_TILES(F_)
-    if constexpr (LAZY) {
+    auto any_bad_wg = [&]() -> unsigned {
         const float c0 = ot[0][OB][ORR], c1 = ot[1][OB][ORR];
         const bool bad = overshoot || (g4 == OG && (!(c0 > 0.f && c0 < 1.0e30f) || !(c1 > 0.f && c1 < 1.0e30f)));
         volatile unsigned* flags = reinterpret_cast<volatile unsigned*>(smem);
@@ -885,48 +904,108 @@
         for (int w = 0; w < NW; ++w) any_bad |= flags[w];
         __builtin_amdgcn_s_waitcnt(0xC07F);
         __builtin_amdgcn_s_barrier();
-        if (any_bad) {
+        return any_bad;
+    };
+    auto reset_state = [&]() {
+#pragma unroll
+        for (int qh = 0; qh < 2; ++qh)
+#pragma unroll
+            for (int i = 0; i < DB; ++i)
+#pragma unroll
+                for (int r = 0; r < 4; ++r) ot[qh][i][r] = 0.f;
+        m_run = 0.f;
+        if (half == 1) qf[2][0] = f2bf(0.f);
+    };
+    auto write_o = [&](int bo) {
+        const int ob = P.d >> 4, og = (P.d & 15) >> 2, orr = P.d & 3;
+#pragma unroll
+        for (int qh = 0; qh < 2; ++qh) {
+            float cand = 0.f;
+#pragma unroll
+            for (int i = 0; i < DB; ++i)
+#pragma unroll
+                for (int r = 0; r < 4; ++r)
+                    if (i == ob && r == orr) cand = ot[qh][i][r];
+            const float l_tot = __shfl(cand, 16 * og + l15, 64);
+            const float inv = 1.f / l_tot;
+            const int q = q0 + 16 * qh + l15;
+            if (q < P.Nq) {
+                bf16* orow = P.o + ((size_t)bo * P.o_rows_per_b + q) * P.ldo + h * P.d;
+#pragma unroll
+                for (int i = 0; i < DB; ++i) {
+                    const int dd0 = 16 * i + 4 * g4;
+                    if (dd0 < P.d) {
+                        U2BF4 o;
+#pragma unroll
+                        for (int e = 0; e < 4; ++e) o.e[e] = f2bf(ot[qh][i][e] * inv);
+                        *reinterpret_cast<uint2*>(orow + dd0) = o.u;
+                    }
+                }
+            }
+        }
+    };
+    if constexpr (!PAIR) {
+        GL_ATTN3_TILES(F_, nt)
+        if constexpr (LAZY) {
+            if (any_bad_wg()) {
+                if constexpr (COUNT) { if (t == 0) atomicAdd(P.counters + ATTN_CTR_RERUNS, 1u); }
+                reset_state();
+                issue_k(0, 0);
+                GL_ATTN3_TILES(T_, nt)
+            }
+        }
+        write_o(b);
+    } else {
+        using ST = std::integral_constant<int, -2>;
+        nt_run = ns;
+        GL_ATTN3_TILES(F_, ns)
+        f32x4_t ot_s[2][DB];
+#pragma unroll
+        for (int qh = 0; qh < 2; ++qh)
+#pragma unroll
+            for (int i = 0; i < DB; ++i) ot_s[qh][i] = ot[qh][i];
+        const float m_s = m_run;
+        const bf16 q_s = qf[2][0];
+        const bool over_s = overshoot;
+        unsigned rerun = 0;
+#pragma unroll 1
+        for (int r = 0; r < 2; ++r) {
+#pragma unroll
+            for (int qh = 0; qh < 2; ++qh)
+#pragma unroll
+                for (int i = 0; i < DB; ++i) ot[qh][i] = ot_s[qh][i];
+            m_run = m_s;
+            qf[2][0] = q_s;
+            overshoot = over_s;
+            tslot = 2 + r;
+            iter(ns, sb2, sa, ST{}, I0{}, F_{}, T_{}, T_{}, F_{}, F_{});
+            iter(ns + 1, sa, sb2, ST{}, I0{}, T_{}, F_{}, F_{}, F_{}, F_{});
+            if (any_bad_wg()) rerun |= 1u << r;
+            else write_o(b + r * P.Bp);
+        }
+#pragma unroll 1
+        for (int r = 0; r < 2; ++r) {
+            if (!((rerun >> r) & 1u)) continue;
             if constexpr (COUNT) { if (t == 0) atomicAdd(P.counters + ATTN_CTR_RERUNS, 1u); }
-#pragma unroll
-            for (int qh = 0; qh < 2; ++qh)
-#pragma unroll
-                for (int i = 0; i < DB; ++i)
-#pragma unroll
-                    for (int r = 0; r < 4; ++r) ot[qh][i][r] = 0.f;
-            m_run = 0.f;
-            if (half == 1) qf[2][0] = f2bf(0.f);
+            __builtin_amdgcn_s_barrier();
+            reset_state();
+            rep = r;
+            nt_run = nt;
             issue_k(0, 0);
-            GL_ATTN3_TILES(T_)
+            GL_ATTN3_TILES(T_, nt)
+            write_o(b + r * P.Bp);
         }
     }
 #undef GL_ATTN3_TILES
-
-    const int ob = P.d >> 4, og = (P.d & 15) >> 2, orr = P.d & 3;
-#pragma unroll
-    for (int qh = 0; qh < 2; ++qh) {
-        float cand = 0.f;
-#pragma unroll
-        for (int i = 0; i < DB; ++i)
-#pragma unroll
-            for (int r = 0; r < 4; ++r)
-                if (i == ob && r == orr) cand = ot[qh][i][r];
-        const float l_tot = __shfl(cand, 16 * og + l15, 64);
-        const float inv = 1.f / l_tot;
-        const int q = q0 + 16 * qh + l15;
-        if (q < P.Nq) {
-            bf16* orow = P.o + ((size_t)b * P.o_rows_per_b + q) * P.ldo + h * P.d;
-#pragma unroll
-            for (int i = 0; i < DB; ++i) {
-                const int dd0 = 16 * i + 4 * g4;
-                if (dd0 < P.d) {
-                    U2BF4 o;
-#pragma unroll
-                    for (int e = 0; e < 4; ++e) o.e[e] = f2bf(ot[qh][i][e] * inv);
-                    *reinterpret_cast<uint2*>(orow + dd0) = o.u;
-                }
-            }
-        }
-    }
+}
+
+template <int DP, int DPV, bool BIAS, int NW, bool COUNT>
+__global__ void __launch_bounds__(NW * 64, NW == 4 ? 2 : 1) attn3_kernel(AttnParams P) {
+    attn3_body<DP, DPV, BIAS, NW, COUNT, false>(P);
+}
+template <int DP, int DPV, bool BIAS, int NW, bool COUNT>
+__global__ void __launch_bounds__(NW * 64, NW == 4 ? 2 : 1) attn3_pair_kernel(AttnParams P) {
+    attn3_body<DP, DPV, BIAS, NW, COUNT, true>(P);
 }
 
 template <int DP, int DPV, bool BIAS, int NW>
@@ -941,6 +1020,27 @@
     return GL_OK;
 }
 
+bool attn_pair_supported(int d, int Nk, int n_shared, int vt_layout) {
+    return d == 40 && vt_layout == 1 && n_shared >= 1 && (Nk + 63) / 64 == n_shared + 1;
+}
+int attn_pair_launch(const AttnParams& P, int Bp, hipStream_t stream) {
+    if (P.Nq <= 0 || P.Nk <= 0 || Bp <= 0) return set_error(GL_ERR_ARG, "pair attention: empty Nq=%d Nk=%d Bp=%d", P.Nq, P.Nk, Bp);
+    if (P.Tq_pad % 128 != 0 || P.Tk_pad % 64 != 0 || P.Tq_pad < P.Nq || P.Tk_pad < P.Nk)
+        return set_error(GL_ERR_ARG, "pair attention: bad padding Tq_pad=%d Tk_pad=%d (Nq=%d Nk=%d)", P.Tq_pad, P.Tk_pad, P.Nq, P.Nk);
+    if (P.Bp != Bp || !attn_pair_supported(P.d, P.Nk, P.n_shared, P.vt_layout))
+        return set_error(GL_ERR_ARG, "pair attention: d=%d Nk=%d n_shared=%d vt_layout=%d Bp=%d/%d (d = 40, layout 1, exactly one key tile behind the shared ones)",
+                         P.d, P.Nk, P.n_shared, P.vt_layout, P.Bp, Bp);
+    constexpr int DP = 48, DPV = 48, NW = 4;
+    const size_t lds = 4 * ((DP / 8) * 1024 + (DPV / 8) * 1024);
+    AttnParams Q = P;
+    Q.nqb = cdiv(P.Nq, NW * 32);
+    dim3 grid(Q.nqb * P.H * Bp);
+    if (P.counters) hipLaunchKernelGGL((attn3_pair_kernel<DP, DPV, true, NW, true>), grid, dim3(NW * 64), lds, stream, Q);
+    else hipLaunchKernelGGL((attn3_pair_kernel<DP, DPV, true, NW, false>), grid, dim3(NW * 64), lds, stream, Q);
+    GL_LAUNCH_CHECK();
+    return GL_OK;
+}
+
 template <int DP, int DPV, bool BIAS, int NW>
 static int launch_attn2(const AttnParams& P, int B, hipStream_t stream) {
     const size_t lds = 2 * ((DP / 8) * 1024 + (DPV / 8) * 1024);
diff --git a/gligen_amd/csrc/capi.hip b/gligen_amd/csrc/capi.hip
--- a/gligen_amd/csrc/capi.hip
+++ b/gligen_amd/csrc/capi.hip
@@ -9,6 +9,7 @@
 #include "../../include/gligen_amd_train_prims.h"
 #include "../../include/gligen_amd_trainer.h"
 #include "../../include/gligen_amd_sampler.h"
+#include "../../include/gligen_amd_pair.h"
 
 #include <cstdlib>
 
@@ -1133,11 +1134,13 @@
     GL_API_END
 }
 
-int gl_op_attention(gl_ctx* ctx, const void* xq, const void* xkv, int B, int Nq, int Nk, int C, int Ck, int H,
-                    const float* wq, const float* wk, const float* wv, void* o, gl_stream s) {
-    NEED(ctx);
-    GL_API_BEGIN
-    Engine& eng = *ctx->eng;
+static int op_attention(gl_ctx* ctx, const void* xq, const void* xkv, int B, int Nq, int Nk, int C, int Ck, int H,
+                        const float* wq, const float* wk, const float* wv, void* o, int n_shared, gl_stream s) {
+    NEED(ctx);
+    GL_API_BEGIN
+    Engine& eng = *ctx->eng;
+    if (n_shared && (B % 2 != 0 || C % H != 0 || !attn_pair_supported(C / H, Nk, n_shared, attn_vt_layout(C / H, Nk, nullptr))))
+        throw GlError(GL_ERR_ARG, "gl_op_attention_pair: an even batch, head dim 40, more than two key tiles, exactly one of them behind the shared ones");
     Arena& ar = eng.arena();
     ar.reset();
     if (C % H != 0) throw GlError(GL_ERR_ARG, "C must be divisible by H");
@@ -1186,8 +1189,23 @@
     }
     AttnParams P = attn_params(bufs.q, bufs.k, bufs.vt, (bf16*)o, H, d, Nq, Nk, bufs.Tq_pad, bufs.Tk_pad, vt_layout);
     P.counters = eng.attn_counters();
-    ck(attn_launch(P, B, S(s)));
-    GL_API_END
+    if (n_shared) {
+        P.n_shared = n_shared;
+        P.Bp = B / 2;
+        ck(attn_pair_launch(P, B / 2, S(s)));
+    } else ck(attn_launch(P, B, S(s)));
+    GL_API_END
+}
+
+int gl_op_attention(gl_ctx* ctx, const void* xq, const void* xkv, int B, int Nq, int Nk, int C, int Ck, int H,
+                    const float* wq, const float* wk, const float* wv, void* o, gl_stream s) {
+    return op_attention(ctx, xq, xkv, B, Nq, Nk, C, Ck, H, wq, wk, wv, o, 0, s);
+}
+
+int gl_op_attention_pair(gl_ctx* ctx, const void* xq, const void* xkv, int B, int Nq, int Nk, int C, int Ck, int H,
+                         const float* wq, const float* wk, const float* wv, void* o, int n_shared, gl_stream s) {
+    if (n_shared <= 0) return gl::set_error(GL_ERR_ARG, "gl_op_attention_pair: n_shared = %d", n_shared);
+    return op_attention(ctx, xq, xkv, B, Nq, Nk, C, Ck, H, wq, wk, wv, o, n_shared, s);
 }
 
 int gl_attn_regime_counters(gl_ctx* ctx, int enable, unsigned* lazy_moves, unsigned* reruns) {
diff --git a/gligen_amd/csrc/engine.h b/gligen_amd/csrc/engine.h
--- a/gligen_amd/csrc/engine.h
+++ b/gligen_amd/csrc/engine.h
@@ -299,7 +299,9 @@
     bool qkv_rows_ok(const SelfAttnW& a, int B, int T, int Nk, int C, int d) const;
     void qkv_project_gemm(const SelfAttnW& a, const bf16* ln, int B, int T, int Nk, int C, int d, hipStream_t s, const RowStats* in_stats, int Tbuf, int slot);
     void qkv_rows_project(const SelfAttnW& a, const bf16* x, int B, int T, int Nk, int C, int d, const LinW& pre, const bf16* pre_res, bf16* mid,
-                          RowStats* mid_stats, int Tbuf, int slot, hipStream_t s, int Bin = 0);
+                          RowStats* mid_stats, int Tbuf, int slot, hipStream_t s, int Bin = 0, bool twin = false);
+    bool fuser_pair_ok(const STW& t, int B, int Bp, int HW) const;
+    void fuser_pair(const STW& t, const bf16* x, const bf16* res, bf16* mid, bf16* o, int Bp, int HW, hipStream_t s);
     float* emb_rows(const int64_t* t_dev, int R, float* out, hipStream_t s);
     void emb_table_build(const int64_t* t_host, int R, hipStream_t s);
     float* emb_table_ = nullptr;
@@ -309,7 +311,7 @@
     std::vector<int64_t> emb_t_cache_;
 
     bool ff_rows_for(const STW& t, int which, int B, int HW, hipStream_t s);
-    bool qkv_rows_for(const STW& t, int which, int B, int HW, int Nk, hipStream_t s);
+    bool qkv_rows_for(const STW& t, int which, int B, int HW, int Nk, hipStream_t s, int pair_Bp = 0);
     template <class Run>
     bool timed_form(uint64_t key, int M, int C, int n_zero, const char* name, int form, hipStream_t s, Run&& run);
 
diff --git a/gligen_amd/csrc/engine_policy.hip b/gligen_amd/csrc/engine_policy.hip
--- a/gligen_amd/csrc/engine_policy.hip
+++ b/gligen_amd/csrc/engine_policy.hip
@@ -46,7 +46,7 @@
     }
     return v;
 }
-static std::atomic<long long> count[3];
+static std::atomic<long long> count[4];
 }
 bool cfg_shared_prefix() { return cfg_prefix::current() != 0; }
 void cfg_shared_prefix_note(int what) { cfg_prefix::count[what].fetch_add(1); }
@@ -70,8 +70,8 @@
                               kv.second.rows ? "rows" : "gemm", kv.second.us_rows, kv.second.us_gemm);
     }
     if (n + 128 < cap)
-        snprintf(buf + n, cap - n, ";cfg_shared_prefix=%d evals=%lld rows_at_prefix=%lld rows_periodic=%lld", cfg_prefix::current(),
-                 cfg_prefix::count[0].load(), cfg_prefix::count[1].load(), cfg_prefix::count[2].load());
+        snprintf(buf + n, cap - n, ";pair_attn=%lld;cfg_shared_prefix=%d evals=%lld rows_at_prefix=%lld rows_periodic=%lld", cfg_prefix::count[3].load(),
+                 cfg_prefix::current(), cfg_prefix::count[0].load(), cfg_prefix::count[1].load(), cfg_prefix::count[2].load());
     return GL_OK;
 }
 
@@ -149,14 +149,18 @@
     });
 }
 
-bool Engine::qkv_rows_for(const STW& t, int which, int B, int HW, int Nk, hipStream_t s) {
+bool Engine::qkv_rows_for(const STW& t, int which, int B, int HW, int Nk, hipStream_t s, int pair_Bp) {
     const SelfAttnW& a = which ? t.fa : t.a1;
     const int M = B * HW, C = t.C, d = t.d;
-    if (!qkv_rows_ok(a, B, HW, Nk, C, d)) return false;
+    if (!qkv_rows_ok(a, pair_Bp ? pair_Bp : B, HW, Nk, C, d)) return false;
     if (qkv_rows_ >= 2) return true;
     const LinW& pre = which ? t.a1.out : t.proj_in;
     const int Tf = which ? round_up(Nk, 64) : 0, slot = which ? t.idx + 1 : 0;
-    return timed_form(ff_policy::key(device_, 3 + which, 0, C, M), M, C, 2, which ? "attn1.to_out+fuser.qkv" : "proj_in+attn1.qkv", -1, s, [&](bool rows, bf16* const* z) {
+    return timed_form(ff_policy::key(device_, 3 + which, pair_Bp ? 1 : 0, C, M), M, C, 2, which ? "attn1.to_out+fuser.qkv" : "proj_in+attn1.qkv", pair_Bp ? 1 : -1, s, [&](bool rows, bf16* const* z) {
+        if (rows && pair_Bp) {
+            fuser_pair(t, z[0], z[1], z[2], z[3], pair_Bp, HW, s);
+            return;
+        }
         if (rows) {
             qkv_rows_project(a, z[0], B, HW, Nk, C, d, pre, which ? z[1] : nullptr, z[2], nullptr, Tf, slot, s);
         } else {
diff --git a/gligen_amd/csrc/engine_unet.hip b/gligen_amd/csrc/engine_unet.hip
--- a/gligen_amd/csrc/engine_unet.hip
+++ b/gligen_amd/csrc/engine_unet.hip
@@ -307,16 +307,18 @@
 }
 
 void Engine::qkv_rows_project(const SelfAttnW& a, const bf16* x, int B, int T, int Nk, int C, int d, const LinW& pre, const bf16* pre_res, bf16* mid,
-                              RowStats* mid_stats, int Tbuf, int slot, hipStream_t s, int Bin) {
+                              RowStats* mid_stats, int Tbuf, int slot, hipStream_t s, int Bin, bool twin) {
     const int H = C / d, M = B * T;
+    if (twin && (Bin || mid_stats)) throw GlError(GL_ERR_STATE, "qkv_rows_project: the pair form takes prefix rows and writes no statistics");
     if (Bin < 0 || (Bin && B % Bin != 0)) throw GlError(GL_ERR_STATE, fmt("qkv_rows_project: %d input samples for a batch of %d", Bin, B));
     int dp, dpv;
     CK(attn_dims(d, &dp, &dpv));
     const int vt_layout = attn_vt_layout(d, Nk, &dpv);
-    AttnBufs& bufs = attn_bufs(B, H, d, Tbuf ? Tbuf : T, Tbuf ? Tbuf : T, dpv, slot);
+    AttnBufs& bufs = attn_bufs(twin ? 2 * B : B, H, d, Tbuf ? Tbuf : T, Tbuf ? Tbuf : T, dpv, slot);
     QkvRowsParams P{};
     P.x = x; P.ldx = C; P.eps = 1e-5f; P.stream = a.rows_stream; P.M = M;
     P.in_period = (Bin && Bin != B) ? Bin * T : 0;
+    P.mid_twin = twin ? M : 0;
     P.pre = 1; P.pre_b = pre.b; P.pre_res = pre_res; P.ld_pre_res = C; P.mid_out = mid; P.ld_mid = C;
     if (mid_stats) {
         *mid_stats = RowStats{};
@@ -335,6 +337,38 @@
         fprintf(launch_log, "qkv_rows_kernel<320, 40, true, 3>|%d|%d|%d|0|%.0f\n", M, 4 * C, C,
                 (double)qkv_rows_stream_bytes(C, true, 3) + (pre_res ? 6.0 : 4.0) * M * C + 2.0 * M * H * (2.0 * dp + dpv));
         fflush(launch_log);
+    }
+    ++n_launches;
+}
+
+static bool cfg_pair_attn() {
+    static const bool on = !(dev_env("GL_CFG_PAIR_ATTN") && atoi(dev_env("GL_CFG_PAIR_ATTN")) == 0);
+    return on;
+}
+
+bool Engine::fuser_pair_ok(const STW& t, int B, int Bp, int HW) const {
+    const int Nk = HW + cond_.Ng;
+    int dpv = 0;
+    return cfg_pair_attn() && B == 2 * Bp && HW % 64 == 0 && cond_.Ng > 0 && attn_vt_layout(t.d, Nk, &dpv) == 1 && attn_pair_supported(t.d, Nk, HW / 64, 1);
+}
+
+void Engine::fuser_pair(const STW& t, const bf16* x, const bf16* res, bf16* mid, bf16* o, int Bp, int HW, hipStream_t s) {
+    const int C = t.C, d = t.d, H = C / d, Nk = HW + cond_.Ng, Tf = round_up(Nk, 64);
+    qkv_rows_project(t.fa, x, Bp, HW, Nk, C, d, t.a1.out, res, mid, nullptr, Tf, t.idx + 1, s, 0, true);
+    int dp, dpv;
+    CK(attn_dims(d, &dp, &dpv));
+    const int vt_layout = attn_vt_layout(d, Nk, &dpv);
+    AttnBufs& bufs = attn_bufs(2 * Bp, H, d, Tf, Tf, dpv, t.idx + 1);
+    AttnParams P = attn_params(bufs.q, bufs.k, bufs.vt, o, H, d, HW, Nk, bufs.Tq_pad, bufs.Tk_pad, vt_layout);
+    P.n_shared = HW / 64;
+    P.Bp = Bp;
+    const char* sym = "attn3_pair_kernel<48, 48, true, 4>";
+    const double Ng = cond_.Ng;
+    ProfScope ps(this, s, sym, 4.0 * Bp * H * (double)HW * (HW + 2.0 * Ng) * d, 0.0);
+    CK(attn_pair_launch(P, Bp, s));
+    if (FILE* f = launch_log_file()) {
+        fprintf(f, "%s|%d|%d|%d|2|%.0f\n", sym, HW, Nk, d, 2.0 * Bp * H * d * (3.0 * HW + 4.0 * Ng + 2.0 * HW));
+        fflush(f);
     }
     ++n_launches;
 }
@@ -578,7 +612,8 @@
     }
     }
     const int Ng = cond_.Ng;
-    const bool rq2 = !fuser_off_ && unet_.cfg.fuser_kind == 0 && fuser_hoist_ && aligned && cond_.Ng > 0 && qkv_rows_for(t, 1, B, HW, HW + Ng, s);
+    const bool pair = shared && !fuser_off_ && fuser_pair_ok(t, B, Bp, HW);
+    const bool rq2 = !fuser_off_ && unet_.cfg.fuser_kind == 0 && fuser_hoist_ && aligned && cond_.Ng > 0 && qkv_rows_for(t, 1, B, HW, HW + Ng, s, pair ? Bp : 0);
     if (shared && !rq2) {
         replicate(o, o + (size_t)Mp * C, (size_t)Mp * C, B / Bp - 1, s);
         bf16* t0b = arena_.get<bf16>((size_t)M * C);
@@ -594,7 +629,12 @@
         st3 = st1;
     } else if (unet_.cfg.fuser_kind == 0) {
         const int Tf = round_up(HW + Ng, 64);
-        if (rq2) {
+        if (rq2 && pair) {
+            ensure_fuser_kv(t, B, HW, s);
+            fuser_pair(t, o, t0, t1, o, Bp, HW, s);
+            cfg_shared_prefix_note(2);
+            cfg_shared_prefix_note(3);
+        } else if (rq2) {
             ensure_fuser_kv(t, B, HW, s);
             qkv_rows_project(t.fa, o, B, HW, HW + Ng, C, d, t.a1.out, t0, t1, nullptr, Tf, t.idx + 1, s, shared ? Bp : 0);
             if (shared) cfg_shared_prefix_note(2);
diff --git a/gligen_amd/csrc/ffn.h b/gligen_amd/csrc/ffn.h
--- a/gligen_amd/csrc/ffn.h
+++ b/gligen_amd/csrc/ffn.h
@@ -60,6 +60,7 @@
     bf16* vt;
     int H, d, DP, DPV, T, Tpad_q, Tpad_k, vt_perm32;
     int in_period;
+    int mid_twin;
 };
 bool qkv_rows_supported(int M, int C, int d, int T);
 size_t qkv_rows_stream_bytes(int C, bool pre, int np);
diff --git a/gligen_amd/csrc/ffn.hip b/gligen_amd/csrc/ffn.hip
--- a/gligen_amd/csrc/ffn.hip
+++ b/gligen_amd/csrc/ffn.hip
@@ -817,7 +817,10 @@
                     ss = fmaf(t_, t_, ss);
                 }
                 if constexpr (GL_QKV_ABL & 2) asm volatile("" ::"v"(o.u.x), "v"(o.u.y));
-                else *reinterpret_cast<uint2*>(mrow + cb * 32 + j * 8) = o.u;
+                else {
+                    *reinterpret_cast<uint2*>(mrow + cb * 32 + j * 8) = o.u;
+                    if (p.mid_twin) *reinterpret_cast<uint2*>(mrow + (size_t)p.mid_twin * p.ld_mid + cb * 32 + j * 8) = o.u;
+                }
             }
         }
         s += __shfl_xor(s, 32, 64);
@@ -1023,7 +1026,8 @@
     if (p.np == 3 && (p.vt_perm32 != 1 || p.Tpad_k % 32)) return set_error(GL_ERR_UNSUPPORTED, "qkv_rows: v^T is written in the 32-token form only (attn3_kernel)");
     if (p.H * p.d != C || p.DP < p.d || p.DP % 8 || (p.np == 3 && p.DPV < p.d)) return set_error(GL_ERR_ARG, "qkv_rows: head geometry");
     if (p.pre && (!p.pre_b || !p.mid_out || p.ld_mid % 4 || (p.pre_res && p.ld_pre_res % 4))) return set_error(GL_ERR_ARG, "qkv_rows: the leading projection needs its bias and the buffer for its result");
-    if (p.in_period < 0 || (p.in_period && (p.in_period % p.T || p.M % p.in_period))) return set_error(GL_ERR_ARG, "qkv_rows: the input period must be whole samples and divide M");
+    if (p.mid_twin < 0 || (p.mid_twin && (!p.pre || p.stats_out || p.mid_twin < p.M))) return set_error(GL_ERR_ARG, "qkv_rows: a second copy of t needs the leading projection, no statistics, and rows behind the launch's own");
+    if (p.in_period < 0 || (p.in_period &&(p.in_period % p.T || p.M % p.in_period))) return set_error(GL_ERR_ARG, "qkv_rows: the input period must be whole samples and divide M");
     using G = FFGeom<320>;
     constexpr int LDS = 3 * G::PJ_BLK * 1024 + 4 * 320 * (int)sizeof(float);
     const dim3 grid(p.M / 128), block(256);
diff --git a/gligen_amd/engine.py b/gligen_amd/engine.py
--- a/gligen_amd/engine.py
+++ b/gligen_amd/engine.py
@@ -1066,6 +1066,14 @@
                                        _ptr(o), _stream(self.device)))
         return o
 
+    def op_attention_pair(self, xq, xkv, wq, wk, wv, heads, n_shared):
+        B, Nq, Cc = xq.shape
+        _, Nk, Ck = xkv.shape
+        o = torch.empty((B, Nq, Cc), device=xq.device, dtype=torch.bfloat16)
+        check(self.lib.gl_op_attention_pair(self._ctx, _ptr(xq), _ptr(xkv), B, Nq, Nk, Cc, Ck, heads, _ptr(wq), _ptr(wk), _ptr(wv),
+                                            _ptr(o), n_shared, _stream(self.device)))
+        return o
+
     def attn_regime_counters(self, enable):
         lazy, reruns = C.c_uint(0), C.c_uint(0)
         check(self.lib.gl_attn_regime_counters(self._ctx, 1 if enable else 0, C.byref(lazy), C.byref(reruns)))
diff --git a/include/gligen_amd_pair.h b/include/gligen_amd_pair.h
--- /dev/null
+++ b/include/gligen_amd_pair.h
@@ -0,0 +1,15 @@
+#ifndef GLIGEN_AMD_PAIR_H
+#define GLIGEN_AMD_PAIR_H
+#include "gligen_amd.h"
+
+#ifdef __cplusplus
+extern "C" {
+#endif
+
+int gl_op_attention_pair(gl_ctx* ctx, const void* xq, const void* xkv, int B, int Nq, int Nk, int C, int Ck, int H,
+                         const float* wq, const float* wk, const float* wv, void* o, int n_shared, gl_stream s);
+
+#ifdef __cplusplus
+}
+#endif
+#endif
```

New measurement: 6.644 images/s, median of 6. About the same (+0.8%).
